# martellab-sri/ModalTune

Measured on AMD Instinct MI355X. Metric: slides/sec (train step) at 10k patches x 1536-d, higher is better.
Workload: dtype f16; 1 GPU; Prov-GigaPath ModalAdapter train step, 10000 patches x 1536-d, 6 pathways -> 64 gene tokens + 1 task token, 3 task passes, fp16 operands / fp32 accumulate, 1 slide per GPU per step, task passes as two concurrent groups (B = 2 | 1 on two HIP streams), train mode: Dropout(0.25) on the embedded input and both backbone branches, DropPath(0..0.1) per layer and on the Extractor FFN (Philox masks regener; patches=10000, parallelism=dp1, dropout=True

## Files before the change

include/modaltune_hip.h:

```cpp
#ifndef MODALTUNE_HIP_H
#define MODALTUNE_HIP_H

#include <stdint.h>

#ifdef __cplusplus
extern "C" {
#endif

typedef void* mt_stream_t;
typedef uint16_t mt_half;

typedef enum {
  MT_OK = 0,
  MT_ERR_BAD_ARG = -1,
  MT_ERR_LAUNCH = -2,
  MT_ERR_UNSUPPORTED = -3
} MtStatus;

typedef struct { int seg_rows, seg_stride, row0; } MtRowMap;

int mt_version(void);
const char* mt_status_string(int status);
const char* mt_build_id(void);

// ... 60 lines not shown
  float* rowsum;
  float* pre_out;
  const float* resid;
  MtDropout c_drop;
  const float* a_aux; int a_act;
  MtDropout a_drop;
  float resid_scale; int a_ld;
} MtSgemm;
int mt_sgemm_multi(const MtSgemm* probs, int n, mt_stream_t stream);

int mt_layernorm_fwd(const void* x, long ldx, const MtRowMap* xmap, int in_dtype, int gelu_in, const float* w,
                     const float* b, const float* add_rows, int add_period, void* y, long ldy, const MtRowMap* ymap,
                     int out_dtype, float* stats, int M, int D, mt_stream_t stream);
int mt_layernorm_fwd_live(const void* x, long ldx, const MtRowMap* xmap, int in_dtype, int gelu_in, const float* w,
                          const float* b, const float* add_rows, int add_period, void* y, long ldy, const MtRowMap* ymap,
                          int out_dtype, float* stats, int M, int D, const int* live, int live_rows, mt_stream_t stream);
int mt_add_layernorm_fwd(const float* x, const mt_half* branch, const MtDropout* drop, const float* w, const float* b,
                         float* h, mt_half* y, float* stats, int M, int D, mt_stream_t stream);

int mt_layernorm_fwd_eps(const void* x, long ldx, const MtRowMap* xmap, int in_dtype, int gelu_in, const float* w,
                         const float* b, const float* add_rows, int add_period, void* y, long ldy, const MtRowMap* ymap,
                         int out_dtype, float* stats, int M, int D, float eps, mt_stream_t stream);
int mt_add_layernorm_fwd_eps(const float* x, const mt_half* branch, const MtDropout* drop, const float* w, const float* b,
                             float* h, mt_half* y, float* stats, int M, int D, float eps, mt_stream_t stream);

int mt_layernorm_bwd(const void* dy, long lddy, const MtRowMap* dymap, int dy_dtype, const void* x, long ldx,
                     const MtRowMap* xmap, int in_dtype, int gelu_in, const float* w, const float* stats, void* dx,
                     long lddx, const MtRowMap* dxmap, int dx_dtype, int accumulate, float* dw, float* db,
                     mt_half* dx_f16, const MtDropout* dx_f16_drop, int M, int D, mt_stream_t stream);

int mt_layernorm_bwd_live(const void* dy, long lddy, const MtRowMap* dymap, int dy_dtype, const void* x, long ldx,
                          const MtRowMap* xmap, int in_dtype, int gelu_in, const float* w, const float* stats, void* dx,
                          long lddx, const MtRowMap* dxmap, int dx_dtype, int accumulate, float* dw, float* db,
                          mt_half* dx_f16, const MtDropout* dx_f16_drop, int M, int D, const int* live, int live_rows,
                          mt_stream_t stream);

#define MT_MAX_BRANCHES 8
#define MT_QK_SCALE_LOG2 0.20823509396846288f
typedef struct {
  int nbranch;
  int N;
  int B;
  int seg[MT_MAX_BRANCHES];
  int ratio[MT_MAX_BRANCHES];
  int nseg[MT_MAX_BRANCHES];
  int n[MT_MAX_BRANCHES];
  int qlimit[MT_MAX_BRANCHES];
} MtDilatedPlan;

int mt_dilated_attn_fwd(const mt_half* qkv, const MtDilatedPlan* plan, mt_half* o_br, float* lse_br,
                        mt_stream_t stream);

int mt_dilated_attn_fwd_live(const mt_half* qkv, const MtDilatedPlan* plan, mt_half* o_br, float* lse_br, const int* live,
                             mt_stream_t stream);

int mt_dilated_mix_ln_fwd(const mt_half* o_br, const float* lse_br, const MtDilatedPlan* plan, const float* ln_w,
                          const float* ln_b, mt_half* y, float* stats, float* lse_tot, mt_stream_t stream);

int mt_dilated_mix_ln_bwd(const mt_half* dy, const mt_half* o_br, const float* lse_br, const float* lse_tot,
                          const MtDilatedPlan* plan, const float* ln_w, const float* stats, mt_half* dmixed,
                          float* delta_br, mt_stream_t stream);
int mt_dilated_mix_ln_fwd_live(const mt_half* o_br, const float* lse_br, const MtDilatedPlan* plan, const float* ln_w,
                               const float* ln_b, mt_half* y, float* stats, float* lse_tot, const int* live, mt_stream_t stream);
int mt_dilated_mix_ln_bwd_live(const mt_half* dy, const mt_half* o_br, const float* lse_br, const float* lse_tot,
                               const MtDilatedPlan* plan, const float* ln_w, const float* stats, mt_half* dmixed,
                               float* delta_br, const int* live, mt_stream_t stream);
int mt_dilated_mix_ln_fwd_grid(const mt_half* o_br, const float* lse_br, const MtDilatedPlan* plan, const float* ln_w,
                               const float* ln_b, mt_half* y, float* stats, float* lse_tot, int grid_wgs, mt_stream_t stream);
int mt_dilated_mix_ln_bwd_grid(const mt_half* dy, const mt_half* o_br, const float* lse_br, const float* lse_tot,
                               const MtDilatedPlan* plan, const float* ln_w, const float* stats, mt_half* dmixed,
                               float* delta_br, int grid_wgs, mt_stream_t stream);

long mt_dilated_attn_bwd_workspace_bytes(const MtDilatedPlan* plan);
enum { MT_ATTN_BWD_KV = 1, MT_ATTN_BWD_Q = 2, MT_ATTN_BWD_COMBINE = 4, MT_ATTN_BWD_ALL = 7 };
int mt_dilated_attn_bwd(const mt_half* qkv, const mt_half* dmixed, const float* lse_tot, const float* delta_br,
                        const MtDilatedPlan* plan, void* workspace, mt_half* dqkv, int phases, mt_stream_t stream);
int mt_dilated_attn_bwd_inplace(const mt_half* qkv, const mt_half* dmixed, const float* lse_tot, const float* delta_br,
                                const MtDilatedPlan* plan, void* workspace, mt_half* dqkv, int phases, mt_stream_t stream);

int mt_dilated_attn_bwd_inplace_live(const mt_half* qkv, const mt_half* dmixed, const float* lse_tot, const float* delta_br,
                                     const MtDilatedPlan* plan, void* workspace, mt_half* dqkv, int phases, const int* live,
                                     mt_stream_t stream);

#define MT_DENSE_QK_SCALE_LOG2 0.18033688011112042f
typedef struct {
  int N;
  int B;
  int H;
  const mt_half* dist;
  const float* nslope;
} MtDensePlan;
long mt_alibi_dist_halves(int N);
int mt_alibi_dist(const int* cells, int N, mt_half* table, mt_stream_t stream);
int mt_dense_attn_fwd(const mt_half* qkv, const MtDensePlan* plan, mt_half* o, float* lse, mt_stream_t stream);
enum { MT_DENSE_BWD_DELTA = 1, MT_DENSE_BWD_KV = 2, MT_DENSE_BWD_Q = 4, MT_DENSE_BWD_ALL = 7 };
int mt_dense_attn_bwd(const mt_half* qkv, const mt_half* o, const mt_half* d_o, const float* lse, const MtDensePlan* plan,
                      float* delta, mt_half* dqkv, int phases, mt_stream_t stream);

int mt_gelu_f16_fwd(const mt_half* x, mt_half* y, long n, mt_stream_t stream);
int mt_gelu_f16_bwd(const mt_half* x, const mt_half* dy, mt_half* dx, long n, mt_stream_t stream);

long mt_pool_attn_workspace_floats(int B, int N, int heads, int nq);
int mt_pool_attn_fwd(const float* q, const mt_half* kv, int B, int N, int E, int heads, int nq, float* out, float* scores,
                     float* lse, float* workspace, mt_stream_t stream);
int mt_pool_attn_bwd(const float* q, const mt_half* kv, const float* scores, const float* lse, const float* out,
                     const float* dout, int B, int N, int E, int heads, int nq, mt_half* dkv, mt_stream_t stream);

typedef struct {
  const float *ln1_w, *ln1_b, *inner_ln_w, *inner_ln_b, *ln2_w, *ln2_b, *ffn_ln_w, *ffn_ln_b;
  const float *b_qkv, *b_out, *b_fc1, *b_fc2;
  const mt_half *w_qkv, *w_out, *w_fc1, *w_fc2;
  const mt_half *wt_qkv, *wt_out, *wt_fc1, *wt_fc2;
} MtLongNetLayerWeights;
typedef struct {
  float *hin, *hmid; mt_half *qkv, *o_br; float *lse_br, *lse_tot; mt_half* a1; float *st1, *stin, *st2, *stf;
  mt_half *u16, *br16, *t16;
  float* dh; mt_half *dy16, *dh16, *dt16, *da1, *dmixed, *dqkv16; float* delta; void* attn_ws;
  const int *live_attn, *live_ffn;
} MtLongNetLayerBuffers;
enum { MT_LAYER_ALL = 0x7fffffff };
enum { MT_LNF_LN1 = 1 << 0, MT_LNF_QKV = 1 << 1, MT_LNF_ATTN = 1 << 2, MT_LNF_MIX = 1 << 3, MT_LNF_OUT = 1 << 4, MT_LNF_LN2 = 1 << 5,
       MT_LNF_FC1 = 1 << 6, MT_LNF_FFN_LN = 1 << 7, MT_LNF_FC2 = 1 << 8 };
int mt_longnet_layer_fwd(const MtLongNetLayerWeights* w, const MtLongNetLayerBuffers* b, const MtDilatedPlan* plan, int M, int D, int F,
                         const float* pend_x, const mt_half* pend_branch, const MtDropout* pend_drop, int defer, float* out,
                         const MtDropout* drop_attn, const MtDropout* drop_ffn, int steps, mt_stream_t stream);
enum { MT_LNB_CAST = 1 << 0, MT_LNB_FC2 = 1 << 1, MT_LNB_FFN_LN = 1 << 2, MT_LNB_FC1 = 1 << 3, MT_LNB_LN2 = 1 << 4, MT_LNB_OUT = 1 << 5,
       MT_LNB_MIX = 1 << 6, MT_LNB_ATTN_SHIFT = 7, MT_LNB_QKV = 1 << 10, MT_LNB_LN1 = 1 << 11 };
int mt_longnet_layer_bwd(const MtLongNetLayerWeights* w, const MtLongNetLayerBuffers* b, const MtDilatedPlan* plan, int M, int D, int F,
                         int dh16_valid, int feeds_lower, const MtDropout* drop_attn, const MtDropout* drop_ffn,
                         const MtDropout* drop_lower_ffn, int steps, mt_stream_t stream);
typedef struct {
  const float *n1_w, *n1_b, *n2_w, *n2_b; float n1_eps, n2_eps;
  const float *b_qkv, *b_proj, *b_fc1, *b_fc2;
  const mt_half *w_qkv, *w_proj, *w_fc1, *w_fc2;
  const mt_half *wt_qkv, *wt_proj, *wt_fc1, *wt_fc2;
} MtVitBlockWeights;
typedef struct {
  float *hin, *hmid; mt_half *qkv, *o16; float* lse; mt_half* a1; float *st1, *st2;
  mt_half *u16, *br16, *t16;
  float* dh; mt_half *dy16, *dh16, *dt16, *da1, *dqkv16; float* delta;
} MtVitBlockBuffers;
enum { MT_VBF_LN1 = 1 << 0, MT_VBF_QKV = 1 << 1, MT_VBF_ATTN = 1 << 2, MT_VBF_PROJ = 1 << 3, MT_VBF_LN2 = 1 << 4, MT_VBF_FC1 = 1 << 5,
       MT_VBF_GELU = 1 << 6, MT_VBF_FC2 = 1 << 7 };
int mt_vit_block_fwd(const MtVitBlockWeights* w, const MtVitBlockBuffers* b, const MtDensePlan* plan, int M, int D, int F,
                     const float* pend_x, const mt_half* pend_branch, int defer, float* out, int steps, mt_stream_t stream);
enum { MT_VBB_CAST = 1 << 0, MT_VBB_FC2 = 1 << 1, MT_VBB_GELU = 1 << 2, MT_VBB_FC1 = 1 << 3, MT_VBB_LN2 = 1 << 4, MT_VBB_PROJ = 1 << 5,
       MT_VBB_ATTN_SHIFT = 6, MT_VBB_QKV = 1 << 9, MT_VBB_LN1 = 1 << 10 };
int mt_vit_block_bwd(const MtVitBlockWeights* w, const MtVitBlockBuffers* b, const MtDensePlan* plan, int M, int D, int F,
                     int dh16_valid, int feeds_lower, int steps, mt_stream_t stream);

int mt_inject_attn_fwd(const mt_half* q, int M, int rows_per_pass, const float* k, const float* v, int T,
                       mt_half* a, float* lse, mt_stream_t stream);
int mt_inject_attn_bwd(const mt_half* q, const mt_half* a, const float* lse, const mt_half* da, int M,
                       int rows_per_pass, const float* k, const float* v, int T, mt_half* dq, float* dk, float* dv,
                       mt_stream_t stream);

int mt_extract_attn_fwd(const float* q, const mt_half* kv, int B, int T, int L, float* out, float* lse,
                        float* part_acc, float* part_ml, int nsplit, mt_stream_t stream);
int mt_extract_attn_bwd(const float* q, const mt_half* kv, const float* out, const float* lse, const float* dout,
                        int B, int T, int L, float* dq, mt_half* dkv, mt_stream_t stream);

int mt_inject_attn_fwd_hd(const mt_half* q, int M, int rows_per_pass, const float* k, const float* v, int T, int heads,
                          int head_dim, mt_half* a, float* lse, mt_stream_t stream);
int mt_inject_attn_bwd_hd(const mt_half* q, const mt_half* a, const float* lse, const mt_half* da, int M,
                          int rows_per_pass, const float* k, const float* v, int T, int heads, int head_dim, mt_half* dq,
                          float* dk, float* dv, mt_stream_t stream);
int mt_extract_attn_fwd_hd(const float* q, const mt_half* kv, int B, int T, int L, int heads, int head_dim, float* out,
                           float* lse, float* part_acc, float* part_ml, int nsplit, mt_stream_t stream);
int mt_extract_attn_bwd_hd(const float* q, const mt_half* kv, const float* out, const float* lse, const float* dout,
                           int B, int T, int L, int heads, int head_dim, float* dq, mt_half* dkv, mt_stream_t stream);

int mt_gene_snn_fwd(const float* params, const long* offs, const int* sizes, const long* goff, const float* genes, int G,
                    int latent, int passes, float* a1, float* a2, float* z, const MtDropout* alpha_drop, mt_stream_t stream);
int mt_gene_snn_bwd(const float* params, float* grads, const long* offs, const int* sizes, const long* goff,
                    const float* genes, int G, int latent, int passes, const float* a1, const float* a2, const float* dz,
                    const MtDropout* alpha_drop, mt_stream_t stream);

int mt_gene_snn_fwd_points(const float* params, const long* offs, const int* sizes, const long* goff, const float* genes,
                           const float* baseline, const float* alphas, int G, int latent, int points, float* a1, float* a2, float* z,
                           mt_stream_t stream);
int mt_gene_snn_bwd_input(const float* params, const long* offs, const int* sizes, const long* goff, int G, int latent, int points,
                          const float* a1, const float* a2, const float* dz, const float* weights, const float* unscale,
                          float* dgenes, int accumulate, mt_stream_t stream);
int mt_ig_finalize(const float* genes, const float* baseline, const float* dgenes, const int* sizes, const long* goff, int G,
                   float* attr, float* pathway, mt_stream_t stream);

int mt_token_mha_fwd(const float* q, const float* k, const float* v, int B, int T, int E, int heads, float* out,
                     float* probs, mt_stream_t stream);
int mt_token_mha_bwd(const float* q, const float* k, const float* v, const float* probs, const float* dout, int B,
                     int T, int E, int heads, float* dq, float* dk, float* dv, mt_stream_t stream);

int mt_extract_attn_probs(const float* q, const mt_half* kv, const float* lse, int B, int T, int L, float* w, mt_stream_t stream);
int mt_inject_attn_probs(const mt_half* q, int M, int rows_per_pass, const float* k, const float* lse, int T, float* w,
                         mt_stream_t stream);
int mt_extract_attn_probs_hd(const float* q, const mt_half* kv, const float* lse, int B, int T, int L, int heads,
                             int head_dim, float* w, mt_stream_t stream);
int mt_inject_attn_probs_hd(const mt_half* q, int M, int rows_per_pass, const float* k, const float* lse, int T, int heads,
                            int head_dim, float* w, mt_stream_t stream);
int mt_token_probs_mean(const float* probs, int B, int heads, int T, float* out, mt_stream_t stream);

int mt_cast_f32_to_f16(const float* x, mt_half* y, long n, const MtDropout* drop, int D, mt_stream_t stream);
// ... 75 lines not shown
```

modaltune_amd/_lib.py:

```python
from __future__ import annotations

import ctypes as C
import os

_HERE = os.path.dirname(os.path.abspath(__file__))
LIB_PATH = os.environ.get("MODALTUNE_HIP_LIB", os.path.join(_HERE, "_C", "libmodaltune_hip.so"))

P, I, L, F, D = C.c_void_p, C.c_int, C.c_long, C.c_float, C.c_double


class MtRowMap(C.Structure):
    _fields_ = [("seg_rows", I), ("seg_stride", I), ("row0", I)]


class MtDropout(C.Structure):
    _fields_ = [("rng", P), ("site", C.c_uint), ("p", F), ("path_site", C.c_uint), ("path_p", F), ("rows_per_pass", I)]


class MtGemmEpilogue(C.Structure):
    _fields_ = [("bias", P), ("resid", P), ("ldr", L), ("rmap", MtRowMap), ("colscale", P),
                ("pos_table", P), ("pos_row", P), ("pos_col", P), ("drop", MtDropout)]


MT_SGEMM_MAX = 3


class MtSgemm(C.Structure):
    _fields_ = [("A", P), ("as0", L), ("as1", L), ("a_bs", L), ("B", P), ("bs0", L), ("bs1", L), ("b_bs", L),
                ("bias", P), ("bias_on_m", I), ("C", P), ("cs0", L), ("cs1", L), ("c_bs", L),
                ("M", I), ("N", I), ("K", I), ("batch", I), ("act", I), ("accumulate", I),
                ("rowsum", P), ("pre_out", P), ("resid", P), ("c_drop", MtDropout),
                ("a_aux", P), ("a_act", I), ("a_drop", MtDropout), ("resid_scale", F), ("a_ld", I)]


MT_MAX_BRANCHES = 8


class MtDilatedPlan(C.Structure):
    _fields_ = [("nbranch", I), ("N", I), ("B", I), ("seg", I * MT_MAX_BRANCHES), ("ratio", I * MT_MAX_BRANCHES),
                ("nseg", I * MT_MAX_BRANCHES), ("n", I * MT_MAX_BRANCHES), ("qlimit", I * MT_MAX_BRANCHES)]


class MtDensePlan(C.Structure):
    _fields_ = [("N", I), ("B", I), ("H", I), ("dist", P), ("nslope", P)]


class MtLongNetLayerWeights(C.Structure):
    _fields_ = [(n, P) for n in ("ln1_w", "ln1_b", "inner_ln_w", "inner_ln_b", "ln2_w", "ln2_b", "ffn_ln_w", "ffn_ln_b", "b_qkv", "b_out",
                                 "b_fc1", "b_fc2", "w_qkv", "w_out", "w_fc1", "w_fc2", "wt_qkv", "wt_out", "wt_fc1", "wt_fc2")]


class MtLongNetLayerBuffers(C.Structure):
    _fields_ = [(n, P) for n in ("hin", "hmid", "qkv", "o_br", "lse_br", "lse_tot", "a1", "st1", "stin", "st2", "stf", "u16", "br16", "t16",
                                 "dh", "dy16", "dh16", "dt16", "da1", "dmixed", "dqkv16", "delta", "attn_ws", "live_attn", "live_ffn")]


class MtVitBlockWeights(C.Structure):
    _fields_ = [(n, P) for n in ("n1_w", "n1_b", "n2_w", "n2_b")] + [("n1_eps", F), ("n2_eps", F)] + \
               [(n, P) for n in ("b_qkv", "b_proj", "b_fc1", "b_fc2", "w_qkv", "w_proj", "w_fc1", "w_fc2", "wt_qkv", "wt_proj", "wt_fc1", "wt_fc2")]


class MtVitBlockBuffers(C.Structure):
    _fields_ = [(n, P) for n in ("hin", "hmid", "qkv", "o16", "lse", "a1", "st1", "st2", "u16", "br16", "t16", "dh", "dy16", "dh16", "dt16",
                                 "da1", "dqkv16", "delta")]


RM = C.POINTER(MtRowMap)
DR = C.POINTER(MtDropout)
EP = C.POINTER(MtGemmEpilogue)
PL = C.POINTER(MtDilatedPlan)
DP = C.POINTER(MtDensePlan)

SIGNATURES = {
    "mt_version": [],
    "mt_status_string": [I],
    "mt_build_id": [],
    "mt_gemm_nt_f16": [P, L, RM, P, I, I, I, I, EP, P, L, RM, I, P],
    "mt_gemm_tn_f16": [P, L, RM, P, L, RM, I, I, I, P, L, P, P],
    "mt_colsum_f16": [P, L, RM, I, I, P, P],
    "mt_sgemm_small": [P, L, L, L, P, L, L, L, P, I, P, L, L, L, I, I, I, I, I, I, P, P],
    "mt_sgemm_multi": [C.POINTER(MtSgemm), I, P],
    "mt_layernorm_fwd": [P, L, RM, I, I, P, P, P, I, P, L, RM, I, P, I, I, P],
    "mt_add_layernorm_fwd": [P, P, DR, P, P, P, P, P, I, I, P],
    "mt_layernorm_fwd_eps": [P, L, RM, I, I, P, P, P, I, P, L, RM, I, P, I, I, F, P],
    "mt_add_layernorm_fwd_eps": [P, P, DR, P, P, P, P, P, I, I, F, P],
    "mt_layernorm_bwd": [P, L, RM, I, P, L, RM, I, I, P, P, P, L, RM, I, I, P, P, P, DR, I, I, P],
    "mt_droppath_live": [P, P, I, I, P, P, P],
    "mt_gemm_nt_f16_live": [P, L, RM, P, I, I, I, I, EP, P, L, RM, I, P, I, P],
    "mt_layernorm_fwd_live": [P, L, RM, I, I, P, P, P, I, P, L, RM, I, P, I, I, P, I, P],
    "mt_layernorm_bwd_live": [P, L, RM, I, P, L, RM, I, I, P, P, P, L, RM, I, I, P, P, P, DR, I, I, P, I, P],
    "mt_dilated_attn_fwd_live": [P, PL, P, P, P, P],
    "mt_dilated_mix_ln_fwd_live": [P, P, PL, P, P, P, P, P, P, P],
    "mt_dilated_mix_ln_bwd_live": [P, P, P, P, PL, P, P, P, P, P, P],
    "mt_dilated_attn_bwd_inplace_live": [P, P, P, P, PL, P, P, I, P, P],
    "mt_dilated_attn_fwd": [P, PL, P, P, P],
    "mt_dilated_mix_ln_fwd": [P, P, PL, P, P, P, P, P, P],
    "mt_dilated_mix_ln_bwd": [P, P, P, P, PL, P, P, P, P, P],
    "mt_dilated_mix_ln_fwd_grid": [P, P, PL, P, P, P, P, P, I, P],
    "mt_dilated_mix_ln_bwd_grid": [P, P, P, P, PL, P, P, P, P, I, P],
    "mt_dilated_attn_bwd_workspace_bytes": [PL],
    "mt_dilated_attn_bwd": [P, P, P, P, PL, P, P, I, P],
    "mt_dilated_attn_bwd_inplace": [P, P, P, P, PL, P, P, I, P],
    "mt_gene_snn_fwd": [P, P, P, P, P, I, I, I, P, P, P, DR, P],
    "mt_gene_snn_bwd": [P, P, P, P, P, P, I, I, I, P, P, P, DR, P],
    "mt_gene_snn_fwd_points": [P, P, P, P, P, P, P, I, I, I, P, P, P, P],
    "mt_gene_snn_bwd_input": [P, P, P, P, I, I, I, P, P, P, P, P, P, I, P],
    "mt_ig_finalize": [P, P, P, P, P, I, P, P, P],
    "mt_inject_attn_fwd": [P, I, I, P, P, I, P, P, P],
    "mt_inject_attn_bwd": [P, P, P, P, I, I, P, P, I, P, P, P, P],
    "mt_extract_attn_fwd": [P, P, I, I, I, P, P, P, P, I, P],
    "mt_extract_attn_bwd": [P, P, P, P, P, I, I, I, P, P, P],
    "mt_inject_attn_fwd_hd": [P, I, I, P, P, I, I, I, P, P, P],
    "mt_inject_attn_bwd_hd": [P, P, P, P, I, I, P, P, I, I, I, P, P, P, P],
    "mt_extract_attn_fwd_hd": [P, P, I, I, I, I, I, P, P, P, P, I, P],
    "mt_extract_attn_bwd_hd": [P, P, P, P, P, I, I, I, I, I, P, P, P],
    "mt_token_mha_fwd": [P, P, P, I, I, I, I, P, P, P],
    "mt_token_mha_bwd": [P, P, P, P, P, I, I, I, I, P, P, P, P],
    "mt_extract_attn_probs": [P, P, P, I, I, I, P, P],
    "mt_inject_attn_probs": [P, I, I, P, P, I, P, P],
    "mt_extract_attn_probs_hd": [P, P, P, I, I, I, I, I, P, P],
    "mt_inject_attn_probs_hd": [P, I, I, P, P, I, I, I, P, P],
    "mt_token_probs_mean": [P, I, I, I, P, P],
    "mt_cast_f32_to_f16": [P, P, L, DR, I, P],
    "mt_rng_advance": [P, P],
    "mt_dropout_f32": [P, L, RM, P, I, I, DR, P],
    "mt_droppath_rows_f32": [P, I, I, DR, P],
    "mt_cast_f16_to_f32": [P, P, L, P],
    "mt_pack_weight_f16": [P, I, I, P, I, P],
    "mt_pack_weights_f16": [P, I, P],
    "mt_act_fwd": [P, P, L, I, P],
    "mt_act_bwd": [P, P, P, L, I, P],
    "mt_axpy": [P, P, F, P, L, P],
    "mt_axpy_bcast": [P, P, F, P, L, L, P],
    "mt_fold_rows": [P, I, L, P, P],
    "mt_copy_rows_f32": [P, L, RM, P, L, RM, I, I, I, P],
    "mt_inject_resid_bwd": [P, L, RM, P, L, RM, P, P, P, L, RM, I, P, P, I, I, P],
    "mt_l2norm_rows": [P, P, I, I, P],
    "mt_distill_loss": [P, P, I, I, F, P, P, P, P],
    "mt_adamw_step": [P, P, P, P, L, D, D, D, D, D, I, P, F, P, P, P, P],
    "mt_scaler_update": [P, P, P, P, F, F, I, P],
    "mt_check_finite": [P, L, P, P],
    "mt_absmax_scale": [P, L, F, P, P],
    "mt_axpy_dev": [P, P, P, P, L, P],
    "mt_coords_to_grid": [P, I, F, I, P, P, P, P],
    "mt_mfma_probe": [P, I, I, P],
    "mt_longnet_layer_fwd": [P, P, PL, I, I, I, P, P, DR, I, P, DR, DR, I, P],
    "mt_longnet_layer_bwd": [P, P, PL, I, I, I, I, I, DR, DR, DR, I, P],
    "mt_vit_block_fwd": [P, P, DP, I, I, I, P, P, I, P, I, P],
    "mt_vit_block_bwd": [P, P, DP, I, I, I, I, I, I, P],
    "mt_alibi_dist": [P, I, P, P],
    "mt_alibi_dist_halves": [I],
    "mt_dense_attn_fwd": [P, DP, P, P, P],
    "mt_dense_attn_bwd": [P, P, P, P, DP, P, P, I, P],
    "mt_gelu_f16_fwd": [P, P, L, P],
    "mt_gelu_f16_bwd": [P, P, P, L, P],
    "mt_pool_attn_workspace_floats": [I, I, I, I],
    "mt_pool_attn_fwd": [P, P, I, I, I, I, I, P, P, P, P, P],
    "mt_pool_attn_bwd": [P, P, P, P, P, P, I, I, I, I, I, P, P],
    "mt_titan_grid": [P, I, F, P, P, P, P],
    "mt_titan_cell_sums": [P, L, P, I, I, P, P, P, P, P],
    "mt_titan_token_order": [P, P, P, I, P, P, P, P],
    "mt_titan_gather_tokens": [P, P, I, I, P, P],
    "mt_scatter_rows_f32": [P, P, P, P, I, I, I, P],
    "mt_row_absmax_f32": [P, P, I, I, P],
    "mt_gemm_tn_f16_det_elems": [I, I, I, I],
    "mt_gemm_tn_f16_det": [P, L, RM, P, L, RM, I, I, I, P, L, P, P, L, P],
    "mt_colsum_f16_det_elems": [I, I],
    "mt_colsum_f16_det": [P, L, RM, I, I, P, P, L, P],
    "mt_layernorm_bwd_det_elems": [I, I],
    "mt_layernorm_bwd_det": [P, L, RM, I, P, L, RM, I, I, P, P, P, L, RM, I, I, P, P, P, DR, I, I, P, L, P],
    "mt_inject_resid_bwd_det_elems": [I, I],
    "mt_inject_resid_bwd_det": [P, L, RM, P, L, RM, P, P, P, L, RM, I, P, P, I, I, P, L, P],
    "mt_inject_attn_bwd_hd_det_elems": [I, I, I, I, I],
    "mt_inject_attn_bwd_hd_det": [P, P, P, P, I, I, P, P, I, I, I, P, P, P, P, L, P],
    "mt_extract_attn_bwd_hd_det_elems": [I, I, I, I, I],
    "mt_extract_attn_bwd_hd_det": [P, P, P, P, P, I, I, I, I, I, P, P, P, L, P],
}
_RESTYPE = {"mt_status_string": C.c_char_p, "mt_build_id": C.c_char_p, "mt_dilated_attn_bwd_workspace_bytes": C.c_long, "mt_pool_attn_workspace_floats": C.c_long,
             "mt_alibi_dist_halves": C.c_long,
             **{n + "_det_elems": C.c_long for n in ("mt_gemm_tn_f16", "mt_colsum_f16", "mt_layernorm_bwd", "mt_inject_resid_bwd",
                                                     "mt_inject_attn_bwd_hd", "mt_extract_attn_bwd_hd")}}

_lib = None


def load():
    global _lib
    if _lib is not None:
        return _lib
    import torch
    if not os.path.exists(LIB_PATH):
        raise RuntimeError(
            f"modaltune_amd: {LIB_PATH} is missing -- run `python __graft_entry__.py` (hipcc, gfx950) first; "
            "there is no CPU/PyTorch fallback for the hot path")
    lib = C.CDLL(LIB_PATH)
    for name, args in SIGNATURES.items():
        fn = getattr(lib, name)
        fn.argtypes = args
        fn.restype = _RESTYPE.get(name, I)
    _lib = lib
    return lib


def build_info() -> dict:
    from ._build_id import tree_build_id
    bid = load().mt_build_id().decode()
    try:
        ok = bid == tree_build_id()
    except Exception:
        ok = None
    return {"build_id": bid, "build_id_matches_tree": ok, "lib": os.path.relpath(LIB_PATH, os.path.dirname(_HERE))}


def check(status: int, what: str = ""):
    if status != 0:
        msg = load().mt_status_string(status).decode()
        raise RuntimeError(f"modaltune_hip {what} failed: {msg} ({status})")


def rowmap(seg_rows=0, seg_stride=0, row0=0):
    return MtRowMap(seg_rows, seg_stride, row0)
```

modaltune_amd/csrc/attn.hip:

```cpp
#include "attn_common.h"

namespace {

template <bool LIVE>
__global__ __launch_bounds__(256) void dilated_attn_fwd_kernel(const h16* __restrict__ qkv, Plan p, h16* __restrict__ o_br,
                                                               float* __restrict__ lse_br) {
  __shared__ __attribute__((aligned(16))) h16 smem[4 * IMG_HALVES];
  h16* const Ks = smem;
  h16* const Vs = smem + 2 * IMG_HALVES;
  const int tid = threadIdx.x, lane = tid & 63, wave = tid >> 6;
  const int hh = lane >> 5, l31 = lane & 31;
  const WorkItem w = decode(p, blockIdx.x);
  const Seq sq = make_seq(p, w);
  const long M = (long)p.B * p.N;
  const int nv = __builtin_amdgcn_readfirstlane(sq.nvalid());
  const int nvq = min(nv, p.qlimit[w.br]);
  if (w.qt * 128 >= nvq || (LIVE && pass_dead(p, w.b))) return;

  {
    const int buf = tid >> 7, row = (tid >> 1) & 63, which = 6 + (tid & 1);
    const h16x8 one = {(h16)1.f, 0, 0, 0, (h16)1.f, 0, 0, 0}, zero = {0, 0, 0, 0, 0, 0, 0, 0};
    *reinterpret_cast<h16x8*>(&Vs[buf * IMG_HALVES + img_off(row, which)]) = which == 6 ? one : zero;
  }

  const int iq = w.qt * 128 + wave * 32 + l31;
  const bool qvalid = sq.valid(iq) && iq < nvq;
  const long qrow = sq.row_clamped(iq);
  h16x8 qf[3];
#pragma unroll
  for (int ks = 0; ks < 3; ++ks)
    qf[ks] = sel8(qvalid, ldg8(hm_ptr(qkv, M, w.h, qrow) + ks * 16 + hh * 8));

  const int ntile = (sq.n + 63) / 64;
  const int nproc = (nv + 63) >> 6;
  const int row_bytes = sq.dr * HD * 2;
  const long valid_bytes = (long)(nv - 1) * row_bytes + HD * 2;
  const long tile_bytes = 64L * row_bytes;
  const h16* const kseq = hm_ptr(qkv, M, H + w.h, sq.row(0));
  const h16* const vseq = hm_ptr(qkv, M, 2 * H + w.h, sq.row(0));
  const DmaLane dl(tid, row_bytes);
  auto dma = [&](int t) {
    dma_tile(Ks + (t & 1) * IMG_HALVES, tile_rsrc(kseq, t * tile_bytes, valid_bytes), dl);
    dma_tile(Vs + (t & 1) * IMG_HALVES, tile_rsrc(vseq, t * tile_bytes, valid_bytes), dl);
  };
  const int grp = lane >> 4, li = lane & 15, tq = li >> 2, tp = li & 3;
  int krd[3];
#pragma unroll
  for (int ks = 0; ks < 3; ++ks) krd[ks] = img_off(l31, 2 * ks + hh);
  const int vc = 2 * (grp & 1) + (tp >> 1), vo = 4 * (tp & 1);
  const int va0 = img_off(4 * hh + tq, vc) + vo, va1 = img_off(4 * hh + tq, vc + 4) + vo;
  const int vb0 = img_off(4 * hh + tq + 8, vc) + vo, vb1 = img_off(4 * hh + tq + 8, vc + 4) + vo;

  auto qk = [&](const h16* Kb, f32x16 (&s)[2], const f32x16& init) {
#pragma unroll
    for (int sub = 0; sub < 2; ++sub) {
#pragma unroll
      for (int ks = 0; ks < 3; ++ks) {
        const h16x8 kf = *reinterpret_cast<const h16x8*>(&Kb[sub * 32 * IMG_ROW + krd[ks]]);
        s[sub] = __builtin_amdgcn_mfma_f32_32x32x16_f16(kf, qf[ks], ks == 0 ? init : s[sub], 0, 0, 0);
      }
    }
  };

  f32x16 o0, o1;
#pragma unroll
  for (int i = 0; i < 16; ++i) { o0[i] = 0.f; o1[i] = 0.f; }

  dma(0);
  dma_wait_all();
  __syncthreads();
  float m2;
  f32x16 minit;
  {
    f32x16 s0[2], zero;
#pragma unroll
    for (int i = 0; i < 16; ++i) zero[i] = 0.f;
    qk(Ks, s0, zero);
    float mx = NEG_BIG;
#pragma unroll
    for (int sub = 0; sub < 2; ++sub)
#pragma unroll
      for (int i = 0; i < 16; ++i) {
        const int kidx = sub * 32 + (i & 3) + 8 * (i >> 2) + 4 * hh;
        mx = fmaxf(mx, kidx < sq.n ? s0[sub][i] : NEG_BIG);
      }
    m2 = max_halves(mx);
#pragma unroll
    for (int i = 0; i < 16; ++i) minit[i] = -m2;
  }

  auto tile = [&](int t, auto tail_tag) {
    constexpr bool TAIL = decltype(tail_tag)::value;
    const int kb = t * 64;
    const h16* Kb = Ks + (t & 1) * IMG_HALVES;
    const h16* Vb = Vs + (t & 1) * IMG_HALVES;
    if (t + 1 < nproc) dma(t + 1);
    f32x16 s_cur[2];
    qk(Kb, s_cur, minit);
    float mx = NEG_BIG;
#pragma unroll
    for (int sub = 0; sub < 2; ++sub)
#pragma unroll
      for (int i = 0; i < 16; ++i) {
        if (TAIL) {
          const int kidx = kb + sub * 32 + (i & 3) + 8 * (i >> 2) + 4 * hh;
          if (kidx >= sq.n) s_cur[sub][i] = NEG_BIG;
        }
        mx = fmaxf(mx, s_cur[sub][i]);
      }
    mx = max_halves(mx);
    if (__any(mx > RESCALE_LOG2)) {
      const float up = fmaxf(mx, 0.f);
      const float alpha = __builtin_amdgcn_exp2f(-up);
#pragma unroll
      for (int i = 0; i < 16; ++i) { o0[i] *= alpha; o1[i] *= alpha; s_cur[0][i] -= up; s_cur[1][i] -= up; }
      m2 += up;
#pragma unroll
      for (int i = 0; i < 16; ++i) minit[i] = -m2;
    }
#pragma unroll
    for (int sub = 0; sub < 2; ++sub)
#pragma unroll
      for (int s2 = 0; s2 < 2; ++s2) {
        h16x8 pf;
#pragma unroll
        for (int e = 0; e < 8; e += 2) {
          const f32x2 a = pk_exp2((f32x2){s_cur[sub][8 * s2 + e], s_cur[sub][8 * s2 + e + 1]});
          pf[e] = (h16)a[0]; pf[e + 1] = (h16)a[1];
        }
        const h16* vblk = Vb + (sub * 32 + s2 * 16) * IMG_ROW;
        const h16x8 v0 = cat8(lds_tr4(vblk + va0), lds_tr4(vblk + vb0));
        const h16x8 v1 = cat8(lds_tr4(vblk + va1), lds_tr4(vblk + vb1));
        o0 = __builtin_amdgcn_mfma_f32_32x32x16_f16(v0, pf, o0, 0, 0, 0);
        o1 = __builtin_amdgcn_mfma_f32_32x32x16_f16(v1, pf, o1, 0, 0, 0);
      }
    dma_wait_all();
    __syncthreads();
  };
  const bool tail_last = nproc == ntile && (sq.n & 63);
  const int nplain = tail_last ? nproc - 1 : nproc;
  for (int t = 0; t < nplain; ++t) tile(t, std::false_type{});
  if (tail_last) tile(nproc - 1, std::true_type{});
  const int rest = sq.n - nproc * 64;
  if (rest > 0) {
    if (__any(-m2 > RESCALE_LOG2)) {
      const float up = fmaxf(-m2, 0.f);
      const float alpha = __builtin_amdgcn_exp2f(-up);
#pragma unroll
      for (int i = 0; i < 16; ++i) { o0[i] *= alpha; o1[i] *= alpha; }
      m2 += up;
    }
    o1[8] += (float)rest * __builtin_amdgcn_exp2f(-m2);
  }

  if (qvalid) {
    const float l = o1[8];
    const float inv = 1.0f / l;
    h16* orow = o_br + ((long)w.br * M + qrow) * DM + w.h * HD;
#pragma unroll
    for (int gq = 0; gq < 4; ++gq) {
      h16x4 v = {(h16)(o0[4 * gq] * inv), (h16)(o0[4 * gq + 1] * inv), (h16)(o0[4 * gq + 2] * inv), (h16)(o0[4 * gq + 3] * inv)};
      *reinterpret_cast<h16x4*>(orow + 8 * gq + 4 * hh) = v;
    }
#pragma unroll
    for (int gq = 0; gq < 2; ++gq) {
      h16x4 v = {(h16)(o1[4 * gq] * inv), (h16)(o1[4 * gq + 1] * inv), (h16)(o1[4 * gq + 2] * inv), (h16)(o1[4 * gq + 3] * inv)};
      *reinterpret_cast<h16x4*>(orow + 32 + 8 * gq + 4 * hh) = v;
    }
    if (hh == 0) lse_br[((long)w.br * M + qrow) * H + w.h] = (m2 + __log2f(l)) * LN2;
  }
}

struct MixGeom {
  int grp[MT_MAX_BRANCHES];
  MT_DEVINL MixGeom(const Plan& p, int h) {
#pragma unroll
    for (int b = 0; b < MT_MAX_BRANCHES; ++b) grp[b] = b < p.nbranch ? h / (H / p.ratio[b]) : -1;
  }
};
MT_DEVINL void seg_split(const Plan& p, int b, int pos, int& j, int& loc) {
  const int sg = p.seg[b];
  if (sg >= p.N) { j = 0; loc = pos; return; }
  j = (int)((float)pos * p.inv_seg[b]);
  loc = pos - j * sg;
  if (loc < 0) { loc += sg; --j; }
  if (loc >= sg) { loc -= sg; ++j; }
}
MT_DEVINL int residue(const Plan& p, int b, int pos) {
  int j, loc;
  seg_split(p, b, pos, j, loc);
  const int dr = p.ratio[b];
  return (dr & (dr - 1)) == 0 ? (loc & (dr - 1)) : loc % dr;
}
MT_DEVINL int dense_branch(const Plan& p) {
  int d = 0;
#pragma unroll
  for (int b = 0; b < MT_MAX_BRANCHES; ++b) if (b < p.nbranch && p.ratio[b] == 1) d = b;
  return d;
}
constexpr int MIX_CPL = 24;
struct H24 { h16x8 a, b, c; };
MT_DEVINL H24 ld24(const h16* p) {
  return H24{*reinterpret_cast<const h16x8*>(p), *reinterpret_cast<const h16x8*>(p + 8), *reinterpret_cast<const h16x8*>(p + 16)};
}
MT_DEVINL float h24(const H24& v, int e) { return (float)(e < 8 ? v.a[e & 7] : e < 16 ? v.b[e & 7] : v.c[e & 7]); }
MT_DEVINL float half_sum(float v) {
#pragma unroll
  for (int o = 16; o > 0; o >>= 1) v += __shfl_xor(v, o, 64);
  return v;
}

template <int NB>
__global__ __launch_bounds__(256) void mix_ln_fwd_kernel(const h16* __restrict__ o_br, const float* __restrict__ lse_br, Plan p,
                                                         const float* __restrict__ ln_w, const float* __restrict__ ln_b,
                                                         h16* __restrict__ y, float* __restrict__ stats, float* __restrict__ lse_tot) {
  const int lane = threadIdx.x & 63, wave = __builtin_amdgcn_readfirstlane(threadIdx.x >> 6), sub = lane >> 5, l5 = lane & 31;
  const long M = (long)p.B * p.N;
  const int h = l5 >> 1, c0 = l5 * MIX_CPL;
  const MixGeom geo(p, h);
  const int db = dense_branch(p);
  float w[MIX_CPL], bb[MIX_CPL];
#pragma unroll
  for (int e = 0; e < MIX_CPL; ++e) { w[e] = ln_w[c0 + e]; bb[e] = ln_b[c0 + e]; }
  const LivePasses lp = live_passes(p);
  const long m_end = min(M, (long)lp.b1 * p.N);
  for (long m2 = (long)lp.b0 * p.N + ((long)blockIdx.x * 4 + wave) * 2; m2 < m_end; m2 += (long)gridDim.x * 8) {
    const bool live = m2 + sub < m_end;
    const long m = live ? m2 + sub : m_end - 1;
    const int pos = (int)(m % p.N);
    bool cov[NB];
    float lse[NB];
    H24 ob[NB];
#pragma unroll
    for (int b = 0; b < NB; ++b) {
      cov[b] = b < p.nbranch && geo.grp[b] == residue(p, b, pos);
      const int sb = cov[b] ? b : db;
      lse[b] = lse_br[((long)sb * M + m) * H + h];
      ob[b] = ld24(o_br + ((long)sb * M + m) * DM + c0);
    }
    float mx = NEG_BIG;
#pragma unroll
    for (int b = 0; b < NB; ++b) { lse[b] = cov[b] ? lse[b] : NEG_BIG; mx = fmaxf(mx, lse[b]); }
    float den = 0.f;
#pragma unroll
    for (int b = 0; b < NB; ++b) den += cov[b] ? __expf(lse[b] - mx) : 0.f;
    const float tot = mx + __logf(den);
    float v[MIX_CPL];
#pragma unroll
    for (int e = 0; e < MIX_CPL; ++e) v[e] = 0.f;
#pragma unroll
    for (int b = 0; b < NB; ++b) {
      const float wgt = cov[b] ? __expf(lse[b] - tot) : 0.f;
#pragma unroll
      for (int e = 0; e < MIX_CPL; ++e) v[e] = fmaf(wgt, cov[b] ? h24(ob[b], e) : 0.f, v[e]);
    }
    float s = 0.f;
#pragma unroll
    for (int e = 0; e < MIX_CPL; ++e) s += v[e];
    const float mean = half_sum(s) * (1.0f / DM);
    float q = 0.f;
#pragma unroll
    for (int e = 0; e < MIX_CPL; ++e) { const float d = v[e] - mean; q += d * d; }
    const float rstd = rsqrtf(half_sum(q) * (1.0f / DM) + 1e-5f);
    if (live) {
      h16* dst = y + m * DM + c0;
#pragma unroll
      for (int k = 0; k < 3; ++k) {
        h16x8 o;
#pragma unroll
        for (int e = 0; e < 8; ++e) o[e] = (h16)((v[8 * k + e] - mean) * rstd * w[8 * k + e] + bb[8 * k + e]);
        *reinterpret_cast<h16x8*>(dst + 8 * k) = o;
      }
      if (l5 == 0) { stats[2 * m] = mean; stats[2 * m + 1] = rstd; }
      if ((l5 & 1) == 0) lse_tot[m * H + h] = tot;
    }
  }
}

template <int NB>
__global__ __launch_bounds__(256) void mix_ln_bwd_kernel(const h16* __restrict__ dy, const h16* __restrict__ o_br,
                                                         const float* __restrict__ lse_br, const float* __restrict__ lse_tot, Plan p,
                                                         const float* __restrict__ ln_w, const float* __restrict__ stats,
                                                         h16* __restrict__ dmixed, float* __restrict__ delta_br) {
  const int lane = threadIdx.x & 63, wave = __builtin_amdgcn_readfirstlane(threadIdx.x >> 6), sub = lane >> 5, l5 = lane & 31;
  const long M = (long)p.B * p.N;
  const int h = l5 >> 1, c0 = l5 * MIX_CPL;
  const MixGeom geo(p, h);
  const int db = dense_branch(p);
  float w[MIX_CPL];
#pragma unroll
  for (int e = 0; e < MIX_CPL; ++e) w[e] = ln_w[c0 + e];
  const LivePasses lp = live_passes(p);
  const long m_end = min(M, (long)lp.b1 * p.N);
  for (long m2 = (long)lp.b0 * p.N + ((long)blockIdx.x * 4 + wave) * 2; m2 < m_end; m2 += (long)gridDim.x * 8) {
    const bool live = m2 + sub < m_end;
    const long m = live ? m2 + sub : m_end - 1;
    const int pos = (int)(m % p.N);
    const float tot = lse_tot[m * H + h];
    const float mean = stats[2 * m], rstd = stats[2 * m + 1];
    const H24 dyv = ld24(dy + m * DM + c0);
    bool cov[NB];
    float lse[NB];
    H24 ob[NB];
#pragma unroll
    for (int b = 0; b < NB; ++b) {
      cov[b] = b < p.nbranch && geo.grp[b] == residue(p, b, pos);
      const int sb = cov[b] ? b : db;
      lse[b] = lse_br[((long)sb * M + m) * H + h];
      ob[b] = ld24(o_br + ((long)sb * M + m) * DM + c0);
    }
    float v[MIX_CPL];
#pragma unroll
    for (int e = 0; e < MIX_CPL; ++e) v[e] = 0.f;
#pragma unroll
    for (int b = 0; b < NB; ++b) {
      const float wgt = cov[b] ? __expf(lse[b] - tot) : 0.f;
#pragma unroll
      for (int e = 0; e < MIX_CPL; ++e) v[e] = fmaf(wgt, cov[b] ? h24(ob[b], e) : 0.f, v[e]);
    }
    float g[MIX_CPL], xh[MIX_CPL];
    float s1 = 0.f, s2 = 0.f;
#pragma unroll
    for (int i = 0; i < MIX_CPL; ++i) {
      xh[i] = (v[i] - mean) * rstd;
      g[i] = h24(dyv, i) * w[i];
      s1 += g[i]; s2 = fmaf(g[i], xh[i], s2);
    }
    const float c1 = half_sum(s1) * (1.0f / DM), c2 = half_sum(s2) * (1.0f / DM);
    float dm[MIX_CPL];
    h16* dst = dmixed + ((long)h * M + m) * HD + (c0 - h * HD);
#pragma unroll
    for (int k = 0; k < 3; ++k) {
      h16x8 o;
#pragma unroll
      for (int e = 0; e < 8; ++e) {
        const int i = 8 * k + e;
        o[e] = (h16)(rstd * (g[i] - c1 - xh[i] * c2));
        dm[i] = (float)o[e];
      }
      if (live) *reinterpret_cast<h16x8*>(dst + 8 * k) = o;
    }
#pragma unroll
    for (int b = 0; b < NB; ++b) {
      float d = 0.f;
#pragma unroll
      for (int e = 0; e < MIX_CPL; ++e) d = fmaf(dm[e], h24(ob[b], e), d);
      d += __shfl_xor(d, 1, 64);
      if (live && (l5 & 1) == 0 && cov[b]) delta_br[((long)b * M + m) * H + h] = d;
    }
  }
}


}

extern "C" int mt_dilated_attn_fwd_live(const mt_half* qkv, const MtDilatedPlan* plan, mt_half* o_br, float* lse_br, const int* live,
                                        mt_stream_t stream) {
  if (!qkv || !o_br || !lse_br || !plan_ok(plan)) return MT_ERR_BAD_ARG;
  const Plan p = make_plan(plan, 128, live);
  const int nblk = p.blk_off[p.nbranch];
  if (p.live) hipLaunchKernelGGL(dilated_attn_fwd_kernel<true>, dim3(nblk), dim3(256), 0, (hipStream_t)stream, (const h16*)qkv, p,
                     (h16*)o_br, lse_br);
  else hipLaunchKernelGGL(dilated_attn_fwd_kernel<false>, dim3(nblk), dim3(256), 0, (hipStream_t)stream, (const h16*)qkv, p,
                     (h16*)o_br, lse_br);
  MT_CHECK_LAUNCH();
  return MT_OK;
}

extern "C" int mt_dilated_attn_fwd(const mt_half* qkv, const MtDilatedPlan* plan, mt_half* o_br, float* lse_br,
                                   mt_stream_t stream) {
  return mt_dilated_attn_fwd_live(qkv, plan, o_br, lse_br, nullptr, stream);
}

constexpr int MIX_CUS = 256, MIX_FWD_WG_PER_CU = 3, MIX_BWD_WG_PER_CU = 2;
static dim3 mix_grid(long M, int grid_wgs, int wg_per_cu) {
  return dim3((int)min((M + 7) / 8, (long)(grid_wgs > 0 ? grid_wgs : wg_per_cu * MIX_CUS)));
}

namespace {
int mix_ln_fwd(const mt_half* o_br, const float* lse_br, const MtDilatedPlan* plan, const float* ln_w, const float* ln_b, mt_half* y,
               float* stats, float* lse_tot, int grid_wgs, const int* live, mt_stream_t stream) {
  if (!o_br || !lse_br || !ln_w || !ln_b || !y || !stats || !lse_tot || !plan_ok(plan)) return MT_ERR_BAD_ARG;
  const Plan p = make_plan(plan, 128, live);
  const long M = (long)p.B * p.N;
  const dim3 grid = mix_grid(M, grid_wgs, MIX_FWD_WG_PER_CU);
  if (p.nbranch <= 5)
    hipLaunchKernelGGL(mix_ln_fwd_kernel<5>, grid, dim3(256), 0, (hipStream_t)stream, (const h16*)o_br, lse_br, p, ln_w, ln_b,
                       (h16*)y, stats, lse_tot);
  else
    hipLaunchKernelGGL(mix_ln_fwd_kernel<MT_MAX_BRANCHES>, grid, dim3(256), 0, (hipStream_t)stream, (const h16*)o_br, lse_br, p,
                       ln_w, ln_b, (h16*)y, stats, lse_tot);
  MT_CHECK_LAUNCH();
  return MT_OK;
}
}

extern "C" int mt_dilated_mix_ln_fwd_grid(const mt_half* o_br, const float* lse_br, const MtDilatedPlan* plan,
                                          const float* ln_w, const float* ln_b, mt_half* y, float* stats, float* lse_tot,
                                          int grid_wgs, mt_stream_t stream) {
  return mix_ln_fwd(o_br, lse_br, plan, ln_w, ln_b, y, stats, lse_tot, grid_wgs, nullptr, stream);
}

extern "C" int mt_dilated_mix_ln_fwd(const mt_half* o_br, const float* lse_br, const MtDilatedPlan* plan,
                                     const float* ln_w, const float* ln_b, mt_half* y, float* stats, float* lse_tot,
                                     mt_stream_t stream) {
  return mix_ln_fwd(o_br, lse_br, plan, ln_w, ln_b, y, stats, lse_tot, 0, nullptr, stream);
}

extern "C" int mt_dilated_mix_ln_fwd_live(const mt_half* o_br, const float* lse_br, const MtDilatedPlan* plan,
                                          const float* ln_w, const float* ln_b, mt_half* y, float* stats, float* lse_tot,
                                          const int* live, mt_stream_t stream) {
  return mix_ln_fwd(o_br, lse_br, plan, ln_w, ln_b, y, stats, lse_tot, 0, live, stream);
}

namespace {
int mix_ln_bwd(const mt_half* dy, const mt_half* o_br, const float* lse_br, const float* lse_tot, const MtDilatedPlan* plan,
               const float* ln_w, const float* stats, mt_half* dmixed, float* delta_br, int grid_wgs, const int* live, mt_stream_t stream) {
  if (!dy || !o_br || !lse_br || !lse_tot || !ln_w || !stats || !dmixed || !delta_br || !plan_ok(plan)) return MT_ERR_BAD_ARG;
  const Plan p = make_plan(plan, 128, live);
  const long M = (long)p.B * p.N;
  const dim3 grid = mix_grid(M, grid_wgs, MIX_BWD_WG_PER_CU);
  if (p.nbranch <= 5)
    hipLaunchKernelGGL(mix_ln_bwd_kernel<5>, grid, dim3(256), 0, (hipStream_t)stream, (const h16*)dy, (const h16*)o_br, lse_br,
                       lse_tot, p, ln_w, stats, (h16*)dmixed, delta_br);
  else
    hipLaunchKernelGGL(mix_ln_bwd_kernel<MT_MAX_BRANCHES>, grid, dim3(256), 0, (hipStream_t)stream, (const h16*)dy,
                       (const h16*)o_br, lse_br, lse_tot, p, ln_w, stats, (h16*)dmixed, delta_br);
  MT_CHECK_LAUNCH();
  return MT_OK;
}
}

extern "C" int mt_dilated_mix_ln_bwd_grid(const mt_half* dy, const mt_half* o_br, const float* lse_br, const float* lse_tot,
                                          const MtDilatedPlan* plan, const float* ln_w, const float* stats, mt_half* dmixed,
                                          float* delta_br, int grid_wgs, mt_stream_t stream) {
  return mix_ln_bwd(dy, o_br, lse_br, lse_tot, plan, ln_w, stats, dmixed, delta_br, grid_wgs, nullptr, stream);
}

extern "C" int mt_dilated_mix_ln_bwd(const mt_half* dy, const mt_half* o_br, const float* lse_br, const float* lse_tot,
                                     const MtDilatedPlan* plan, const float* ln_w, const float* stats, mt_half* dmixed,
                                     float* delta_br, mt_stream_t stream) {
  return mix_ln_bwd(dy, o_br, lse_br, lse_tot, plan, ln_w, stats, dmixed, delta_br, 0, nullptr, stream);
}

extern "C" int mt_dilated_mix_ln_bwd_live(const mt_half* dy, const mt_half* o_br, const float* lse_br, const float* lse_tot,
                                          const MtDilatedPlan* plan, const float* ln_w, const float* stats, mt_half* dmixed,
                                          float* delta_br, const int* live, mt_stream_t stream) {
  return mix_ln_bwd(dy, o_br, lse_br, lse_tot, plan, ln_w, stats, dmixed, delta_br, 0, live, stream);
}

extern "C" long mt_dilated_attn_bwd_workspace_bytes(const MtDilatedPlan* plan) {
  if (!plan_ok(plan)) return MT_ERR_BAD_ARG;
  const Plan p = make_plan(plan, 128);
  return p.ws_off[p.nbranch] * (long)sizeof(h16);
}

namespace {
int attn_bwd(const mt_half* qkv, const mt_half* dmixed, const float* lse_tot, const float* delta_br, const MtDilatedPlan* plan,
             void* workspace, mt_half* dqkv, int phases, bool inplace, const int* live, mt_stream_t stream) {
  if (!qkv || !dmixed || !lse_tot || !delta_br || !workspace || !dqkv || !plan_ok(plan) || !(phases & 7)) return MT_ERR_BAD_ARG;
  hipStream_t s = (hipStream_t)stream;
  inplace = inplace && dense_branch_host(plan) >= 0;
  if (inplace && (long)plan->B * plan->N >= (1L << 31)) return MT_ERR_UNSUPPORTED;
  mt_half* dense_dst = inplace ? dqkv : nullptr;
  if (phases & MT_ATTN_BWD_KV) mt_attn::launch_bwd_kv(qkv, dmixed, lse_tot, delta_br, plan, workspace, dense_dst, live, s);
  if (phases & MT_ATTN_BWD_Q) mt_attn::launch_bwd_q(qkv, dmixed, lse_tot, delta_br, plan, workspace, dense_dst, live, s);
  if (phases & MT_ATTN_BWD_COMBINE) {
    if (inplace) mt_attn::launch_bwd_combine_inplace(workspace, plan, dqkv, live, s);
    else mt_attn::launch_bwd_combine(workspace, plan, dqkv, s);
  }
  MT_CHECK_LAUNCH();
  return MT_OK;
}
}

extern "C" int mt_dilated_attn_bwd(const mt_half* qkv, const mt_half* dmixed, const float* lse_tot,
                                   const float* delta_br, const MtDilatedPlan* plan, void* workspace, mt_half* dqkv,
                                   int phases, mt_stream_t stream) {
  return attn_bwd(qkv, dmixed, lse_tot, delta_br, plan, workspace, dqkv, phases, false, nullptr, stream);
}

extern "C" int mt_dilated_attn_bwd_inplace(const mt_half* qkv, const mt_half* dmixed, const float* lse_tot,
                                           const float* delta_br, const MtDilatedPlan* plan, void* workspace, mt_half* dqkv,
                                           int phases, mt_stream_t stream) {
  return attn_bwd(qkv, dmixed, lse_tot, delta_br, plan, workspace, dqkv, phases, true, nullptr, stream);
}

extern "C" int mt_dilated_attn_bwd_inplace_live(const mt_half* qkv, const mt_half* dmixed, const float* lse_tot,
                                                const float* delta_br, const MtDilatedPlan* plan, void* workspace, mt_half* dqkv,
                                                int phases, const int* live, mt_stream_t stream) {
  return attn_bwd(qkv, dmixed, lse_tot, delta_br, plan, workspace, dqkv, phases, true, live, stream);
}
```

modaltune_amd/csrc/attn_bwd_kv.hip:

```cpp
#include "attn_common.h"

namespace {

template <bool LIVE>
__global__ __launch_bounds__(256, 3) void dilated_attn_bwd_kv_kernel(const h16* __restrict__ qkv, const h16* __restrict__ dmixed,
                                                                  const float* __restrict__ lse_tot, const float* __restrict__ delta_br,
                                                                  Plan p, h16* __restrict__ ws, DenseDst dd) {
  __shared__ __attribute__((aligned(16))) h16 smem[4 * IMG_HALVES];
  __shared__ __attribute__((aligned(16))) float L2s[2][64];
  __shared__ __attribute__((aligned(16))) float Dls[2][64];
  h16* const Qx = smem;
  h16* const Dx = smem + 2 * IMG_HALVES;
  const int tid = threadIdx.x, lane = tid & 63, wave = tid >> 6;
  const int hh = lane >> 5, l31 = lane & 31;
  const WorkItem w = decode(p, blockIdx.x);
  const Seq sq = make_seq(p, w);
  const long M = (long)p.B * p.N;
  const h16x8 zero8 = {0, 0, 0, 0, 0, 0, 0, 0};
  const int nv = __builtin_amdgcn_readfirstlane(sq.nvalid());
  if (w.qt * 128 >= nv || (LIVE && pass_dead(p, w.b))) return;

  {
    const int img = tid >> 6, row = tid & 63;
    *reinterpret_cast<h16x8*>(&smem[img * IMG_HALVES + img_off(row, 6)]) = zero8;
    *reinterpret_cast<h16x8*>(&smem[img * IMG_HALVES + img_off(row, 7)]) = zero8;
  }

  const int ik = w.qt * 128 + wave * 32 + l31;
  const bool kvalid = sq.valid(ik);
  const long krow = sq.row_clamped(ik);
  h16x8 kf[3], vf[3];
#pragma unroll
  for (int ks = 0; ks < 3; ++ks) {
    kf[ks] = sel8(kvalid, ldg8(hm_ptr(qkv, M, H + w.h, krow) + ks * 16 + hh * 8));
    vf[ks] = sel8(kvalid, ldg8(hm_ptr(qkv, M, 2 * H + w.h, krow) + ks * 16 + hh * 8));
  }

  const int nvq = min(nv, p.qlimit[w.br]);
  const int ntile = (nvq + 63) >> 6;
  const int row_bytes = sq.dr * HD * 2;
  const long valid_bytes = (long)(nvq - 1) * row_bytes + HD * 2;
  const long tile_bytes = 64L * row_bytes;
  const h16* const qseq = hm_ptr(qkv, M, w.h, sq.row(0));
  const h16* const dseq = hm_ptr(dmixed, M, w.h, sq.row(0));
  const DmaLane dl(tid, row_bytes);
  const float* const lbase = lse_tot + sq.row(0) * H + w.h;
  const float* const dbase = delta_br + ((long)w.br * M + sq.row(0)) * H + w.h;
  float rl2 = 0.f, rdl = 0.f;
  auto issue = [&](int t) {
    dma_tile(Qx + (t & 1) * IMG_HALVES, tile_rsrc(qseq, t * tile_bytes, valid_bytes), dl);
    dma_tile(Dx + (t & 1) * IMG_HALVES, tile_rsrc(dseq, t * tile_bytes, valid_bytes), dl);
    if (tid < 64) {
      const long off = (long)min(t * 64 + lane, nvq - 1) * sq.dr * H;
      rl2 = lbase[off];
      rdl = dbase[off];
    }
  };
  auto publish = [&](int t) {
    if (tid < 64) {
      const bool ok = t * 64 + lane < nvq;
      L2s[t & 1][tid] = ok ? fmaf(-rl2, LOG2E, LOG2_LN2) : 0.f;
      Dls[t & 1][tid] = ok ? -rdl : 0.f;
    }
  };

  f32x16 dk0, dk1, dv0, dv1;
#pragma unroll
  for (int i = 0; i < 16; ++i) { dk0[i] = 0.f; dk1[i] = 0.f; dv0[i] = 0.f; dv1[i] = 0.f; }
  const int grp = lane >> 4, li = lane & 15, tq = li >> 2, tp = li & 3;
  int rrd[3];
#pragma unroll
  for (int ks = 0; ks < 3; ++ks) rrd[ks] = img_off(l31, 2 * ks + hh);
  const int trc = 2 * (grp & 1) + (tp >> 1), tro = 4 * (tp & 1);
  const int tr_a0 = img_off(4 * hh + tq, trc) + tro, tr_a1 = img_off(4 * hh + tq, trc + 4) + tro;
  const int tr_b0 = img_off(4 * hh + tq + 8, trc) + tro, tr_b1 = img_off(4 * hh + tq + 8, trc + 4) + tro;

  issue(0);
  publish(0);
  dma_wait_all();
  __syncthreads();
  for (int t = 0; t < ntile; ++t) {
    const h16* Qb = Qx + (t & 1) * IMG_HALVES;
    const h16* Db = Dx + (t & 1) * IMG_HALVES;
    const float* L2b = L2s[t & 1];
    const float* Dlb = Dls[t & 1];
    if (t + 1 < ntile) issue(t + 1);
#pragma unroll
    for (int sub = 0; sub < 2; ++sub) {
      f32x16 s, dp;
#pragma unroll
      for (int g4 = 0; g4 < 4; ++g4) {
        const f32x4 a = *reinterpret_cast<const f32x4*>(&L2b[sub * 32 + 8 * g4 + 4 * hh]);
        const f32x4 b = *reinterpret_cast<const f32x4*>(&Dlb[sub * 32 + 8 * g4 + 4 * hh]);
#pragma unroll
        for (int e = 0; e < 4; ++e) { s[4 * g4 + e] = a[e]; dp[4 * g4 + e] = b[e]; }
      }
      __builtin_amdgcn_sched_barrier(0);
      h16x8 qa[3], da[3];
#pragma unroll
      for (int ks = 0; ks < 3; ++ks) {
        qa[ks] = *reinterpret_cast<const h16x8*>(&Qb[sub * 32 * IMG_ROW + rrd[ks]]);
        da[ks] = *reinterpret_cast<const h16x8*>(&Db[sub * 32 * IMG_ROW + rrd[ks]]);
      }
#pragma unroll
      for (int ks = 0; ks < 3; ++ks) {
        s = __builtin_amdgcn_mfma_f32_32x32x16_f16(qa[ks], kf[ks], s, 0, 0, 0);
        dp = __builtin_amdgcn_mfma_f32_32x32x16_f16(da[ks], vf[ks], dp, 0, 0, 0);
      }
      __builtin_amdgcn_sched_group_barrier(0x100, 3, 0);
#pragma unroll
      for (int i = 0; i < 3; ++i) {
        __builtin_amdgcn_sched_group_barrier(0x8, 1, 0);
        __builtin_amdgcn_sched_group_barrier(0x100, 1, 0);
      }
      __builtin_amdgcn_sched_group_barrier(0x8, 3, 0);
      h16x8 pf[2], dsf[2];
#pragma unroll
      for (int i = 0; i < 16; i += 2) {
        const f32x2 pt = pk_exp2((f32x2){s[i], s[i + 1]});
        const f32x2 d = pt * (f32x2){dp[i], dp[i + 1]};
        pf[i >> 3][i & 7] = (h16)pt[0]; pf[i >> 3][(i & 7) + 1] = (h16)pt[1];
        dsf[i >> 3][i & 7] = (h16)d[0]; dsf[i >> 3][(i & 7) + 1] = (h16)d[1];
      }
#pragma unroll
      for (int s2 = 0; s2 < 2; ++s2) {
        const int rb = (sub * 32 + s2 * 16) * IMG_ROW;
        const h16x8 d0 = cat8(lds_tr4(&Db[rb + tr_a0]), lds_tr4(&Db[rb + tr_b0]));
        const h16x8 d1 = cat8(lds_tr4(&Db[rb + tr_a1]), lds_tr4(&Db[rb + tr_b1]));
        dv0 = __builtin_amdgcn_mfma_f32_32x32x16_f16(d0, pf[s2], dv0, 0, 0, 0);
        dv1 = __builtin_amdgcn_mfma_f32_32x32x16_f16(d1, pf[s2], dv1, 0, 0, 0);
        const h16x8 q0 = cat8(lds_tr4(&Qb[rb + tr_a0]), lds_tr4(&Qb[rb + tr_b0]));
        const h16x8 q1 = cat8(lds_tr4(&Qb[rb + tr_a1]), lds_tr4(&Qb[rb + tr_b1]));
        dk0 = __builtin_amdgcn_mfma_f32_32x32x16_f16(q0, dsf[s2], dk0, 0, 0, 0);
        dk1 = __builtin_amdgcn_mfma_f32_32x32x16_f16(q1, dsf[s2], dk1, 0, 0, 0);
      }
    }
    if (t + 1 < ntile) publish(t + 1);
    dma_wait_all();
    __syncthreads();
  }
  if (kvalid) {
    h16* outk = ws_base(ws, dd, w) + ws_slot(p, w, krow) + ws_which_stride(p, w.br);
    h16* outv = outk + ws_which_stride(p, w.br);
#pragma unroll
    for (int gq = 0; gq < 4; ++gq) {
      const h16x4 a = {(h16)dk0[4 * gq], (h16)dk0[4 * gq + 1], (h16)dk0[4 * gq + 2], (h16)dk0[4 * gq + 3]};
      const h16x4 b = {(h16)(dv0[4 * gq] * INV_LN2), (h16)(dv0[4 * gq + 1] * INV_LN2), (h16)(dv0[4 * gq + 2] * INV_LN2),
                       (h16)(dv0[4 * gq + 3] * INV_LN2)};
      *reinterpret_cast<h16x4*>(outk + 8 * gq + 4 * hh) = a;
      *reinterpret_cast<h16x4*>(outv + 8 * gq + 4 * hh) = b;
    }
#pragma unroll
    for (int gq = 0; gq < 2; ++gq) {
      const h16x4 a = {(h16)dk1[4 * gq], (h16)dk1[4 * gq + 1], (h16)dk1[4 * gq + 2], (h16)dk1[4 * gq + 3]};
      const h16x4 b = {(h16)(dv1[4 * gq] * INV_LN2), (h16)(dv1[4 * gq + 1] * INV_LN2), (h16)(dv1[4 * gq + 2] * INV_LN2),
                       (h16)(dv1[4 * gq + 3] * INV_LN2)};
      *reinterpret_cast<h16x4*>(outk + 32 + 8 * gq + 4 * hh) = a;
      *reinterpret_cast<h16x4*>(outv + 32 + 8 * gq + 4 * hh) = b;
    }
  }
}

}

void mt_attn::launch_bwd_kv(const mt_half* qkv, const mt_half* dmixed, const float* lse_tot, const float* delta_br, const MtDilatedPlan* plan, void* ws, mt_half* dense_dst, const int* live, hipStream_t s) {
  const Plan p = make_plan(plan, 128, live);
  if (p.live) hipLaunchKernelGGL(dilated_attn_bwd_kv_kernel<true>, dim3(p.blk_off[p.nbranch]), dim3(256), 0, s, (const h16*)qkv, (const h16*)dmixed, lse_tot, delta_br, p, (h16*)ws, make_dense_dst(plan, p, dense_dst));
  else hipLaunchKernelGGL(dilated_attn_bwd_kv_kernel<false>, dim3(p.blk_off[p.nbranch]), dim3(256), 0, s, (const h16*)qkv, (const h16*)dmixed, lse_tot, delta_br, p, (h16*)ws, make_dense_dst(plan, p, dense_dst));
}
```

modaltune_amd/csrc/attn_bwd_q.hip:

```cpp
#include "attn_common.h"

namespace {

template <bool LIVE>
__global__ __launch_bounds__(256) void dilated_attn_bwd_q_kernel(const h16* __restrict__ qkv, const h16* __restrict__ dmixed,
                                                                 const float* __restrict__ lse_tot, const float* __restrict__ delta_br,
                                                                 Plan p, h16* __restrict__ ws, DenseDst dd) {
  __shared__ __attribute__((aligned(16))) h16 smem[4 * IMG_HALVES];
  h16* const Ks = smem;
  h16* const Vs = smem + 2 * IMG_HALVES;
  const int tid = threadIdx.x, lane = tid & 63, wave = tid >> 6;
  const int hh = lane >> 5, l31 = lane & 31;
  const WorkItem w = decode(p, blockIdx.x);
  const Seq sq = make_seq(p, w);
  const long M = (long)p.B * p.N;
  const h16x8 zero8 = {0, 0, 0, 0, 0, 0, 0, 0};
  const int nv = __builtin_amdgcn_readfirstlane(sq.nvalid());
  const int nvq = min(nv, p.qlimit[w.br]);
  if (w.qt * 128 >= nvq || (LIVE && pass_dead(p, w.b))) return;

  {
    const int buf = tid >> 7, row = (tid >> 1) & 63, which = 6 + (tid & 1);
    *reinterpret_cast<h16x8*>(&Ks[buf * IMG_HALVES + img_off(row, which)]) = zero8;
  }

  const int iq = w.qt * 128 + wave * 32 + l31;
  const bool qvalid = sq.valid(iq) && iq < nvq;
  const long qrow = sq.row_clamped(iq);
  h16x8 qf[3], dof[3];
#pragma unroll
  for (int ks = 0; ks < 3; ++ks) {
    qf[ks] = sel8(qvalid, ldg8(hm_ptr(qkv, M, w.h, qrow) + ks * 16 + hh * 8));
    dof[ks] = sel8(qvalid, ldg8(hm_ptr(dmixed, M, w.h, qrow) + ks * 16 + hh * 8));
  }
  const float L2raw = lse_tot[qrow * H + w.h], dlraw = delta_br[((long)w.br * M + qrow) * H + w.h];
  const float nl2 = qvalid ? fmaf(-L2raw, LOG2E, LOG2_LN2) : -1.0e30f;
  const float ndl = qvalid ? -dlraw : 0.f;
  f32x16 nl2i, ndli;
#pragma unroll
  for (int i = 0; i < 16; ++i) { nl2i[i] = nl2; ndli[i] = ndl; }

  const int ntile = (nv + 63) >> 6;
  const int row_bytes = sq.dr * HD * 2;
  const long valid_bytes = (long)(nv - 1) * row_bytes + HD * 2;
  const long tile_bytes = 64L * row_bytes;
  const h16* const kseq = hm_ptr(qkv, M, H + w.h, sq.row(0));
  const h16* const vseq = hm_ptr(qkv, M, 2 * H + w.h, sq.row(0));
  const DmaLane dl(tid, row_bytes);
  auto dma = [&](int t) {
    dma_tile_pair(Ks + (t & 1) * IMG_HALVES, tile_rsrc(kseq, t * tile_bytes, valid_bytes), Vs + (t & 1) * IMG_HALVES,
                  tile_rsrc(vseq, t * tile_bytes, valid_bytes), dl, __builtin_amdgcn_readfirstlane(tid >> 6));
  };
  const int grp = lane >> 4, li = lane & 15, tq = li >> 2, tp = li & 3;
  int rrd[3];
#pragma unroll
  for (int ks = 0; ks < 3; ++ks) rrd[ks] = img_off(l31, 2 * ks + hh);
  const int kc = 2 * (grp & 1) + (tp >> 1), ko = 4 * (tp & 1);
  const int ka0 = img_off(4 * hh + tq, kc) + ko, ka1 = img_off(4 * hh + tq, kc + 4) + ko;
  const int kb0 = img_off(4 * hh + tq + 8, kc) + ko, kb1 = img_off(4 * hh + tq + 8, kc + 4) + ko;

  f32x16 dq0, dq1;
#pragma unroll
  for (int i = 0; i < 16; ++i) { dq0[i] = 0.f; dq1[i] = 0.f; }
  dma(0);
  dma_wait_all();
  __syncthreads();
  auto tile = [&](int t, auto tail_tag) {
    constexpr bool TAIL = decltype(tail_tag)::value;
    const int kb = t * 64;
    const h16* Kb = Ks + (t & 1) * IMG_HALVES;
    const h16* Vb = Vs + (t & 1) * IMG_HALVES;
    if (t + 1 < ntile) dma(t + 1);
#pragma unroll
    for (int sub = 0; sub < 2; ++sub) {
      f32x16 s, dp;
      h16x8 ka[3], va[3];
#pragma unroll
      for (int ks = 0; ks < 3; ++ks) {
        ka[ks] = *reinterpret_cast<const h16x8*>(&Kb[sub * 32 * IMG_ROW + rrd[ks]]);
        va[ks] = *reinterpret_cast<const h16x8*>(&Vb[sub * 32 * IMG_ROW + rrd[ks]]);
      }
#pragma unroll
      for (int ks = 0; ks < 3; ++ks) {
        s = __builtin_amdgcn_mfma_f32_32x32x16_f16(ka[ks], qf[ks], ks == 0 ? nl2i : s, 0, 0, 0);
        dp = __builtin_amdgcn_mfma_f32_32x32x16_f16(va[ks], dof[ks], ks == 0 ? ndli : dp, 0, 0, 0);
      }
      __builtin_amdgcn_sched_group_barrier(0x100, 3, 0);
#pragma unroll
      for (int i = 0; i < 3; ++i) {
        __builtin_amdgcn_sched_group_barrier(0x8, 1, 0);
        __builtin_amdgcn_sched_group_barrier(0x100, 1, 0);
      }
      __builtin_amdgcn_sched_group_barrier(0x8, 3, 0);
      h16x8 dsf[2];
#pragma unroll
      for (int i = 0; i < 16; i += 2) {
        f32x2 pt = pk_exp2((f32x2){s[i], s[i + 1]});
        if (TAIL) {
          const int kidx = kb + sub * 32 + (i & 3) + 8 * (i >> 2) + 4 * hh;
          if (kidx >= sq.n) pt[0] = 0.f;
          if (kidx + 1 >= sq.n) pt[1] = 0.f;
        }
        const f32x2 d = pt * (f32x2){dp[i], dp[i + 1]};
        dsf[i >> 3][i & 7] = (h16)d[0];
        dsf[i >> 3][(i & 7) + 1] = (h16)d[1];
      }
#pragma unroll
      for (int s2 = 0; s2 < 2; ++s2) {
        const h16* kblk = Kb + (sub * 32 + s2 * 16) * IMG_ROW;
        const h16x8 k0 = cat8(lds_tr4(kblk + ka0), lds_tr4(kblk + kb0));
        const h16x8 k1 = cat8(lds_tr4(kblk + ka1), lds_tr4(kblk + kb1));
        dq0 = __builtin_amdgcn_mfma_f32_32x32x16_f16(k0, dsf[s2], dq0, 0, 0, 0);
        dq1 = __builtin_amdgcn_mfma_f32_32x32x16_f16(k1, dsf[s2], dq1, 0, 0, 0);
      }
    }
    dma_wait_all();
    __syncthreads();
  };
  const bool tail_last = ntile * 64 > sq.n;
  const int nplain = tail_last ? ntile - 1 : ntile;
  for (int t = 0; t < nplain; ++t) tile(t, std::false_type{});
  if (tail_last) tile(ntile - 1, std::true_type{});
  if (qvalid) {
    h16* out = ws_base(ws, dd, w) + ws_slot(p, w, qrow);
#pragma unroll
    for (int gq = 0; gq < 4; ++gq) {
      const h16x4 v = {(h16)dq0[4 * gq], (h16)dq0[4 * gq + 1], (h16)dq0[4 * gq + 2], (h16)dq0[4 * gq + 3]};
      *reinterpret_cast<h16x4*>(out + 8 * gq + 4 * hh) = v;
    }
#pragma unroll
    for (int gq = 0; gq < 2; ++gq) {
      const h16x4 v = {(h16)dq1[4 * gq], (h16)dq1[4 * gq + 1], (h16)dq1[4 * gq + 2], (h16)dq1[4 * gq + 3]};
      *reinterpret_cast<h16x4*>(out + 32 + 8 * gq + 4 * hh) = v;
    }
  }
}

}

void mt_attn::launch_bwd_q(const mt_half* qkv, const mt_half* dmixed, const float* lse_tot, const float* delta_br, const MtDilatedPlan* plan, void* ws, mt_half* dense_dst, const int* live, hipStream_t s) {
  const Plan p = make_plan(plan, 128, live);
  if (p.live) hipLaunchKernelGGL(dilated_attn_bwd_q_kernel<true>, dim3(p.blk_off[p.nbranch]), dim3(256), 0, s, (const h16*)qkv, (const h16*)dmixed, lse_tot, delta_br, p, (h16*)ws, make_dense_dst(plan, p, dense_dst));
  else hipLaunchKernelGGL(dilated_attn_bwd_q_kernel<false>, dim3(p.blk_off[p.nbranch]), dim3(256), 0, s, (const h16*)qkv, (const h16*)dmixed, lse_tot, delta_br, p, (h16*)ws, make_dense_dst(plan, p, dense_dst));
}
```

modaltune_amd/csrc/attn_common.h:

```cpp
#pragma once
#include <stdlib.h>
#include <type_traits>

#include "common.h"

namespace {

constexpr int H = 16, HD = 48, DM = 768, QKV_LD = 2304;
constexpr int KSTR = 56;
constexpr int VSTR = 96;
constexpr float LOG2E = 1.4426950408889634f, LN2 = 0.6931471805599453f;
constexpr float NEG_BIG = -1.0e30f;
constexpr float RESCALE_LOG2 = 8.0f;
constexpr float QK_SCALE_LOG2 = 0.14433756729740643f * 1.4426950408889634f;
constexpr float LOG2_LN2 = -0.52876637294489768f;
constexpr float INV_LN2 = 1.4426950408889634f;

struct Plan {
  int nbranch, N, B;
  int seg[MT_MAX_BRANCHES], ratio[MT_MAX_BRANCHES], nseg[MT_MAX_BRANCHES], n[MT_MAX_BRANCHES];
  int order[MT_MAX_BRANCHES], qtiles[MT_MAX_BRANCHES], blk_off[MT_MAX_BRANCHES + 1];
  long ws_off[MT_MAX_BRANCHES + 1];
  float inv_seg[MT_MAX_BRANCHES];
  int qlimit[MT_MAX_BRANCHES];
  const int* live;
};

Plan make_plan(const MtDilatedPlan* p, int qtile, const int* live = nullptr) {
  Plan d;
  d.nbranch = p->nbranch; d.N = p->N; d.B = p->B; d.live = live;
  for (int i = 0; i < p->nbranch; ++i) {
    d.seg[i] = p->seg[i]; d.ratio[i] = p->ratio[i]; d.nseg[i] = p->nseg[i]; d.n[i] = p->n[i];
    d.order[i] = i;
    d.qtiles[i] = cdiv(p->n[i], qtile);
    d.inv_seg[i] = 1.0f / (float)p->seg[i];
    d.qlimit[i] = p->qlimit[i] > 0 ? p->qlimit[i] : p->n[i];
  }
  for (int i = 0; i < d.nbranch; ++i)
    for (int j = i + 1; j < d.nbranch; ++j)
      if (d.n[d.order[j]] > d.n[d.order[i]]) { int t = d.order[i]; d.order[i] = d.order[j]; d.order[j] = t; }
  d.blk_off[0] = 0;
  for (int i = 0; i < d.nbranch; ++i) {
    const int b = d.order[i];
    d.blk_off[i + 1] = d.blk_off[i] + d.B * d.nseg[b] * H * d.qtiles[b];
  }
  d.ws_off[0] = 0;
  for (int b = 0; b < d.nbranch; ++b) d.ws_off[b + 1] = d.ws_off[b] + (long)d.B * d.N * 3 * (H / d.ratio[b]) * HD;
  return d;
}

int dense_branch_host(const MtDilatedPlan* p) {
  int d = -1;
  for (int b = 0; b < p->nbranch; ++b) if (p->ratio[b] == 1) d = b;
  return d;
}

bool plan_ok(const MtDilatedPlan* p) {
  if (!p || p->nbranch < 1 || p->nbranch > MT_MAX_BRANCHES || p->N < 1 || p->B < 1) return false;
  for (int i = 0; i < p->nbranch; ++i) {
    const int r = p->ratio[i], s = p->seg[i];
    if (r < 1 || r > H || (H % r) != 0 || s < 1 || s > p->N) return false;
    if (p->nseg[i] != cdiv(p->N, s) || p->n[i] != cdiv(s, r)) return false;
    if (p->qlimit[i] < 0 || p->qlimit[i] > p->n[i]) return false;
  }
  return true;
}

struct WorkItem { int br, b, j, h, qt; };

MT_DEVINL WorkItem decode(const Plan& p, int bid) {
  const int x = bid & 7, j = bid >> 3;
  int oi = 0;
#pragma unroll
  for (int i = 1; i < MT_MAX_BRANCHES; ++i)
    if (i < p.nbranch && j >= (p.blk_off[i] >> 3)) oi = i;
  WorkItem w;
  w.br = p.order[oi];
  int local = j - (p.blk_off[oi] >> 3);
  w.qt = local % p.qtiles[w.br];
  const int gid = (local / p.qtiles[w.br]) * 8 + x;
  w.h = gid % H;
  const int r = gid / H;
  w.j = r % p.nseg[w.br];
  w.b = r / p.nseg[w.br];
  w.br = __builtin_amdgcn_readfirstlane(w.br); w.qt = __builtin_amdgcn_readfirstlane(w.qt);
  w.h = __builtin_amdgcn_readfirstlane(w.h); w.j = __builtin_amdgcn_readfirstlane(w.j);
  w.b = __builtin_amdgcn_readfirstlane(w.b);
  return w;
}

struct LivePasses { int b0, b1; };
MT_DEVINL LivePasses live_passes(const Plan& p) {
  LivePasses r = {0, p.B};
  if (p.live) { r.b0 = max(p.live[0], 0); r.b1 = min(p.live[1], p.B); }
  return r;
}
MT_DEVINL bool pass_dead(const Plan& p, int b) {
  const LivePasses r = live_passes(p);
  return b < r.b0 || b >= r.b1;
}

MT_DEVINL WorkItem decode_branch(const Plan& p, int br, int bid) {
  const int x = bid & 7, j = bid >> 3;
  WorkItem w;
  w.br = br;
  w.qt = j % p.qtiles[br];
  const int gid = (j / p.qtiles[br]) * 8 + x;
  w.h = gid % H;
  const int r = gid / H;
  w.j = r % p.nseg[br];
  w.b = r / p.nseg[br];
  return w;
}

MT_DEVINL int swz(int row, int chunk) { return row * VSTR + ((chunk ^ ((row >> 2) & 3)) << 3); }

MT_DEVINL h16x4 lds_tr4(const h16* p) {
  s16x4 r = __builtin_amdgcn_ds_read_tr16_b64_v4i16(
      (__attribute__((address_space(3))) s16x4*)(__attribute__((address_space(3))) void*)p);
  return __builtin_bit_cast(h16x4, r);
}
MT_DEVINL h16x8 cat8(h16x4 lo, h16x4 hi) { return (h16x8){lo[0], lo[1], lo[2], lo[3], hi[0], hi[1], hi[2], hi[3]}; }

struct Seq {
  int n, s, dr, r, seg_base, N;
  long row_base;
  MT_DEVINL bool valid(int i) const {
    const int loc = r + i * dr;
    return i < n && loc < s && seg_base + loc < N;
  }
  MT_DEVINL long row(int i) const { return row_base + seg_base + r + (long)i * dr; }
  MT_DEVINL long row_clamped(int i) const { return min(row(i), row_base + (long)N - 1); }
  MT_DEVINL int nvalid() const {
    const int lim = min(s, N - seg_base) - r;
    return lim <= 0 ? 0 : min(n, (lim + dr - 1) / dr);
  }
};

MT_DEVINL const h16* hm_ptr(const h16* base, long M, int slab, long row) { return base + ((long)slab * M + row) * HD; }

MT_DEVINL h16x8 ldg8_off(const h16* base, uint32_t byte_off) {
  return *reinterpret_cast<const h16x8*>(reinterpret_cast<const char*>(base) + byte_off);
}
MT_DEVINL float ldf_off(const float* base, uint32_t byte_off) {
  return *reinterpret_cast<const float*>(reinterpret_cast<const char*>(base) + byte_off);
}
typedef __attribute__((ext_vector_type(4))) unsigned int u32x4;
MT_DEVINL __amdgpu_buffer_rsrc_t make_rsrc(const void* base) {
  return __builtin_amdgcn_make_buffer_rsrc(const_cast<void*>(base), 0, 0x7fffffff, 0x00020000);
}
MT_DEVINL h16x8 buf_ldg8(__amdgpu_buffer_rsrc_t r, uint32_t voff, uint32_t soff) {
  return __builtin_bit_cast(h16x8, __builtin_amdgcn_raw_buffer_load_b128(r, voff, soff, 0));
}
MT_DEVINL float buf_ldf(__amdgpu_buffer_rsrc_t r, uint32_t voff, uint32_t soff) {
  return __builtin_bit_cast(float, __builtin_amdgcn_raw_buffer_load_b32(r, voff, soff, 0));
}
MT_DEVINL f32x2 pk_fma(f32x2 a, f32x2 b, f32x2 c) { return __builtin_elementwise_fma(a, b, c); }
MT_DEVINL f32x2 pk_exp2(f32x2 a) { return (f32x2){__builtin_amdgcn_exp2f(a[0]), __builtin_amdgcn_exp2f(a[1])}; }

MT_DEVINL float max_halves(float x) {
  float lo = x, hi = x;
  asm volatile("s_nop 1\n\tv_permlane32_swap_b32 %0, %1" : "+v"(lo), "+v"(hi));
  return fmaxf(lo, hi);
}

MT_DEVINL h16x8 sel8(bool ok, h16x8 v) {
  const h16x8 z = {0, 0, 0, 0, 0, 0, 0, 0};
  return ok ? v : z;
}

MT_DEVINL long ws_slot(const Plan& p, const WorkItem& w, long token_row) {
  const int hb = H / p.ratio[w.br];
  return p.ws_off[w.br] + (token_row * 3) * (hb * HD) + (w.h % hb) * HD;
}
MT_DEVINL int ws_which_stride(const Plan& p, int br) { return (H / p.ratio[br]) * HD; }
struct DenseDst { h16* base; int br; };
DenseDst make_dense_dst(const MtDilatedPlan* plan, const Plan& p, mt_half* dense_dst) {
  const int db = dense_dst ? dense_branch_host(plan) : -1;
  return DenseDst{db >= 0 ? (h16*)dense_dst - p.ws_off[db] : nullptr, db};
}
MT_DEVINL h16* ws_base(h16* ws, const DenseDst& dd, const WorkItem& w) { return w.br == dd.br ? dd.base : ws; }

MT_DEVINL Seq make_seq(const Plan& p, const WorkItem& w) {
  Seq q;
  q.n = p.n[w.br]; q.s = p.seg[w.br]; q.dr = p.ratio[w.br];
  q.r = __builtin_amdgcn_readfirstlane(w.h / (H / q.dr));
  q.seg_base = w.j * q.s; q.N = p.N; q.row_base = (long)w.b * p.N;
  return q;
}

constexpr int IMG_ROW = 64;
constexpr int IMG_HALVES = 64 * IMG_ROW;
MT_DEVINL int img_f(int row) { return (((row >> 1) & 1) << 2) | ((row >> 2) & 3); }
MT_DEVINL int img_off(int row, int chunk) { return row * IMG_ROW + ((chunk ^ img_f(row)) << 3); }

struct DmaLane {
  uint32_t voff[2]; bool act[2]; int lds_halves[2];
  MT_DEVINL DmaLane(int tid, int row_stride_bytes) {
    const int wave = tid >> 6, j = tid & 63;
#pragma unroll
    for (int i = 0; i < 2; ++i) {
      const int piece = 2 * wave + i, row = 8 * piece + (j >> 3);
      const int c = (j & 7) ^ img_f(row);
      act[i] = c < 6;
      voff[i] = (uint32_t)(row * row_stride_bytes + min(c, 5) * 16);
      lds_halves[i] = piece * 512;
    }
  }
};
MT_DEVINL __amdgpu_buffer_rsrc_t tile_rsrc(const h16* seq_base, long tile_byte_off, long valid_bytes) {
  const long left = valid_bytes - tile_byte_off;
  const int rec = (int)__builtin_amdgcn_readfirstlane((int)(left > 0 ? (left < 0x7fffffffL ? left : 0x7fffffffL) : 0));
  const char* b = reinterpret_cast<const char*>(seq_base) + tile_byte_off;
  const uint32_t lo = __builtin_amdgcn_readfirstlane((uint32_t)(uintptr_t)b), hi = __builtin_amdgcn_readfirstlane((uint32_t)((uintptr_t)b >> 32));
  return __builtin_amdgcn_make_buffer_rsrc(reinterpret_cast<void*>(((uintptr_t)hi << 32) | lo), 0, rec, 0x00020000);
}
MT_DEVINL void dma_tile(h16* img, __amdgpu_buffer_rsrc_t rs, const DmaLane& d) {
#pragma unroll
  for (int i = 0; i < 2; ++i)
    if (d.act[i])
      __builtin_amdgcn_raw_ptr_buffer_load_lds(rs, (__attribute__((address_space(3))) void*)(img + d.lds_halves[i]), 16, d.voff[i], 0, 0, 0);
}
MT_DEVINL void dma_tile_pair(h16* img_a, __amdgpu_buffer_rsrc_t ra, h16* img_b, __amdgpu_buffer_rsrc_t rb, const DmaLane& d, int wave_u) {
#pragma unroll
  for (int i = 0; i < 2; ++i)
    if (d.act[i]) {
      const int off = (2 * wave_u + i) * 512;
      __builtin_amdgcn_raw_ptr_buffer_load_lds(ra, (__attribute__((address_space(3))) void*)(img_a + off), 16, d.voff[i], 0, 0, 0);
      __builtin_amdgcn_raw_ptr_buffer_load_lds(rb, (__attribute__((address_space(3))) void*)(img_b + off), 16, d.voff[i], 0, 0, 0);
    }
}
MT_DEVINL void dma_wait_all() { asm volatile("s_waitcnt vmcnt(0)" ::: "memory"); }

struct StageIdx {
  int row0, part0, row1, part1; bool has1;
  MT_DEVINL StageIdx(int tid) {
    row0 = tid / 6; part0 = tid - row0 * 6;
    const int c = 256 + tid;
    row1 = c / 6; part1 = c - row1 * 6; has1 = tid < 128;
  }
};
struct StageRow {
  int row0, row1, part; bool act;
  MT_DEVINL StageRow(int tid) {
    row0 = tid >> 3; row1 = 32 + row0;
    act = (tid & 7) < 6;
    part = min(tid & 7, 5);
  }
};

}

namespace mt_attn {
void launch_bwd_kv(const mt_half* qkv, const mt_half* dmixed, const float* lse_tot, const float* delta_br, const MtDilatedPlan* plan, void* ws, mt_half* dense_dst, const int* live, hipStream_t s);
void launch_bwd_q(const mt_half* qkv, const mt_half* dmixed, const float* lse_tot, const float* delta_br, const MtDilatedPlan* plan, void* ws, mt_half* dense_dst, const int* live, hipStream_t s);
void launch_bwd_combine(const void* ws, const MtDilatedPlan* plan, mt_half* dqkv, hipStream_t s);
void launch_bwd_combine_inplace(const void* ws, const MtDilatedPlan* plan, mt_half* dqkv, const int* live, hipStream_t s);
}
```

modaltune_amd/csrc/layer.hip:

```cpp
#include "common.h"

namespace {

MtGemmEpilogue epi_bias(const float* bias) {
  MtGemmEpilogue e{};
  e.bias = bias;
  return e;
}
#define MT_TRY(call)              \
  do {                            \
    const int st__ = (call);      \
    if (st__ != MT_OK) return st__; \
  } while (0)
#define MT_STEP(bits, call) \
  do { if (steps & (bits)) MT_TRY(call); } while (0)

}

extern "C" int mt_longnet_layer_fwd(const MtLongNetLayerWeights* w, const MtLongNetLayerBuffers* b, const MtDilatedPlan* plan, int M,
                                    int D, int F, const float* pend_x, const mt_half* pend_branch, const MtDropout* pend_drop, int defer,
                                    float* out, const MtDropout* drop_attn, const MtDropout* drop_ffn, int steps, mt_stream_t s) {
  if (!w || !b || !plan || M < 1 || D != 768 || (!defer && !out)) return MT_ERR_BAD_ARG;
  if (!pend_x)
    MT_STEP(MT_LNF_LN1, mt_layernorm_fwd(b->hin, D, nullptr, MT_OUT_F32, 0, w->ln1_w, w->ln1_b, nullptr, 0, b->u16, D, nullptr, MT_OUT_F16, b->st1, M, D, s));
  else
    MT_STEP(MT_LNF_LN1, mt_add_layernorm_fwd(pend_x, pend_branch, pend_drop, w->ln1_w, w->ln1_b, b->hin, b->u16, b->st1, M, D, s));
  MtGemmEpilogue e = epi_bias(w->b_qkv);
  MT_STEP(MT_LNF_QKV, mt_gemm_nt_f16_live(b->u16, D, nullptr, w->w_qkv, M, 3 * D, D, MT_EPI_QKV_HM, &e, b->qkv, 3 * D, nullptr, MT_OUT_F16, b->live_attn,
                                          plan->N, s));
  MT_STEP(MT_LNF_ATTN, mt_dilated_attn_fwd_live(b->qkv, plan, b->o_br, b->lse_br, b->live_attn, s));
  MT_STEP(MT_LNF_MIX, mt_dilated_mix_ln_fwd_live(b->o_br, b->lse_br, plan, w->inner_ln_w, w->inner_ln_b, b->u16, b->stin, b->lse_tot, b->live_attn, s));
  e = epi_bias(w->b_out);
  MT_STEP(MT_LNF_OUT, mt_gemm_nt_f16_live(b->u16, D, nullptr, w->w_out, M, D, D, MT_EPI_BIAS, &e, b->br16, D, nullptr, MT_OUT_F16, b->live_attn, plan->N, s));
  MT_STEP(MT_LNF_LN2, mt_add_layernorm_fwd(b->hin, b->br16, drop_attn, w->ln2_w, w->ln2_b, b->hmid, b->u16, b->st2, M, D, s));
  e = epi_bias(w->b_fc1);
  MT_STEP(MT_LNF_FC1, mt_gemm_nt_f16_live(b->u16, D, nullptr, w->w_fc1, M, F, D, MT_EPI_BIAS, &e, b->a1, F, nullptr, MT_OUT_F16, b->live_ffn, plan->N, s));
  MT_STEP(MT_LNF_FFN_LN,
          mt_layernorm_fwd_live(b->a1, F, nullptr, MT_OUT_F16, 1, w->ffn_ln_w, w->ffn_ln_b, nullptr, 0, b->t16, F, nullptr, MT_OUT_F16, b->stf, M, F,
                                b->live_ffn, plan->N, s));
  e = epi_bias(w->b_fc2);
  if (defer) {
    MT_STEP(MT_LNF_FC2, mt_gemm_nt_f16_live(b->t16, F, nullptr, w->w_fc2, M, D, F, MT_EPI_BIAS, &e, b->br16, D, nullptr, MT_OUT_F16, b->live_ffn, plan->N, s));
  } else {
    e.resid = b->hmid; e.ldr = D;
    if (drop_ffn) e.drop = *drop_ffn;
    MT_STEP(MT_LNF_FC2, mt_gemm_nt_f16(b->t16, F, nullptr, w->w_fc2, M, D, F, MT_EPI_BIAS_RESID, &e, out, D, nullptr, MT_OUT_F32, s));
  }
  return MT_OK;
}

extern "C" int mt_longnet_layer_bwd(const MtLongNetLayerWeights* w, const MtLongNetLayerBuffers* b, const MtDilatedPlan* plan, int M,
                                    int D, int F, int dh16_valid, int feeds_lower, const MtDropout* drop_attn, const MtDropout* drop_ffn,
                                    const MtDropout* drop_lower_ffn, int steps, mt_stream_t s) {
  if (!w || !b || !plan || M < 1 || D != 768) return MT_ERR_BAD_ARG;
  const MtGemmEpilogue none{};
  const mt_half* src16 = b->dh16;
  if (!dh16_valid) {
    MT_STEP(MT_LNB_CAST, mt_cast_f32_to_f16(b->dh, b->dy16, (long)M * D, drop_ffn, D, s));
    src16 = b->dy16;
  }
  MT_STEP(MT_LNB_FC2, mt_gemm_nt_f16_live(src16, D, nullptr, w->wt_fc2, M, F, D, MT_EPI_BIAS, &none, b->dt16, F, nullptr, MT_OUT_F16, b->live_ffn, plan->N, s));
  MT_STEP(MT_LNB_FFN_LN, mt_layernorm_bwd_live(b->dt16, F, nullptr, MT_OUT_F16, b->a1, F, nullptr, MT_OUT_F16, 1, w->ffn_ln_w, b->stf, b->da1, F,
                                               nullptr, MT_OUT_F16, 0, nullptr, nullptr, nullptr, nullptr, M, F, b->live_ffn, plan->N, s));
  MT_STEP(MT_LNB_FC1, mt_gemm_nt_f16_live(b->da1, F, nullptr, w->wt_fc1, M, D, F, MT_EPI_BIAS, &none, b->dy16, D, nullptr, MT_OUT_F16, b->live_ffn, plan->N, s));
  MT_STEP(MT_LNB_LN2, mt_layernorm_bwd_live(b->dy16, D, nullptr, MT_OUT_F16, b->hmid, D, nullptr, MT_OUT_F32, 0, w->ln2_w, b->st2, b->dh, D, nullptr,
                                            MT_OUT_F32, 1, nullptr, nullptr, b->dh16, drop_attn, M, D, b->live_ffn, plan->N, s));
  MT_STEP(MT_LNB_OUT, mt_gemm_nt_f16_live(b->dh16, D, nullptr, w->wt_out, M, D, D, MT_EPI_BIAS, &none, b->u16, D, nullptr, MT_OUT_F16, b->live_attn, plan->N, s));
  MT_STEP(MT_LNB_MIX, mt_dilated_mix_ln_bwd_live(b->u16, b->o_br, b->lse_br, b->lse_tot, plan, w->inner_ln_w, b->stin, b->dmixed, b->delta,
                                                 b->live_attn, s));
  MT_STEP(MT_ATTN_BWD_ALL << MT_LNB_ATTN_SHIFT, mt_dilated_attn_bwd_inplace_live(b->qkv, b->dmixed, b->lse_tot, b->delta, plan, b->attn_ws, b->dqkv16,
                                                                         (steps >> MT_LNB_ATTN_SHIFT) & MT_ATTN_BWD_ALL, b->live_attn, s));
  MT_STEP(MT_LNB_QKV, mt_gemm_nt_f16_live(b->dqkv16, 3 * D, nullptr, w->wt_qkv, M, D, 3 * D, MT_EPI_BIAS, &none, b->dy16, D, nullptr, MT_OUT_F16, b->live_attn,
                                          plan->N, s));
  MT_STEP(MT_LNB_LN1, mt_layernorm_bwd_live(b->dy16, D, nullptr, MT_OUT_F16, b->hin, D, nullptr, MT_OUT_F32, 0, w->ln1_w, b->st1, b->dh, D, nullptr,
                                            MT_OUT_F32, 1, nullptr, nullptr, feeds_lower ? b->dh16 : nullptr,
                                            feeds_lower ? drop_lower_ffn : nullptr, M, D, b->live_attn, plan->N, s));
  return MT_OK;
}

extern "C" int mt_vit_block_fwd(const MtVitBlockWeights* w, const MtVitBlockBuffers* b, const MtDensePlan* plan, int M, int D, int F,
                                const float* pend_x, const mt_half* pend_branch, int defer, float* out, int steps, mt_stream_t s) {
  if (!w || !b || !plan || M < 1 || D != 768 || (!defer && !out)) return MT_ERR_BAD_ARG;
  if (!pend_x)
    MT_STEP(MT_VBF_LN1, mt_layernorm_fwd_eps(b->hin, D, nullptr, MT_OUT_F32, 0, w->n1_w, w->n1_b, nullptr, 0, b->u16, D, nullptr, MT_OUT_F16, b->st1,
                                             M, D, w->n1_eps, s));
  else
    MT_STEP(MT_VBF_LN1, mt_add_layernorm_fwd_eps(pend_x, pend_branch, nullptr, w->n1_w, w->n1_b, b->hin, b->u16, b->st1, M, D, w->n1_eps, s));
  MtGemmEpilogue e = epi_bias(w->b_qkv);
  MT_STEP(MT_VBF_QKV, mt_gemm_nt_f16(b->u16, D, nullptr, w->w_qkv, M, 3 * D, D, MT_EPI_BIAS, &e, b->qkv, 3 * D, nullptr, MT_OUT_F16, s));
  MT_STEP(MT_VBF_ATTN, mt_dense_attn_fwd(b->qkv, plan, b->o16, b->lse, s));
  e = epi_bias(w->b_proj);
  MT_STEP(MT_VBF_PROJ, mt_gemm_nt_f16(b->o16, D, nullptr, w->w_proj, M, D, D, MT_EPI_BIAS, &e, b->br16, D, nullptr, MT_OUT_F16, s));
  MT_STEP(MT_VBF_LN2, mt_add_layernorm_fwd_eps(b->hin, b->br16, nullptr, w->n2_w, w->n2_b, b->hmid, b->u16, b->st2, M, D, w->n2_eps, s));
  e = epi_bias(w->b_fc1);
  MT_STEP(MT_VBF_FC1, mt_gemm_nt_f16(b->u16, D, nullptr, w->w_fc1, M, F, D, MT_EPI_BIAS, &e, b->a1, F, nullptr, MT_OUT_F16, s));
  MT_STEP(MT_VBF_GELU, mt_gelu_f16_fwd(b->a1, b->t16, (long)M * F, s));
  e = epi_bias(w->b_fc2);
  if (defer) {
    MT_STEP(MT_VBF_FC2, mt_gemm_nt_f16(b->t16, F, nullptr, w->w_fc2, M, D, F, MT_EPI_BIAS, &e, b->br16, D, nullptr, MT_OUT_F16, s));
  } else {
    e.resid = b->hmid; e.ldr = D;
    MT_STEP(MT_VBF_FC2, mt_gemm_nt_f16(b->t16, F, nullptr, w->w_fc2, M, D, F, MT_EPI_BIAS_RESID, &e, out, D, nullptr, MT_OUT_F32, s));
  }
  return MT_OK;
}

extern "C" int mt_vit_block_bwd(const MtVitBlockWeights* w, const MtVitBlockBuffers* b, const MtDensePlan* plan, int M, int D, int F,
                                int dh16_valid, int feeds_lower, int steps, mt_stream_t s) {
  if (!w || !b || !plan || M < 1 || D != 768) return MT_ERR_BAD_ARG;
  const MtGemmEpilogue none{};
  const mt_half* src16 = b->dh16;
  if (!dh16_valid) {
    MT_STEP(MT_VBB_CAST, mt_cast_f32_to_f16(b->dh, b->dy16, (long)M * D, nullptr, 0, s));
    src16 = b->dy16;
  }
  MT_STEP(MT_VBB_FC2, mt_gemm_nt_f16(src16, D, nullptr, w->wt_fc2, M, F, D, MT_EPI_BIAS, &none, b->dt16, F, nullptr, MT_OUT_F16, s));
  MT_STEP(MT_VBB_GELU, mt_gelu_f16_bwd(b->a1, b->dt16, b->da1, (long)M * F, s));
  MT_STEP(MT_VBB_FC1, mt_gemm_nt_f16(b->da1, F, nullptr, w->wt_fc1, M, D, F, MT_EPI_BIAS, &none, b->dy16, D, nullptr, MT_OUT_F16, s));
  MT_STEP(MT_VBB_LN2, mt_layernorm_bwd(b->dy16, D, nullptr, MT_OUT_F16, b->hmid, D, nullptr, MT_OUT_F32, 0, w->n2_w, b->st2, b->dh, D, nullptr,
                                       MT_OUT_F32, 1, nullptr, nullptr, b->dh16, nullptr, M, D, s));
  MT_STEP(MT_VBB_PROJ, mt_gemm_nt_f16(b->dh16, D, nullptr, w->wt_proj, M, D, D, MT_EPI_BIAS, &none, b->u16, D, nullptr, MT_OUT_F16, s));
  MT_STEP(MT_DENSE_BWD_ALL << MT_VBB_ATTN_SHIFT, mt_dense_attn_bwd(b->qkv, b->o16, b->u16, b->lse, plan, b->delta, b->dqkv16,
                                                                   (steps >> MT_VBB_ATTN_SHIFT) & MT_DENSE_BWD_ALL, s));
  MT_STEP(MT_VBB_QKV, mt_gemm_nt_f16(b->dqkv16, 3 * D, nullptr, w->wt_qkv, M, D, 3 * D, MT_EPI_BIAS, &none, b->dy16, D, nullptr, MT_OUT_F16, s));
  MT_STEP(MT_VBB_LN1, mt_layernorm_bwd(b->dy16, D, nullptr, MT_OUT_F16, b->hin, D, nullptr, MT_OUT_F32, 0, w->n1_w, b->st1, b->dh, D, nullptr,
                                       MT_OUT_F32, 1, nullptr, nullptr, feeds_lower ? b->dh16 : nullptr, nullptr, M, D, s));
  return MT_OK;
}
```

modaltune_amd/engine.py:

```python
from __future__ import annotations


import os
from typing import Dict, List, Optional, Sequence

import numpy as np
import torch

from . import ops
from ._lib import rowmap
from .config import ModelConfig, attention_sites, branch_table, coords_to_rowcol, segment_lengths, sincos_1d_table, DILATED_RATIOS
from .synth import param_specs
from .tape import Param, Tape, Var

H16 = torch.float16
F32 = torch.float32


class ParamStore:

    def __init__(self, cfg: ModelConfig, group_sizes: Sequence[int], device):
        self.cfg, self.group_sizes, self.device = cfg, list(group_sizes), device
        self.specs = param_specs(cfg, group_sizes)
        off = 0
# ... 89 lines not shown

    def refresh(self):
        r = 0
        for s in self.srcs:
            n = s.shape[0]
            ops.pack_weight(s, self.w[r:r + n], n, self.K, transpose=False)
            r += n
        if self.wt is not None:
            if len(self.srcs) == 1:
                ops.pack_weight(self.srcs[0], self.wt, self.N, self.K, transpose=True)
            else:
                full = torch.empty(self.N, self.K, dtype=F32, device=self.w.device)
                r = 0
                for s in self.srcs:
                    full[r:r + s.shape[0]].copy_(s)
                    r += s.shape[0]
                ops.pack_weight(full, self.wt, self.N, self.K, transpose=True)


class GenePoints:
    __slots__ = ("baseline", "alphas", "weights", "dgenes", "unscale")

    def __init__(self, baseline, alphas, weights, dgenes, unscale=None):
        self.baseline, self.alphas, self.weights, self.dgenes, self.unscale = baseline, alphas, weights, dgenes, unscale


def deterministic_default() -> bool:
    return os.environ.get("MT_DETERMINISTIC", "0") == "1" or torch.are_deterministic_algorithms_enabled()


class Engine:
    DETERMINISTIC_REFUSAL = None

    def __init__(self, cfg: ModelConfig, group_sizes: Sequence[int], device="cuda", deterministic: Optional[bool] = None):
        self.deterministic = deterministic_default() if deterministic is None else bool(deterministic)
        if self.deterministic and self.DETERMINISTIC_REFUSAL:
            raise NotImplementedError(self.DETERMINISTIC_REFUSAL)
        cfg.validate()
        self.cfg, self.device = cfg, torch.device(device)
        self.group_sizes = list(group_sizes)
        self.store = ParamStore(cfg, group_sizes, self.device)
        self.tape = Tape(self.device)
        self._fresh_arenas = {"need": 0, "pool": []}
        self.tape.on_realloc = self._bump_generation
        self._main_tape = self.tape
        self.seg_lengths = segment_lengths(cfg.max_wsi_size, cfg.tile_size)
        self.pos_table = torch.from_numpy(sincos_1d_table(cfg.slide_ngrids, cfg.embed_dim // 2)).to(self.device)
        self._frozen16: Dict[str, _W16] = {}
        self._train16: Dict[str, _W16] = {}
        self._ws: Dict[tuple, Dict[str, torch.Tensor]] = {}
        self._ws_store: Dict[tuple, dict] = {}
        self._caches_ready = False
        self.generation = 0
        self.grad_ready_hook = None
        self.record_markers = False
        self._coord_err = torch.zeros(1, dtype=torch.int32, device=self.device)
        self._coord_err_host = None
        self._coord_err_event = None
        self._pin_ring: List[tuple] = []
        self._pin_next = 0
        self.collect_taps = False
        self.taps: Dict[str, torch.Tensor] = {}
        self._maps: Dict[str, torch.Tensor] = {}
        self.T = cfg.num_tokens
        self._mean_w = torch.full((max(self.T, 2),), 1.0 / max(1, cfg.gene.final_groups), device=self.device)
        sl, G = self.store.slots, len(self.group_sizes)
        offs = [[sl[f"gene_encoder.gene_networks.{i}.{a}.0.{w}"][0] for a, w in ((0, "weight"), (0, "bias"), (1, "weight"), (1, "bias"))]
                for i in range(G)]
        goff = np.concatenate([[0], np.cumsum(self.group_sizes)[:-1]]).astype(np.int64)
        self._gene_offs = torch.tensor(offs, dtype=torch.int64, device=self.device)
        self._gene_sizes = torch.tensor(self.group_sizes, dtype=torch.int32, device=self.device)
        self._gene_goff = torch.from_numpy(goff).to(self.device)
        self._gene_total = int(sum(self.group_sizes))
        self.stochastic = False
        self.rng = torch.zeros(4, dtype=torch.int32, device=self.device)
        self._drop_now = False
        self._fresh_calls, self._site_base = 0, 0
        self._fresh_tick = 0
        self._fresh_pool: Dict[int, list] = {}
        dpr = np.linspace(0.0, float(cfg.drop_path_rate), cfg.depth) if cfg.depth > 1 else np.zeros(1)
        self._layer_path_p = [float(v) for v in dpr]
        self.leaf_stream = os.environ.get("MT_LEAF_STREAM", "0") == "1"
        self.droppath_skip = os.environ.get("MT_DROPPATH_SKIP", "1") != "0"
        self._side, self._side_refs, self._side_busy = None, [], False
        if self.deterministic and self.leaf_stream:
            raise ValueError(self._LEAF_DET)

    _LEAF_DET = "MT_LEAF_STREAM=1 / engine.leaf_stream and the deterministic mode exclude each other: the side stream's weight-gradient " \
                "leaves would share the partial workspace of the main stream's launches"

    def _bump_generation(self):
        self.generation += 1

    def _leaf(self, fn, *keep):
        if self.leaf_stream and self.deterministic:
            raise ValueError(self._LEAF_DET)
        if not self.leaf_stream:
            fn()
            return
        if self._side is None:
            self._side = torch.cuda.Stream(device=self.device)
        self._side.wait_stream(torch.cuda.current_stream(self.device))
        with torch.cuda.stream(self._side):
            fn()
        self._side_refs.extend(keep)
        self._side_busy = True

    def _leaf_join(self):
        if self._side_busy:
            torch.cuda.current_stream(self.device).wait_stream(self._side)
            self._side_refs.clear()
            self._side_busy = False

    def set_stochastic(self, on: bool, seed: int = 0):
        if bool(on) != self.stochastic:
            self.generation += 1
        self.stochastic = bool(on)
        self.rng.copy_(torch.tensor([seed & 0x7FFFFFFF, (seed >> 31) & 0x7FFFFFFF, 0, 0], dtype=torch.int32))

    def _drop(self, site: int, p: float, path_site: int = 0, path_p: float = 0.0, rows_per_pass: int = 1):
        if not self._drop_now or (p <= 0.0 and path_p <= 0.0):
            return None
        off = self._site_base
        return ops.dropout_spec(self.rng, site + off, p, path_site + off, path_p, rows_per_pass)

    def _layer_drops(self, l: int, N: int):
        if l < 0:
            return None, None
        p, pp = float(self.cfg.dropout), self._layer_path_p[l]
        return (self._drop(16 + 4 * l, p, 17 + 4 * l, pp, N), self._drop(18 + 4 * l, p, 19 + 4 * l, pp, N))

    def _live_table(self, ws, B: int):
        depth = self.cfg.depth
        if not (self._drop_now and self.droppath_skip) or "live" not in ws or 2 * depth > ops.LIVE_SITES_MAX \
                or not any(p > 0.0 for p in self._layer_path_p):
            return None
        off = self._site_base
        ops.droppath_live([s + 4 * l + off for l in range(depth) for s in (17, 19)],
                          [self._layer_path_p[l] for l in range(depth) for _ in range(2)], B, self.rng, ws["live"])
        return ws["live"]

    def load_state_dict(self, state, strict=True):
        self.store.load(state, strict)
        self._caches_ready = False
        self.generation += 1

    def _build_caches(self):
        t, dev, cfg = self.store.tensors, self.device, self.cfg
        self._frozen16 = {"patch": _W16([t["patch_embed.proj.weight"]], dev, need_t=False)}
        for l in range(cfg.depth):
            p = f"encoder.layers.{l}."
            self._frozen16[p + "qkv"] = _W16([_scaled_copy(t[p + "self_attn.q_proj.weight"], QK_SCALE_LOG2),
                                              t[p + "self_attn.k_proj.weight"], t[p + "self_attn.v_proj.weight"]], dev)
            self._frozen16[p + "out"] = _W16([t[p + "self_attn.out_proj.weight"]], dev)
            self._frozen16[p + "fc1"] = _W16([t[p + "ffn.fc1.weight"]], dev)
            self._frozen16[p + "fc2"] = _W16([t[p + "ffn.fc2.weight"]], dev)
            self._frozen16[p + "bqkv"] = torch.cat([_scaled_copy(t[p + "self_attn.q_proj.bias"], QK_SCALE_LOG2),
                                                    t[p + "self_attn.k_proj.bias"], t[p + "self_attn.v_proj.bias"]]).contiguous()
        self._layer_w = []
        for l in range(cfg.depth):
            p = f"encoder.layers.{l}."
            f16 = self._frozen16
            self._layer_w.append(ops.struct_of(
                ops.MtLongNetLayerWeights, ln1_w=t[p + "self_attn_layer_norm.weight"], ln1_b=t[p + "self_attn_layer_norm.bias"],
                inner_ln_w=t[p + "self_attn.inner_attn_ln.weight"], inner_ln_b=t[p + "self_attn.inner_attn_ln.bias"],
                ln2_w=t[p + "final_layer_norm.weight"], ln2_b=t[p + "final_layer_norm.bias"], ffn_ln_w=t[p + "ffn.ffn_layernorm.weight"],
# ... 15 lines not shown
        if not self._caches_ready:
            self._build_caches()
            return
        if getattr(self, "_pack_table", None) is None:
            recs = []
            for w in self._train16.values():
                r = 0
                for src in w.srcs:
                    assert src.is_contiguous() and src.shape[1] == w.K
                    recs.append([src.data_ptr(), w.w.data_ptr(), 0 if w.wt is None else w.wt.data_ptr(), src.shape[0], w.K, r,
                                 w.K, w.N])
                    r += src.shape[0]
            self._pack_table = torch.tensor(recs, dtype=torch.int64, device=self.device)
        ops.pack_weights(self._pack_table, self._pack_table.shape[0])

    def _cross_attn_prefixes(self) -> List[str]:
        out = []
        nint = len(self.cfg.interaction_indexes)
        for i in range(nint):
            out.append(f"interactions.{i}.injector.attn.")
            out.append(f"interactions.{i}.extractor.attn.")
            if i == nint - 1 and self.cfg.use_extra_extractor:
                out += [f"interactions.{i}.extra_extractors.{j}.attn." for j in range(2)]
        return out

    def _workspace(self, B: int, L: int, fresh: bool = False, slot: int = 0) -> Dict[str, torch.Tensor]:
        key = (B, L, slot)
        if not fresh and key in self._ws:
            return self._ws[key]
        dev = self.device

        def spec(Lx):
            return self._ws_spec(B, Lx)

        def numel(shape):
            n = 1
            for d in shape:
                n *= d
            return n

        if fresh:
            want = spec(L)
            self._fresh_tick += 1
            for pl in self._fresh_pool.values():
                pl[:] = [st for st in pl if self._fresh_tick - st.get("tick", 0) <= 64]
            pool = self._fresh_pool.setdefault(B, [])
            fit = [st for st in pool if st["cap"] >= L and all(k in st["flat"] for k in want)]
            if fit:
                store = min(fit, key=lambda st: st["cap"])
                pool.remove(store)
            else:
                small = [st for st in pool if all(k in st["flat"] for k in want)]
                cap = max([L] + [st["cap"] + st["cap"] // 4 for st in small])
                if small:
                    pool.remove(max(small, key=lambda st: st["cap"]))
                store = {"cap": cap, "flat": {k: torch.empty(numel(shape), dtype=dt, device=dev) for k, (dt, shape) in spec(cap).items()}}
            store["tick"] = self._fresh_tick
            w = {k: store["flat"][k][:numel(shape)].view(shape) for k, (dt, shape) in want.items()}
            w["_lease"] = _Lease(pool, store)
            return w
        store = self._ws_store.get((B, slot))
        if store is None or L > store["cap"] or (self.stochastic and "x0d" not in store["flat"]):
            cap = L if store is None else max(L, store["cap"] + store["cap"] // 4)
            self._ws_store.pop((B, slot), None)
            self._ws.clear()
            self.generation += 1
            store = {"cap": cap, "flat": {k: torch.empty(numel(shape), dtype=dt, device=dev) for k, (dt, shape) in spec(cap).items()}}
            self._ws_store[(B, slot)] = store
        if len(self._ws) > 64:
            self._ws.clear()
        w = {k: store["flat"][k][:numel(shape)].view(shape) for k, (dt, shape) in spec(L).items()}
        self._ws[key] = w
        return w

    def _ws_spec(self, B: int, Lx: int) -> Dict[str, tuple]:
        cfg = self.cfg
        D, Fd = cfg.embed_dim, cfg.ffn_dim
        nb = len(self.seg_lengths)
        N = Lx + 1
        M, Mp = B * N, B * Lx
        sp = {"x16": (H16, (Lx, cfg.in_chans)), "x0": (F32, (Lx, D)), "prow": (torch.int32, (Lx,)), "pcol": (torch.int32, (Lx,))}
        if self.stochastic:
            sp["x0d"] = (F32, (B * Lx, D))
        for l in range(cfg.depth):
            sp[f"hin{l}"] = (F32, (M, D)); sp[f"hmid{l}"] = (F32, (M, D)); sp[f"qkv{l}"] = (H16, (M, 3 * D))
            sp[f"obr{l}"] = (H16, (nb, M, D)); sp[f"lsebr{l}"] = (F32, (nb, M, 16)); sp[f"lsetot{l}"] = (F32, (M, 16))
            sp[f"a1_{l}"] = (H16, (M, Fd))
            for st in ("st1", "stin", "st2", "stf"):
                sp[f"{st}_{l}"] = (F32, (M, 2))
        for i in range(len(cfg.interaction_indexes)):
            sp[f"hout{i}"] = (F32, (M, D))
        if cfg.first_interaction_layer > 0:
            sp["hpre"] = (F32, (M, D))
        for nm in ("u16", "br16", "dy16", "dh16", "dmixed"):
            sp[nm] = (H16, (M, D))
        for nm in ("t16", "dt16", "da1"):
            sp[nm] = (H16, (M, Fd))
        sp["dh"] = (F32, (M, D)); sp["delta"] = (F32, (nb, M, 16)); sp["dqkv16"] = (H16, (M, 3 * D))
        sp["scratch32"] = (F32, (Mp, D))
        sp["live"] = (torch.int32, (2 * cfg.depth, 2))
        plan = ops.make_plan(branch_table(N, self.seg_lengths, DILATED_RATIOS), N, B)
        sp["attn_ws"] = (H16, (ops.dilated_attn_bwd_workspace_bytes(plan) // 2,))
        if self.deterministic:
            sp["det"] = (F32, (self._det_elems(B, Lx),))
        return sp

    def _det_elems(self, B: int, Lx: int) -> int:
        cfg = self.cfg
        D, E, T, Mp = cfg.embed_dim, cfg.adapter_dim, self.T, B * Lx
        AHn, AHd = cfg.num_heads, cfg.adapter_head_dim
        need = [ops.det_elems("gemm_tn_f16", Mp, n1, n2, 1) for n1, n2 in ((D, E), (E, E), (E, D), (2 * E, D))]
        need += [ops.det_elems("layernorm_bwd", Mp, D), ops.det_elems("inject_resid_bwd", Mp, D),
                 ops.det_elems("inject_attn_bwd_hd", Mp, Lx, T, AHn, AHd), ops.det_elems("extract_attn_bwd_hd", B, T, Lx, AHn, AHd)]
        return max(need)

    def forward(self, x: torch.Tensor, coords, genes: Sequence[torch.Tensor], task_onehots: torch.Tensor,
                need_grad: bool = True, fresh: bool = False, staged: bool = False, geometry=None,
                clinical: Optional[torch.Tensor] = None, share: Optional[dict] = None, tape: Optional[Tape] = None,
                site_group: int = 0, ws_slot: int = 0, attn_maps: Optional[Dict[str, torch.Tensor]] = None,
                points: Optional[GenePoints] = None, stochastic: Optional[bool] = None) -> torch.Tensor:
        cfg, dev, t = self.cfg, self.device, self.store.tensors
        drop_now = bool(self.stochastic and need_grad and stochastic is not False)
        if points is not None:
            if drop_now:
                raise ValueError("points: the path points are evaluated with the stochastic sites off (stochastic=False)")
            self._check_points(points, int(task_onehots.shape[0]))
        if self.store.sync is not None:
            self.store.sync()
        if not self._caches_ready:
            self._build_caches()
        if staged:
            B, L = geometry
        else:
            x = x.reshape(-1, x.shape[-1])
            L = x.shape[0]
            B = task_onehots.shape[0]
        if L < 1 or B < 1:
            raise ValueError(f"empty bag: {L} patches, {B} task passes (a slide needs at least one patch embedding; the reference's "
                             "datasets never produce an empty one, data_utils/datasets.py:213-285)")
        N, D, Fd, E, T = L + 1, cfg.embed_dim, cfg.ffn_dim, cfg.adapter_dim, self.T
        M, Mp = B * N, B * L
        self._maps = self._check_maps(attn_maps, B, L, need_grad) if attn_maps else {}
        ws = self._workspace(B, L, fresh=fresh, slot=ws_slot)
        self.tape = tape if tape is not None else (Tape(self.device, shared=self._fresh_arenas) if fresh else self._main_tape)
        tape = self.tape
        tape.deterministic = self.deterministic
        if fresh:
            tape.lease = ws["_lease"]
            if share is not None:
                share.setdefault("_leases", []).append(ws["_lease"])
        tape.grad_enabled = need_grad
        tape.reset()
        self._drop_now = drop_now
        self._ext_calls = 0
        if fresh and self._drop_now:
            self._fresh_calls += 1
        self._site_base = 4096 * (self._fresh_calls & 0xFFFFF) if fresh else 1024 * int(site_group)
        self._ctx = dict(B=B, L=L, N=N, M=M, Mp=Mp, ws=ws)
        self._ctx["plan"] = self._attention_plan(N, B)
        self._ctx["live"] = self._live_table(ws, B)
        P = self.store.param
        patch_map = rowmap(L, N, 1)
        self._ctx["patch_map"] = patch_map

        if share is not None and "x0" in share and tuple(share["x0"].shape) == (L, D):
            ws["x0"] = share["x0"]
        else:
            self._embed_patches(x, coords, ws, staged, L)
            if share is not None:
                share["x0"] = ws["x0"]

        gene = self._gene_encoder(genes, passes=int(task_onehots.shape[0]), points=points)
        c = self._assemble_tokens(gene, task_onehots, clinical)
        pe = P("gene_pe")

        nint = len(cfg.interaction_indexes)
        src, src_map = ws["x0"], rowmap(L, 0, 0)
        d_in = self._drop(1, float(cfg.dropout), rows_per_pass=L)
        if d_in is not None:
            if "x0d" not in ws:
                ws["x0d"] = torch.empty(B * L, D, dtype=F32, device=dev)
            ops.dropout_f32(ws["x0"], ws["x0d"], B * L, D, d_in, xmap=rowmap(L, 0, 0))
            src, src_map = ws["x0d"], rowmap(L, L, 0)
        a0 = cfg.first_interaction_layer
# ... 313 lines not shown
        o = tape.linear(a, P(pref + "self_attn.out_proj.weight"), P(pref + "self_attn.out_proj.bias"))
        return tape.linear(o, P(pref + "output_proj.weight"), P(pref + "output_proj.bias"), resid=c)

    def _injector(self, i: int, c: Var, pe: Param, src: torch.Tensor, src_map, hin: torch.Tensor, first: bool):
        cfg, ctx, tape, P, t = self.cfg, self._ctx, self.tape, self.store.param, self.store.tensors
        B, L, N, Mp, D, E, T = ctx["B"], ctx["L"], ctx["N"], ctx["Mp"], cfg.embed_dim, cfg.adapter_dim, self.T
        pref = f"interactions.{i}.injector."
        ap = pref + "attn."
        pm = ctx["patch_map"]
        w16 = self._train16
        dev = self.device
        chat = tape.layernorm(c, P(ap + "norm_kq.weight"), P(ap + "norm_kq.bias"), add_rows=pe)
        _, Wk, Wv, _, bk, bv = self._mha_in(ap + "multihead_attn.")
        k, v = tape.linear_group([(chat, Wk, bk), (chat, Wv, bv)])
        xhat = torch.empty(Mp, D, dtype=H16, device=dev)
        st = torch.empty(Mp, 2, dtype=F32, device=dev)
        ops.layernorm_fwd(src, t[ap + "norm.weight"], t[ap + "norm.bias"], xhat, st, Mp, D, xmap=src_map)
        q1 = torch.empty(Mp, E, dtype=H16, device=dev)
        ops.gemm_nt(xhat, w16[ap + "q_proj"].w, q1, Mp, E, D, bias=t[ap + "q_proj.bias"])
        q2 = torch.empty(Mp, E, dtype=H16, device=dev)
        bqi = t[ap + "multihead_attn.in_proj_bias"][:E]
        ops.gemm_nt(q1, w16[ap + "q_in"].w, q2, Mp, E, E, bias=bqi)
        a = torch.empty(Mp, E, dtype=H16, device=dev)
        AHn, AHd = cfg.num_heads, cfg.adapter_head_dim
        alse = torch.empty(Mp, AHn, dtype=F32, device=dev)
        ops.inject_attn_fwd(q2, k.data, v.data, a, Mp, L, T, lse=alse, heads=AHn, head_dim=AHd)
        wmap = self._maps.get(ap + "multihead_attn")
        if wmap is not None:
            ops.inject_attn_probs(q2, k.data, alse, wmap, Mp, L, T, heads=AHn, head_dim=AHd)
        o1 = torch.empty(Mp, E, dtype=H16, device=dev)
        ops.gemm_nt(a, w16[ap + "out_in"].w, o1, Mp, E, E, bias=t[ap + "multihead_attn.out_proj.bias"])
        ops.gemm_nt(o1, w16[ap + "output_proj"].w, hin, Mp, D, E, cmap=pm, epilogue=ops.EPI_INJECT, bias=t[ap + "output_proj.bias"],
                    resid=src, ldr=D, rmap=src_map, colscale=t[pref + "gamma"])
        g = self.store.grads
        ws = ctx["ws"]
        det = ws.get("det")

        def bwd():
            dh = ws["dh"]
            proj = torch.empty(Mp, D, dtype=H16, device=dev)
            ops.gemm_nt(o1, w16[ap + "output_proj"].w, proj, Mp, D, E, bias=t[ap + "output_proj.bias"])
            dproj = torch.empty(Mp, D, dtype=H16, device=dev)
            ops.inject_resid_bwd(dh, src, proj, t[pref + "gamma"], dh if not first else ws["scratch32"], dproj,
                                 g[pref + "gamma"], Mp, D, dymap=pm, xmap=src_map, dxmap=pm if not first else None, det=det)
            self._leaf(lambda: ops.gemm_tn(dproj, o1, g[ap + "output_proj.weight"], Mp, D, E, colsum=g[ap + "output_proj.bias"], det=det), dproj, o1)
            do1 = torch.empty(Mp, E, dtype=H16, device=dev)
            ops.gemm_nt(dproj, w16[ap + "output_proj"].wt, do1, Mp, E, D)
            self._leaf(lambda: ops.gemm_tn(do1, a, g[ap + "multihead_attn.out_proj.weight"], Mp, E, E, colsum=g[ap + "multihead_attn.out_proj.bias"], det=det),
                       do1, a)
            da = torch.empty(Mp, E, dtype=H16, device=dev)
            ops.gemm_nt(do1, w16[ap + "out_in"].wt, da, Mp, E, E)
            dq2 = torch.empty(Mp, E, dtype=H16, device=dev)
            ops.inject_attn_bwd(q2, a, alse, da, k.data, v.data, dq2, k.g(), v.g(), Mp, L, T, heads=AHn, head_dim=AHd, det=det)
            self._leaf(lambda: ops.gemm_tn(dq2, q1, g[ap + "multihead_attn.q_proj_weight"], Mp, E, E, colsum=g[ap + "multihead_attn.in_proj_bias"][:E], det=det),
                       dq2, q1)
            dq1 = torch.empty(Mp, E, dtype=H16, device=dev)
            ops.gemm_nt(dq2, w16[ap + "q_in"].wt, dq1, Mp, E, E)
            self._leaf(lambda: ops.gemm_tn(dq1, xhat, g[ap + "q_proj.weight"], Mp, E, D, colsum=g[ap + "q_proj.bias"], det=det), dq1, xhat)
            dxhat = torch.empty(Mp, D, dtype=H16, device=dev)
            ops.gemm_nt(dq1, w16[ap + "q_proj"].wt, dxhat, Mp, D, E)
            if first:
                ops.layernorm_bwd(dxhat, src, t[ap + "norm.weight"], st, ws["scratch32"], Mp, D, xmap=src_map,
                                  dw=g[ap + "norm.weight"], db=g[ap + "norm.bias"], det=det)
            else:
                ops.layernorm_bwd(dxhat, src, t[ap + "norm.weight"], st, dh, Mp, D, xmap=src_map, dxmap=pm, accumulate=True,
                                  dw=g[ap + "norm.weight"], db=g[ap + "norm.bias"], det=det)
        tape.record(bwd)

    def _layer(self, l: int, out: torch.Tensor, pend=None, defer: bool = False):
        cfg, ctx = self.cfg, self._ctx
        M, D, Fd, ws, plan = ctx["M"], cfg.embed_dim, cfg.ffn_dim, ctx["ws"], ctx["plan"]
        N_tok = ctx["N"]
        d_attn, d_ffn = self._layer_drops(l, N_tok)
        feeds_lower = all(l != a for a, _ in cfg.interaction_indexes)
        d_lower_ffn = self._layer_drops(l - 1, N_tok)[1] if feeds_lower else None
        live = ctx.get("live")
        cb = ws.get(("_cb", l, live is not None))
        if cb is None:
            cb = ws[("_cb", l, live is not None)] = ops.struct_of(
                ops.MtLongNetLayerBuffers, hin=ws[f"hin{l}"], hmid=ws[f"hmid{l}"], qkv=ws[f"qkv{l}"], o_br=ws[f"obr{l}"], lse_br=ws[f"lsebr{l}"],
                lse_tot=ws[f"lsetot{l}"], a1=ws[f"a1_{l}"], st1=ws[f"st1_{l}"], stin=ws[f"stin_{l}"], st2=ws[f"st2_{l}"], stf=ws[f"stf_{l}"],
                u16=ws["u16"], br16=ws["br16"], t16=ws["t16"], dh=ws["dh"], dy16=ws["dy16"], dh16=ws["dh16"], dt16=ws["dt16"],
                da1=ws["da1"], dmixed=ws["dmixed"], dqkv16=ws["dqkv16"], delta=ws["delta"], attn_ws=ws["attn_ws"],
                live_attn=live[2 * l] if live is not None else None, live_ffn=live[2 * l + 1] if live is not None else None)
        lw = self._layer_w[l]
        ops.longnet_layer_fwd(lw, cb, plan, M, D, Fd, out, pend=pend, defer=defer, drop_attn=d_attn, drop_ffn=d_ffn)

        def bwd():
            ops.longnet_layer_bwd(lw, cb, plan, M, D, Fd, bool(ctx.get("dh16_valid")), feeds_lower, drop_attn=d_attn, drop_ffn=d_ffn,
                                  drop_lower_ffn=d_lower_ffn)
            ctx["dh16_valid"] = feeds_lower
        self.tape.record(bwd)
        return (ws[f"hmid{l}"], ws["br16"], d_ffn) if defer else None

    def _extractor(self, pref: str, c: Var, pe: Param, hout: torch.Tensor) -> Var:
        cfg, ctx, tape, P, t, g = self.cfg, self._ctx, self.tape, self.store.param, self.store.tensors, self.store.grads
        B, L, N, Mp, D, E, T = ctx["B"], ctx["L"], ctx["N"], ctx["Mp"], cfg.embed_dim, cfg.adapter_dim, self.T
        ap = pref + "attn."
        pm, dev, w16, ws = ctx["patch_map"], self.device, self._train16, ctx["ws"]
        xk = torch.empty(Mp, D, dtype=H16, device=dev)
        st = torch.empty(Mp, 2, dtype=F32, device=dev)
        ops.layernorm_fwd(hout, t[ap + "norm_kq.weight"], t[ap + "norm_kq.bias"], xk, st, Mp, D, xmap=pm)
        kv = torch.empty(Mp, 2 * E, dtype=H16, device=dev)
        bkv = t[ap + "multihead_attn.in_proj_bias"][E:]
        ops.gemm_nt(xk, w16[ap + "kv"].w, kv, Mp, 2 * E, D, bias=bkv)
        t2 = tape.layernorm(c, P(ap + "norm.weight"), P(ap + "norm.bias"), add_rows=pe)
        q1 = tape.linear(t2, P(ap + "q_proj.weight"), P(ap + "q_proj.bias"))
        Wq, _, _, bq, _, _ = self._mha_in(ap + "multihead_attn.")
        q2 = tape.linear(q1, Wq, bq)
        out = Var(tape.new(B, T, E))
        AHn, AHd = cfg.num_heads, cfg.adapter_head_dim
        lse = tape.new(B, T, AHn)
        kps = -(-(-(-L // max(1, min(64, L // 256))) ) // 64) * 64
        nsplit = -(-L // kps)
        pa = tape.new(B * AHn * nsplit * T * AHd)
        pml = tape.new(B * AHn * nsplit * T * 2)
        ops.extract_attn_fwd(q2.data, kv, out.data, lse, pa, pml, B, T, L, nsplit, heads=AHn, head_dim=AHd)
        wmap = self._maps.get(ap + "multihead_attn")
        if wmap is not None:
            ops.extract_attn_probs(q2.data, kv, lse, wmap, B, T, L, heads=AHn, head_dim=AHd)

        det = ws.get("det")

        def bwd_core():
            if out.grad is None:
                return
            dkv = torch.empty(Mp, 2 * E, dtype=H16, device=dev)
            ops.extract_attn_bwd(q2.data, kv, out.data, lse, out.grad, q2.g(), dkv, B, T, L, heads=AHn, head_dim=AHd, det=det)
            self._leaf(lambda: ops.gemm_tn(dkv, xk, g[ap + "multihead_attn.k_proj_weight"], Mp, 2 * E, D,
                                           colsum=g[ap + "multihead_attn.in_proj_bias"][E:], det=det), dkv, xk)
            dxk = torch.empty(Mp, D, dtype=H16, device=dev)
            ops.gemm_nt(dkv, w16[ap + "kv"].wt, dxk, Mp, D, 2 * E)
            ops.layernorm_bwd(dxk, hout, t[ap + "norm_kq.weight"], st, ws["dh"], Mp, D, xmap=pm, dxmap=pm, accumulate=True,
                              dw=g[ap + "norm_kq.weight"], db=g[ap + "norm_kq.bias"], det=det)
        tape.record(bwd_core)
        o = tape.linear(out, P(ap + "multihead_attn.out_proj.weight"), P(ap + "multihead_attn.out_proj.bias"))
        c1 = tape.linear(o, P(ap + "output_proj.weight"), P(ap + "output_proj.bias"), resid=c, resid_scale=2.0)
        fp = pref + "ffn."
        tn = tape.layernorm(c1, P(fp + "norm.weight"), P(fp + "norm.bias"))
        f1 = tape.linear(tn, P(fp + "linear1.weight"), P(fp + "linear1.bias"), act=ops.ACT_RELU)
        self._ext_calls = getattr(self, "_ext_calls", 0) + 1
        d_path = self._drop(0, 0.0, 200 + self._ext_calls, float(cfg.drop_path_rate), T)
        return tape.linear(f1, P(fp + "linear2.weight"), P(fp + "linear2.bias"), drop=d_path, resid=c1)

    def _head(self, c: Var, hout: torch.Tensor) -> Var:
        cfg, ctx, tape, P = self.cfg, self._ctx, self.tape, self.store.param
        B, N, D, T, ws = ctx["B"], ctx["N"], cfg.embed_dim, self.T, ctx["ws"]
        nt, ncl, ngc = int(cfg.is_multi), int(cfg.clinical), int(cfg.has_gene_cls)
        off = ncl + nt
        G64 = T - off - ngc
        cls = self._image_token(hout)
        gene = Var(tape.new(B, D))
        if ngc:
            ops.copy_rows(c.data, gene.data, B, D, smap=rowmap(1, T, off))
        else:
            ops.sgemm(self._mean_w, (0, 1), c.data[:, off:], (1, D), gene.data, (D, 1), 1, D, G64, batch=B, b_bs=T * D, c_bs=D)
        task = clin = None
        if nt:
            task = Var(tape.new(B, D))
            ops.copy_rows(c.data, task.data, B, D, smap=rowmap(1, T, ncl))
        if ncl:
            clin = Var(tape.new(B, D))
            ops.copy_rows(c.data, clin.data, B, D, smap=rowmap(1, T, 0))

        def bwd_gather():
            cg = c.g()
            if gene.grad is not None and ngc:
# ... 46 lines not shown
```

modaltune_amd/ops.py:

```python
from __future__ import annotations

import ctypes as C
import os
from typing import Optional, Sequence

import torch

from . import _lib
from ._lib import MtLongNetLayerBuffers, MtLongNetLayerWeights, MtVitBlockBuffers, MtVitBlockWeights
from ._lib import MT_SGEMM_MAX, MtDensePlan, MtDilatedPlan, MtDropout, MtGemmEpilogue, MtRowMap, MtSgemm, check, rowmap

F16, F32 = 0, 1
EPI_BIAS, EPI_BIAS_RESID, EPI_INJECT, EPI_POSEMB, EPI_QKV_HM = 0, 1, 2, 3, 4
ACT_NONE, ACT_RELU, ACT_GELU, ACT_ELU = 0, 1, 2, 3


def _p(t: Optional[torch.Tensor]):
    return None if t is None else t.data_ptr()


_raw_stream = getattr(torch._C, "_cuda_getCurrentRawStream", None)
_raw_device = getattr(torch._C, "_cuda_getDevice", None)


# ... 108 lines not shown
    q.resid_scale, q.a_ld = float(resid_scale), int(a_ld)
    return q


def sgemm_multi(problems):
    for i in range(0, len(problems), MT_SGEMM_MAX):
        chunk = problems[i:i + MT_SGEMM_MAX]
        arr = (MtSgemm * len(chunk))(*chunk)
        check(_lib.load().mt_sgemm_multi(arr, len(chunk), _s()), "sgemm_multi")


def sgemm(A, a_str, B, b_str, Cm, c_str, M, N, K, **k):
    sgemm_multi([sgemm_problem(A, a_str, B, b_str, Cm, c_str, M, N, K, **k)])


def layernorm_fwd(x, w, b, y, stats, M, D, *, ldx=None, xmap=None, ldy=None, ymap=None, gelu_in=False, add_rows=None,
                  add_period=0, eps=1e-5, live=None, live_rows=0):
    if live is not None:
        if eps != 1e-5:
            raise ValueError("layernorm_fwd: a live table goes with the default eps")
        check(_lib.load().mt_layernorm_fwd_live(_p(x), ldx if ldx is not None else D, _rm(xmap), _dt(x), int(gelu_in), _p(w), _p(b),
                                                _p(add_rows), add_period, _p(y), ldy if ldy is not None else D, _rm(ymap), _dt(y),
                                                _p(stats), M, D, _p(live), int(live_rows), _s()), "layernorm_fwd_live")
        return
    check(_lib.load().mt_layernorm_fwd_eps(_p(x), ldx if ldx is not None else D, _rm(xmap), _dt(x), int(gelu_in), _p(w), _p(b),
                                           _p(add_rows), add_period, _p(y), ldy if ldy is not None else D, _rm(ymap), _dt(y),
                                           _p(stats), M, D, float(eps), _s()), "layernorm_fwd")


def add_layernorm_fwd(x, branch, w, b, h, y, stats, M, D, drop=None, eps=1e-5):
    check(_lib.load().mt_add_layernorm_fwd_eps(_p(x), _p(branch), _dr(drop), _p(w), _p(b), _p(h), _p(y), _p(stats), M, D,
                                               float(eps), _s()), "add_layernorm_fwd")


def layernorm_bwd(dy, x, w, stats, dx, M, D, *, lddy=None, dymap=None, ldx=None, xmap=None, lddx=None, dxmap=None,
                  gelu_in=False, accumulate=False, dw=None, db=None, dx16=None, dx16_drop=None, det=None, live=None, live_rows=0):
    if live is not None and dw is not None:
        raise ValueError("layernorm_bwd: a live table goes with a frozen norm (dw / db of a trainable one sum over every row)")
    if det is not None and dw is not None:
        check(_lib.load().mt_layernorm_bwd_det(_p(dy), lddy if lddy is not None else D, _rm(dymap), _dt(dy), _p(x),
                                               ldx if ldx is not None else D, _rm(xmap), _dt(x), int(gelu_in), _p(w), _p(stats),
                                               _p(dx), lddx if lddx is not None else D, _rm(dxmap), _dt(dx), int(accumulate),
                                               _p(dw), _p(db), _p(dx16), _dr(dx16_drop), M, D, *_det(det), _s()), "layernorm_bwd_det")
        return
    args = (_p(dy), lddy if lddy is not None else D, _rm(dymap), _dt(dy), _p(x), ldx if ldx is not None else D, _rm(xmap), _dt(x), int(gelu_in),
            _p(w), _p(stats), _p(dx), lddx if lddx is not None else D, _rm(dxmap), _dt(dx), int(accumulate), _p(dw), _p(db), _p(dx16),
            _dr(dx16_drop), M, D)
    if live is None:
        check(_lib.load().mt_layernorm_bwd(*args, _s()), "layernorm_bwd")
    else:
        check(_lib.load().mt_layernorm_bwd_live(*args, _p(live), int(live_rows), _s()), "layernorm_bwd_live")


LIVE_SITES_MAX = 64


def droppath_live(path_sites, path_ps, B, rng, table):
    n = len(path_sites)
    check(_lib.load().mt_droppath_live((C.c_uint * n)(*path_sites), (C.c_float * n)(*path_ps), n, B, _p(rng), _p(table), _s()),
          "droppath_live")


def dilated_attn_fwd(qkv, plan, o_br, lse_br, live=None):
    if live is None:
        check(_lib.load().mt_dilated_attn_fwd(_p(qkv), C.byref(plan), _p(o_br), _p(lse_br), _s()), "dilated_attn_fwd")
    else:
        check(_lib.load().mt_dilated_attn_fwd_live(_p(qkv), C.byref(plan), _p(o_br), _p(lse_br), _p(live), _s()), "dilated_attn_fwd_live")


def dilated_mix_ln_fwd(o_br, lse_br, plan, ln_w, ln_b, y, stats, lse_tot, live=None):
    args = (_p(o_br), _p(lse_br), C.byref(plan), _p(ln_w), _p(ln_b), _p(y), _p(stats), _p(lse_tot))
    if live is None:
        check(_lib.load().mt_dilated_mix_ln_fwd(*args, _s()), "dilated_mix_ln_fwd")
    else:
        check(_lib.load().mt_dilated_mix_ln_fwd_live(*args, _p(live), _s()), "dilated_mix_ln_fwd_live")


def dilated_mix_ln_bwd(dy, o_br, lse_br, lse_tot, plan, ln_w, stats, dmixed, delta_br, live=None):
    args = (_p(dy), _p(o_br), _p(lse_br), _p(lse_tot), C.byref(plan), _p(ln_w), _p(stats), _p(dmixed), _p(delta_br))
    if live is None:
        check(_lib.load().mt_dilated_mix_ln_bwd(*args, _s()), "dilated_mix_ln_bwd")
    else:
        check(_lib.load().mt_dilated_mix_ln_bwd_live(*args, _p(live), _s()), "dilated_mix_ln_bwd_live")


def dilated_mix_ln_fwd_grid(o_br, lse_br, plan, ln_w, ln_b, y, stats, lse_tot, grid_wgs=0):
    check(_lib.load().mt_dilated_mix_ln_fwd_grid(_p(o_br), _p(lse_br), C.byref(plan), _p(ln_w), _p(ln_b), _p(y), _p(stats),
                                                 _p(lse_tot), int(grid_wgs), _s()), "dilated_mix_ln_fwd_grid")


def dilated_mix_ln_bwd_grid(dy, o_br, lse_br, lse_tot, plan, ln_w, stats, dmixed, delta_br, grid_wgs=0):
    check(_lib.load().mt_dilated_mix_ln_bwd_grid(_p(dy), _p(o_br), _p(lse_br), _p(lse_tot), C.byref(plan), _p(ln_w), _p(stats),
                                                 _p(dmixed), _p(delta_br), int(grid_wgs), _s()), "dilated_mix_ln_bwd_grid")


def dilated_attn_bwd_workspace_bytes(plan) -> int:
    n = _lib.load().mt_dilated_attn_bwd_workspace_bytes(C.byref(plan))
    if n < 0:
        check(int(n), "dilated_attn_bwd_workspace_bytes")
    return int(n)


ATTN_BWD_KV, ATTN_BWD_Q, ATTN_BWD_COMBINE, ATTN_BWD_ALL = 1, 2, 4, 7


def _dilated_attn_bwd_phase(qkv, dmixed, lse_tot, delta_br, plan, workspace, dqkv16, phases):
    check(_lib.load().mt_dilated_attn_bwd(_p(qkv), _p(dmixed), _p(lse_tot), _p(delta_br), C.byref(plan), _p(workspace),
                                          _p(dqkv16), phases, _s()), "dilated_attn_bwd")


def dilated_attn_bwd_phases(qkv, dmixed, lse_tot, delta_br, plan, workspace, dqkv16, phases):
    _dilated_attn_bwd_phase(qkv, dmixed, lse_tot, delta_br, plan, workspace, dqkv16, phases)


def dilated_attn_bwd_inplace_phases(qkv, dmixed, lse_tot, delta_br, plan, workspace, dqkv16, phases=ATTN_BWD_ALL, live=None):
    args = (_p(qkv), _p(dmixed), _p(lse_tot), _p(delta_br), C.byref(plan), _p(workspace), _p(dqkv16), phases)
    if live is None:
        check(_lib.load().mt_dilated_attn_bwd_inplace(*args, _s()), "dilated_attn_bwd_inplace")
    else:
        check(_lib.load().mt_dilated_attn_bwd_inplace_live(*args, _p(live), _s()), "dilated_attn_bwd_inplace_live")


def dilated_attn_bwd(qkv, dmixed, lse_tot, delta_br, plan, workspace, dqkv16):
    if TIMER is None:
        return _dilated_attn_bwd_phase(qkv, dmixed, lse_tot, delta_br, plan, workspace, dqkv16, ATTN_BWD_ALL)
    for key, ph in (("dilated_attn_bwd_kv", ATTN_BWD_KV), ("dilated_attn_bwd_q", ATTN_BWD_Q), ("dilated_attn_bwd_combine", ATTN_BWD_COMBINE)):
        _bracket(key, _dilated_attn_bwd_phase, qkv, dmixed, lse_tot, delta_br, plan, workspace, dqkv16, ph)


DENSE_QK_SCALE_LOG2 = 0.125 * 1.4426950408889634
DENSE_BWD_DELTA, DENSE_BWD_KV, DENSE_BWD_Q, DENSE_BWD_ALL = 1, 2, 4, 7


def make_dense_plan(N: int, B: int, H: int, dist=None, nslope=None) -> MtDensePlan:
    p = MtDensePlan()
    p.N, p.B, p.H = N, B, H
    p.dist = dist.data_ptr() if dist is not None else None
    p.nslope = nslope.data_ptr() if nslope is not None else None
    return p


def alibi_dist_halves(N: int) -> int:
    return int(_lib.load().mt_alibi_dist_halves(N))


def alibi_dist(cells, N, table):
    assert table.numel() >= alibi_dist_halves(N) and table.dtype == torch.float16
    check(_lib.load().mt_alibi_dist(_p(cells), N, _p(table), _s()), "alibi_dist")


def dense_attn_fwd(qkv, plan, o, lse):
    check(_lib.load().mt_dense_attn_fwd(_p(qkv), C.byref(plan), _p(o), _p(lse), _s()), "dense_attn_fwd")


def _dense_attn_bwd_phase(qkv, o, d_o, lse, plan, delta, dqkv, phases):
    check(_lib.load().mt_dense_attn_bwd(_p(qkv), _p(o), _p(d_o), _p(lse), C.byref(plan), _p(delta), _p(dqkv), phases, _s()),
          "dense_attn_bwd")


def dense_attn_bwd(qkv, o, d_o, lse, plan, delta, dqkv):
    if TIMER is None:
        return _dense_attn_bwd_phase(qkv, o, d_o, lse, plan, delta, dqkv, DENSE_BWD_ALL)
    for key, ph in (("dense_attn_delta", DENSE_BWD_DELTA), ("dense_attn_bwd_kv", DENSE_BWD_KV), ("dense_attn_bwd_q", DENSE_BWD_Q)):
        _bracket(key, _dense_attn_bwd_phase, qkv, o, d_o, lse, plan, delta, dqkv, ph)


# ... 394 lines not shown
```

Baseline: 25.04 slides/s.

## Store dilated attention branch outputs in compact per-row layout instead of branch-major

Adds a compact layout for the per-branch attention outputs and log-sum-exp values. Each row stores only the heads its covering branches produce, rather than a full nb x M x D branch-major buffer. The forward attention, mix+LN forward/backward and in-place attention backward get COMPACT template variants that index through per-branch slot offsets. It is enabled by default through MT_ATTN_COMPACT. The goal is to cut memory footprint and bandwidth for o_br/lse_br/delta across all layers, at the cost of extra slot-index arithmetic and less regular access patterns.

Result: no change. 25.03 slides/s (-0.0%).

```diff
diff --git a/include/modaltune_hip.h b/include/modaltune_hip.h
--- a/include/modaltune_hip.h
+++ b/include/modaltune_hip.h
@@ -166,6 +166,27 @@
                                      const MtDilatedPlan* plan, void* workspace, mt_half* dqkv, int phases, const int* live,
                                      mt_stream_t stream);
 
+long mt_dilated_compact_elems(const MtDilatedPlan* plan, int which);
+int mt_dilated_attn_fwd_compact(const mt_half* qkv, const MtDilatedPlan* plan, mt_half* o_c, float* lse_c, mt_stream_t stream);
+int mt_dilated_attn_fwd_compact_live(const mt_half* qkv, const MtDilatedPlan* plan, mt_half* o_c, float* lse_c, const int* live,
+                                     mt_stream_t stream);
+int mt_dilated_mix_ln_fwd_compact(const mt_half* o_c, const float* lse_c, const MtDilatedPlan* plan, const float* ln_w,
+                                  const float* ln_b, mt_half* y, float* stats, float* lse_tot, mt_stream_t stream);
+int mt_dilated_mix_ln_fwd_compact_live(const mt_half* o_c, const float* lse_c, const MtDilatedPlan* plan, const float* ln_w,
+                                       const float* ln_b, mt_half* y, float* stats, float* lse_tot, const int* live,
+                                       mt_stream_t stream);
+int mt_dilated_mix_ln_bwd_compact(const mt_half* dy, const mt_half* o_c, const float* lse_c, const float* lse_tot,
+                                  const MtDilatedPlan* plan, const float* ln_w, const float* stats, mt_half* dmixed,
+                                  float* delta_c, mt_stream_t stream);
+int mt_dilated_mix_ln_bwd_compact_live(const mt_half* dy, const mt_half* o_c, const float* lse_c, const float* lse_tot,
+                                       const MtDilatedPlan* plan, const float* ln_w, const float* stats, mt_half* dmixed,
+                                       float* delta_c, const int* live, mt_stream_t stream);
+int mt_dilated_attn_bwd_inplace_compact(const mt_half* qkv, const mt_half* dmixed, const float* lse_tot, const float* delta_c,
+                                        const MtDilatedPlan* plan, void* workspace, mt_half* dqkv, int phases, mt_stream_t stream);
+int mt_dilated_attn_bwd_inplace_compact_live(const mt_half* qkv, const mt_half* dmixed, const float* lse_tot, const float* delta_c,
+                                             const MtDilatedPlan* plan, void* workspace, mt_half* dqkv, int phases, const int* live,
+                                             mt_stream_t stream);
+
 #define MT_DENSE_QK_SCALE_LOG2 0.18033688011112042f
 typedef struct {
   int N;
@@ -201,6 +222,7 @@
   mt_half *u16, *br16, *t16;
   float* dh; mt_half *dy16, *dh16, *dt16, *da1, *dmixed, *dqkv16; float* delta; void* attn_ws;
   const int *live_attn, *live_ffn;
+  long attn_branch_major;
 } MtLongNetLayerBuffers;
 enum { MT_LAYER_ALL = 0x7fffffff };
 enum { MT_LNF_LN1 = 1 << 0, MT_LNF_QKV = 1 << 1, MT_LNF_ATTN = 1 << 2, MT_LNF_MIX = 1 << 3, MT_LNF_OUT = 1 << 4, MT_LNF_LN2 = 1 << 5,
diff --git a/modaltune_amd/_lib.py b/modaltune_amd/_lib.py
--- a/modaltune_amd/_lib.py
+++ b/modaltune_amd/_lib.py
@@ -52,7 +52,8 @@
 
 class MtLongNetLayerBuffers(C.Structure):
     _fields_ = [(n, P) for n in ("hin", "hmid", "qkv", "o_br", "lse_br", "lse_tot", "a1", "st1", "stin", "st2", "stf", "u16", "br16", "t16",
-                                 "dh", "dy16", "dh16", "dt16", "da1", "dmixed", "dqkv16", "delta", "attn_ws", "live_attn", "live_ffn")]
+                                 "dh", "dy16", "dh16", "dt16", "da1", "dmixed", "dqkv16", "delta", "attn_ws", "live_attn", "live_ffn")] + \
+               [("attn_branch_major", L)]
 
 
 class MtVitBlockWeights(C.Structure):
@@ -94,6 +95,15 @@
     "mt_dilated_mix_ln_bwd_live": [P, P, P, P, PL, P, P, P, P, P, P],
     "mt_dilated_attn_bwd_inplace_live": [P, P, P, P, PL, P, P, I, P, P],
     "mt_dilated_attn_fwd": [P, PL, P, P, P],
+    "mt_dilated_compact_elems": [PL, I],
+    "mt_dilated_attn_fwd_compact": [P, PL, P, P, P],
+    "mt_dilated_attn_fwd_compact_live": [P, PL, P, P, P, P],
+    "mt_dilated_mix_ln_fwd_compact": [P, P, PL, P, P, P, P, P, P],
+    "mt_dilated_mix_ln_fwd_compact_live": [P, P, PL, P, P, P, P, P, P, P],
+    "mt_dilated_mix_ln_bwd_compact": [P, P, P, P, PL, P, P, P, P, P],
+    "mt_dilated_mix_ln_bwd_compact_live": [P, P, P, P, PL, P, P, P, P, P, P],
+    "mt_dilated_attn_bwd_inplace_compact": [P, P, P, P, PL, P, P, I, P],
+    "mt_dilated_attn_bwd_inplace_compact_live": [P, P, P, P, PL, P, P, I, P, P],
     "mt_dilated_mix_ln_fwd": [P, P, PL, P, P, P, P, P, P],
     "mt_dilated_mix_ln_bwd": [P, P, P, P, PL, P, P, P, P, P],
     "mt_dilated_mix_ln_fwd_grid": [P, P, PL, P, P, P, P, P, I, P],
@@ -176,7 +186,7 @@
     "mt_extract_attn_bwd_hd_det_elems": [I, I, I, I, I],
     "mt_extract_attn_bwd_hd_det": [P, P, P, P, P, I, I, I, I, I, P, P, P, L, P],
 }
-_RESTYPE = {"mt_status_string": C.c_char_p, "mt_build_id": C.c_char_p, "mt_dilated_attn_bwd_workspace_bytes": C.c_long, "mt_pool_attn_workspace_floats": C.c_long,
+_RESTYPE = {"mt_status_string": C.c_char_p, "mt_build_id": C.c_char_p, "mt_dilated_attn_bwd_workspace_bytes": C.c_long, "mt_dilated_compact_elems": C.c_long, "mt_pool_attn_workspace_floats": C.c_long,
              "mt_alibi_dist_halves": C.c_long,
              **{n + "_det_elems": C.c_long for n in ("mt_gemm_tn_f16", "mt_colsum_f16", "mt_layernorm_bwd", "mt_inject_resid_bwd",
                                                      "mt_inject_attn_bwd_hd", "mt_extract_attn_bwd_hd")}}
diff --git a/modaltune_amd/csrc/attn.hip b/modaltune_amd/csrc/attn.hip
--- a/modaltune_amd/csrc/attn.hip
+++ b/modaltune_amd/csrc/attn.hip
@@ -2,7 +2,7 @@
 
 namespace {
 
-template <bool LIVE>
+template <bool LIVE, bool COMPACT>
 __global__ __launch_bounds__(256) void dilated_attn_fwd_kernel(const h16* __restrict__ qkv, Plan p, h16* __restrict__ o_br,
                                                                float* __restrict__ lse_br) {
   __shared__ __attribute__((aligned(16))) h16 smem[4 * IMG_HALVES];
@@ -156,7 +156,7 @@
   if (qvalid) {
     const float l = o1[8];
     const float inv = 1.0f / l;
-    h16* orow = o_br + ((long)w.br * M + qrow) * DM + w.h * HD;
+    h16* orow = COMPACT ? o_br + rec_slot(p, w, qrow) : o_br + ((long)w.br * M + qrow) * DM + w.h * HD;
 #pragma unroll
     for (int gq = 0; gq < 4; ++gq) {
       h16x4 v = {(h16)(o0[4 * gq] * inv), (h16)(o0[4 * gq + 1] * inv), (h16)(o0[4 * gq + 2] * inv), (h16)(o0[4 * gq + 3] * inv)};
@@ -167,7 +167,7 @@
       h16x4 v = {(h16)(o1[4 * gq] * inv), (h16)(o1[4 * gq + 1] * inv), (h16)(o1[4 * gq + 2] * inv), (h16)(o1[4 * gq + 3] * inv)};
       *reinterpret_cast<h16x4*>(orow + 32 + 8 * gq + 4 * hh) = v;
     }
-    if (hh == 0) lse_br[((long)w.br * M + qrow) * H + w.h] = (m2 + __log2f(l)) * LN2;
+    if (hh == 0) lse_br[COMPACT ? lse_slot(p, w, qrow) : ((long)w.br * M + qrow) * H + w.h] = (m2 + __log2f(l)) * LN2;
   }
 }
 
@@ -210,7 +210,21 @@
   return v;
 }
 
-template <int NB>
+template <int NB, bool ON>
+struct MixSlots {
+  int o[NB], l[NB];
+  MT_DEVINL MixSlots(const Plan& p, int h, int col) {
+    if (!ON) return;
+    asm volatile("" : "+v"(h));
+#pragma unroll
+    for (int b = 0; b < NB; ++b) {
+      const int slot = h & (p.hb[b] - 1);
+      o[b] = p.rec_off[b] + slot * HD + col;
+      l[b] = p.lse_off[b] + slot;
+    }
+  }
+};
+template <int NB, bool COMPACT>
 __global__ __launch_bounds__(256) void mix_ln_fwd_kernel(const h16* __restrict__ o_br, const float* __restrict__ lse_br, Plan p,
                                                          const float* __restrict__ ln_w, const float* __restrict__ ln_b,
                                                          h16* __restrict__ y, float* __restrict__ stats, float* __restrict__ lse_tot) {
@@ -228,15 +242,21 @@
     const bool live = m2 + sub < m_end;
     const long m = live ? m2 + sub : m_end - 1;
     const int pos = (int)(m % p.N);
+    const MixSlots<NB, COMPACT> sl(p, h, c0 - h * HD);
     bool cov[NB];
     float lse[NB];
     H24 ob[NB];
 #pragma unroll
     for (int b = 0; b < NB; ++b) {
       cov[b] = b < p.nbranch && geo.grp[b] == residue(p, b, pos);
-      const int sb = cov[b] ? b : db;
-      lse[b] = lse_br[((long)sb * M + m) * H + h];
-      ob[b] = ld24(o_br + ((long)sb * M + m) * DM + c0);
+      if (COMPACT) {
+        lse[b] = lse_br[m * p.lse_len + sl.l[b]];
+        ob[b] = ld24(o_br + m * p.rec_len + sl.o[b]);
+      } else {
+        const int sb = cov[b] ? b : db;
+        lse[b] = lse_br[((long)sb * M + m) * H + h];
+        ob[b] = ld24(o_br + ((long)sb * M + m) * DM + c0);
+      }
     }
     float mx = NEG_BIG;
 #pragma unroll
@@ -277,7 +297,7 @@
   }
 }
 
-template <int NB>
+template <int NB, bool COMPACT>
 __global__ __launch_bounds__(256) void mix_ln_bwd_kernel(const h16* __restrict__ dy, const h16* __restrict__ o_br,
                                                          const float* __restrict__ lse_br, const float* __restrict__ lse_tot, Plan p,
                                                          const float* __restrict__ ln_w, const float* __restrict__ stats,
@@ -296,6 +316,7 @@
     const bool live = m2 + sub < m_end;
     const long m = live ? m2 + sub : m_end - 1;
     const int pos = (int)(m % p.N);
+    const MixSlots<NB, COMPACT> sl(p, h, c0 - h * HD);
     const float tot = lse_tot[m * H + h];
     const float mean = stats[2 * m], rstd = stats[2 * m + 1];
     const H24 dyv = ld24(dy + m * DM + c0);
@@ -305,9 +326,14 @@
 #pragma unroll
     for (int b = 0; b < NB; ++b) {
       cov[b] = b < p.nbranch && geo.grp[b] == residue(p, b, pos);
-      const int sb = cov[b] ? b : db;
-      lse[b] = lse_br[((long)sb * M + m) * H + h];
-      ob[b] = ld24(o_br + ((long)sb * M + m) * DM + c0);
+      if (COMPACT) {
+        lse[b] = lse_br[m * p.lse_len + sl.l[b]];
+        ob[b] = ld24(o_br + m * p.rec_len + sl.o[b]);
+      } else {
+        const int sb = cov[b] ? b : db;
+        lse[b] = lse_br[((long)sb * M + m) * H + h];
+        ob[b] = ld24(o_br + ((long)sb * M + m) * DM + c0);
+      }
     }
     float v[MIX_CPL];
 #pragma unroll
@@ -346,30 +372,52 @@
 #pragma unroll
       for (int e = 0; e < MIX_CPL; ++e) d = fmaf(dm[e], h24(ob[b], e), d);
       d += __shfl_xor(d, 1, 64);
-      if (live && (l5 & 1) == 0 && cov[b]) delta_br[((long)b * M + m) * H + h] = d;
-    }
-  }
-}
-
-
-}
-
-extern "C" int mt_dilated_attn_fwd_live(const mt_half* qkv, const MtDilatedPlan* plan, mt_half* o_br, float* lse_br, const int* live,
-                                        mt_stream_t stream) {
+      if (live && (l5 & 1) == 0 && cov[b])
+        delta_br[COMPACT ? m * p.lse_len + sl.l[b] : ((long)b * M + m) * H + h] = d;
+    }
+  }
+}
+
+
+}
+
+namespace {
+int attn_fwd(const mt_half* qkv, const MtDilatedPlan* plan, mt_half* o_br, float* lse_br, const int* live, bool compact, mt_stream_t stream) {
   if (!qkv || !o_br || !lse_br || !plan_ok(plan)) return MT_ERR_BAD_ARG;
   const Plan p = make_plan(plan, 128, live);
   const int nblk = p.blk_off[p.nbranch];
-  if (p.live) hipLaunchKernelGGL(dilated_attn_fwd_kernel<true>, dim3(nblk), dim3(256), 0, (hipStream_t)stream, (const h16*)qkv, p,
-                     (h16*)o_br, lse_br);
-  else hipLaunchKernelGGL(dilated_attn_fwd_kernel<false>, dim3(nblk), dim3(256), 0, (hipStream_t)stream, (const h16*)qkv, p,
-                     (h16*)o_br, lse_br);
+  auto go = [&](auto kernel) {
+    hipLaunchKernelGGL(kernel, dim3(nblk), dim3(256), 0, (hipStream_t)stream, (const h16*)qkv, p, (h16*)o_br, lse_br);
+  };
+  if (compact) { if (p.live) go(dilated_attn_fwd_kernel<true, true>); else go(dilated_attn_fwd_kernel<false, true>); }
+  else { if (p.live) go(dilated_attn_fwd_kernel<true, false>); else go(dilated_attn_fwd_kernel<false, false>); }
   MT_CHECK_LAUNCH();
   return MT_OK;
 }
+}
+
+extern "C" int mt_dilated_attn_fwd_live(const mt_half* qkv, const MtDilatedPlan* plan, mt_half* o_br, float* lse_br, const int* live,
+                                        mt_stream_t stream) {
+  return attn_fwd(qkv, plan, o_br, lse_br, live, false, stream);
+}
 
 extern "C" int mt_dilated_attn_fwd(const mt_half* qkv, const MtDilatedPlan* plan, mt_half* o_br, float* lse_br,
                                    mt_stream_t stream) {
-  return mt_dilated_attn_fwd_live(qkv, plan, o_br, lse_br, nullptr, stream);
+  return attn_fwd(qkv, plan, o_br, lse_br, nullptr, false, stream);
+}
+
+extern "C" int mt_dilated_attn_fwd_compact(const mt_half* qkv, const MtDilatedPlan* plan, mt_half* o_c, float* lse_c, mt_stream_t stream) {
+  return attn_fwd(qkv, plan, o_c, lse_c, nullptr, true, stream);
+}
+
+extern "C" int mt_dilated_attn_fwd_compact_live(const mt_half* qkv, const MtDilatedPlan* plan, mt_half* o_c, float* lse_c, const int* live,
+                                                mt_stream_t stream) {
+  return attn_fwd(qkv, plan, o_c, lse_c, live, true, stream);
+}
+
+extern "C" long mt_dilated_compact_elems(const MtDilatedPlan* plan, int which) {
+  if (!plan_ok(plan) || which < 0 || which > 1) return MT_ERR_BAD_ARG;
+  return (long)plan->B * plan->N * (which == 0 ? compact_rec_len(plan) : compact_lse_len(plan));
 }
 
 constexpr int MIX_CUS = 256, MIX_FWD_WG_PER_CU = 3, MIX_BWD_WG_PER_CU = 2;
@@ -379,17 +427,16 @@
 
 namespace {
 int mix_ln_fwd(const mt_half* o_br, const float* lse_br, const MtDilatedPlan* plan, const float* ln_w, const float* ln_b, mt_half* y,
-               float* stats, float* lse_tot, int grid_wgs, const int* live, mt_stream_t stream) {
+               float* stats, float* lse_tot, int grid_wgs, const int* live, bool compact, mt_stream_t stream) {
   if (!o_br || !lse_br || !ln_w || !ln_b || !y || !stats || !lse_tot || !plan_ok(plan)) return MT_ERR_BAD_ARG;
   const Plan p = make_plan(plan, 128, live);
   const long M = (long)p.B * p.N;
   const dim3 grid = mix_grid(M, grid_wgs, MIX_FWD_WG_PER_CU);
-  if (p.nbranch <= 5)
-    hipLaunchKernelGGL(mix_ln_fwd_kernel<5>, grid, dim3(256), 0, (hipStream_t)stream, (const h16*)o_br, lse_br, p, ln_w, ln_b,
-                       (h16*)y, stats, lse_tot);
-  else
-    hipLaunchKernelGGL(mix_ln_fwd_kernel<MT_MAX_BRANCHES>, grid, dim3(256), 0, (hipStream_t)stream, (const h16*)o_br, lse_br, p,
-                       ln_w, ln_b, (h16*)y, stats, lse_tot);
+  auto go = [&](auto kernel) {
+    hipLaunchKernelGGL(kernel, grid, dim3(256), 0, (hipStream_t)stream, (const h16*)o_br, lse_br, p, ln_w, ln_b, (h16*)y, stats, lse_tot);
+  };
+  if (p.nbranch <= 5) { if (compact) go(mix_ln_fwd_kernel<5, true>); else go(mix_ln_fwd_kernel<5, false>); }
+  else { if (compact) go(mix_ln_fwd_kernel<MT_MAX_BRANCHES, true>); else go(mix_ln_fwd_kernel<MT_MAX_BRANCHES, false>); }
   MT_CHECK_LAUNCH();
   return MT_OK;
 }
@@ -398,34 +445,47 @@
 extern "C" int mt_dilated_mix_ln_fwd_grid(const mt_half* o_br, const float* lse_br, const MtDilatedPlan* plan,
                                           const float* ln_w, const float* ln_b, mt_half* y, float* stats, float* lse_tot,
                                           int grid_wgs, mt_stream_t stream) {
-  return mix_ln_fwd(o_br, lse_br, plan, ln_w, ln_b, y, stats, lse_tot, grid_wgs, nullptr, stream);
+  return mix_ln_fwd(o_br, lse_br, plan, ln_w, ln_b, y, stats, lse_tot, grid_wgs, nullptr, false, stream);
 }
 
 extern "C" int mt_dilated_mix_ln_fwd(const mt_half* o_br, const float* lse_br, const MtDilatedPlan* plan,
                                      const float* ln_w, const float* ln_b, mt_half* y, float* stats, float* lse_tot,
                                      mt_stream_t stream) {
-  return mix_ln_fwd(o_br, lse_br, plan, ln_w, ln_b, y, stats, lse_tot, 0, nullptr, stream);
+  return mix_ln_fwd(o_br, lse_br, plan, ln_w, ln_b, y, stats, lse_tot, 0, nullptr, false, stream);
 }
 
 extern "C" int mt_dilated_mix_ln_fwd_live(const mt_half* o_br, const float* lse_br, const MtDilatedPlan* plan,
                                           const float* ln_w, const float* ln_b, mt_half* y, float* stats, float* lse_tot,
                                           const int* live, mt_stream_t stream) {
-  return mix_ln_fwd(o_br, lse_br, plan, ln_w, ln_b, y, stats, lse_tot, 0, live, stream);
+  return mix_ln_fwd(o_br, lse_br, plan, ln_w, ln_b, y, stats, lse_tot, 0, live, false, stream);
+}
+
+extern "C" int mt_dilated_mix_ln_fwd_compact(const mt_half* o_c, const float* lse_c, const MtDilatedPlan* plan,
+                                             const float* ln_w, const float* ln_b, mt_half* y, float* stats, float* lse_tot,
+                                             mt_stream_t stream) {
+  return mix_ln_fwd(o_c, lse_c, plan, ln_w, ln_b, y, stats, lse_tot, 0, nullptr, true, stream);
+}
+
+extern "C" int mt_dilated_mix_ln_fwd_compact_live(const mt_half* o_c, const float* lse_c, const MtDilatedPlan* plan,
+                                                  const float* ln_w, const float* ln_b, mt_half* y, float* stats, float* lse_tot,
+                                                  const int* live, mt_stream_t stream) {
+  return mix_ln_fwd(o_c, lse_c, plan, ln_w, ln_b, y, stats, lse_tot, 0, live, true, stream);
 }
 
 namespace {
 int mix_ln_bwd(const mt_half* dy, const mt_half* o_br, const float* lse_br, const float* lse_tot, const MtDilatedPlan* plan,
-               const float* ln_w, const float* stats, mt_half* dmixed, float* delta_br, int grid_wgs, const int* live, mt_stream_t stream) {
+               const float* ln_w, const float* stats, mt_half* dmixed, float* delta_br, int grid_wgs, const int* live, bool compact,
+               mt_stream_t stream) {
   if (!dy || !o_br || !lse_br || !lse_tot || !ln_w || !stats || !dmixed || !delta_br || !plan_ok(plan)) return MT_ERR_BAD_ARG;
   const Plan p = make_plan(plan, 128, live);
   const long M = (long)p.B * p.N;
   const dim3 grid = mix_grid(M, grid_wgs, MIX_BWD_WG_PER_CU);
-  if (p.nbranch <= 5)
-    hipLaunchKernelGGL(mix_ln_bwd_kernel<5>, grid, dim3(256), 0, (hipStream_t)stream, (const h16*)dy, (const h16*)o_br, lse_br,
-                       lse_tot, p, ln_w, stats, (h16*)dmixed, delta_br);
-  else
-    hipLaunchKernelGGL(mix_ln_bwd_kernel<MT_MAX_BRANCHES>, grid, dim3(256), 0, (hipStream_t)stream, (const h16*)dy,
-                       (const h16*)o_br, lse_br, lse_tot, p, ln_w, stats, (h16*)dmixed, delta_br);
+  auto go = [&](auto kernel) {
+    hipLaunchKernelGGL(kernel, grid, dim3(256), 0, (hipStream_t)stream, (const h16*)dy, (const h16*)o_br, lse_br, lse_tot, p, ln_w, stats,
+                       (h16*)dmixed, delta_br);
+  };
+  if (p.nbranch <= 5) { if (compact) go(mix_ln_bwd_kernel<5, true>); else go(mix_ln_bwd_kernel<5, false>); }
+  else { if (compact) go(mix_ln_bwd_kernel<MT_MAX_BRANCHES, true>); else go(mix_ln_bwd_kernel<MT_MAX_BRANCHES, false>); }
   MT_CHECK_LAUNCH();
   return MT_OK;
 }
@@ -434,19 +494,31 @@
 extern "C" int mt_dilated_mix_ln_bwd_grid(const mt_half* dy, const mt_half* o_br, const float* lse_br, const float* lse_tot,
                                           const MtDilatedPlan* plan, const float* ln_w, const float* stats, mt_half* dmixed,
                                           float* delta_br, int grid_wgs, mt_stream_t stream) {
-  return mix_ln_bwd(dy, o_br, lse_br, lse_tot, plan, ln_w, stats, dmixed, delta_br, grid_wgs, nullptr, stream);
+  return mix_ln_bwd(dy, o_br, lse_br, lse_tot, plan, ln_w, stats, dmixed, delta_br, grid_wgs, nullptr, false, stream);
 }
 
 extern "C" int mt_dilated_mix_ln_bwd(const mt_half* dy, const mt_half* o_br, const float* lse_br, const float* lse_tot,
                                      const MtDilatedPlan* plan, const float* ln_w, const float* stats, mt_half* dmixed,
                                      float* delta_br, mt_stream_t stream) {
-  return mix_ln_bwd(dy, o_br, lse_br, lse_tot, plan, ln_w, stats, dmixed, delta_br, 0, nullptr, stream);
+  return mix_ln_bwd(dy, o_br, lse_br, lse_tot, plan, ln_w, stats, dmixed, delta_br, 0, nullptr, false, stream);
 }
 
 extern "C" int mt_dilated_mix_ln_bwd_live(const mt_half* dy, const mt_half* o_br, const float* lse_br, const float* lse_tot,
                                           const MtDilatedPlan* plan, const float* ln_w, const float* stats, mt_half* dmixed,
                                           float* delta_br, const int* live, mt_stream_t stream) {
-  return mix_ln_bwd(dy, o_br, lse_br, lse_tot, plan, ln_w, stats, dmixed, delta_br, 0, live, stream);
+  return mix_ln_bwd(dy, o_br, lse_br, lse_tot, plan, ln_w, stats, dmixed, delta_br, 0, live, false, stream);
+}
+
+extern "C" int mt_dilated_mix_ln_bwd_compact(const mt_half* dy, const mt_half* o_c, const float* lse_c, const float* lse_tot,
+                                             const MtDilatedPlan* plan, const float* ln_w, const float* stats, mt_half* dmixed,
+                                             float* delta_c, mt_stream_t stream) {
+  return mix_ln_bwd(dy, o_c, lse_c, lse_tot, plan, ln_w, stats, dmixed, delta_c, 0, nullptr, true, stream);
+}
+
+extern "C" int mt_dilated_mix_ln_bwd_compact_live(const mt_half* dy, const mt_half* o_c, const float* lse_c, const float* lse_tot,
+                                                  const MtDilatedPlan* plan, const float* ln_w, const float* stats, mt_half* dmixed,
+                                                  float* delta_c, const int* live, mt_stream_t stream) {
+  return mix_ln_bwd(dy, o_c, lse_c, lse_tot, plan, ln_w, stats, dmixed, delta_c, 0, live, true, stream);
 }
 
 extern "C" long mt_dilated_attn_bwd_workspace_bytes(const MtDilatedPlan* plan) {
@@ -457,14 +529,14 @@
 
 namespace {
 int attn_bwd(const mt_half* qkv, const mt_half* dmixed, const float* lse_tot, const float* delta_br, const MtDilatedPlan* plan,
-             void* workspace, mt_half* dqkv, int phases, bool inplace, const int* live, mt_stream_t stream) {
+             void* workspace, mt_half* dqkv, int phases, bool inplace, const int* live, bool compact, mt_stream_t stream) {
   if (!qkv || !dmixed || !lse_tot || !delta_br || !workspace || !dqkv || !plan_ok(plan) || !(phases & 7)) return MT_ERR_BAD_ARG;
   hipStream_t s = (hipStream_t)stream;
   inplace = inplace && dense_branch_host(plan) >= 0;
   if (inplace && (long)plan->B * plan->N >= (1L << 31)) return MT_ERR_UNSUPPORTED;
   mt_half* dense_dst = inplace ? dqkv : nullptr;
-  if (phases & MT_ATTN_BWD_KV) mt_attn::launch_bwd_kv(qkv, dmixed, lse_tot, delta_br, plan, workspace, dense_dst, live, s);
-  if (phases & MT_ATTN_BWD_Q) mt_attn::launch_bwd_q(qkv, dmixed, lse_tot, delta_br, plan, workspace, dense_dst, live, s);
+  if (phases & MT_ATTN_BWD_KV) mt_attn::launch_bwd_kv(qkv, dmixed, lse_tot, delta_br, plan, workspace, dense_dst, live, compact, s);
+  if (phases & MT_ATTN_BWD_Q) mt_attn::launch_bwd_q(qkv, dmixed, lse_tot, delta_br, plan, workspace, dense_dst, live, compact, s);
   if (phases & MT_ATTN_BWD_COMBINE) {
     if (inplace) mt_attn::launch_bwd_combine_inplace(workspace, plan, dqkv, live, s);
     else mt_attn::launch_bwd_combine(workspace, plan, dqkv, s);
@@ -477,17 +549,29 @@
 extern "C" int mt_dilated_attn_bwd(const mt_half* qkv, const mt_half* dmixed, const float* lse_tot,
                                    const float* delta_br, const MtDilatedPlan* plan, void* workspace, mt_half* dqkv,
                                    int phases, mt_stream_t stream) {
-  return attn_bwd(qkv, dmixed, lse_tot, delta_br, plan, workspace, dqkv, phases, false, nullptr, stream);
+  return attn_bwd(qkv, dmixed, lse_tot, delta_br, plan, workspace, dqkv, phases, false, nullptr, false, stream);
 }
 
 extern "C" int mt_dilated_attn_bwd_inplace(const mt_half* qkv, const mt_half* dmixed, const float* lse_tot,
                                            const float* delta_br, const MtDilatedPlan* plan, void* workspace, mt_half* dqkv,
                                            int phases, mt_stream_t stream) {
-  return attn_bwd(qkv, dmixed, lse_tot, delta_br, plan, workspace, dqkv, phases, true, nullptr, stream);
+  return attn_bwd(qkv, dmixed, lse_tot, delta_br, plan, workspace, dqkv, phases, true, nullptr, false, stream);
 }
 
 extern "C" int mt_dilated_attn_bwd_inplace_live(const mt_half* qkv, const mt_half* dmixed, const float* lse_tot,
                                                 const float* delta_br, const MtDilatedPlan* plan, void* workspace, mt_half* dqkv,
                                                 int phases, const int* live, mt_stream_t stream) {
-  return attn_bwd(qkv, dmixed, lse_tot, delta_br, plan, workspace, dqkv, phases, true, live, stream);
-}
+  return attn_bwd(qkv, dmixed, lse_tot, delta_br, plan, workspace, dqkv, phases, true, live, false, stream);
+}
+
+extern "C" int mt_dilated_attn_bwd_inplace_compact(const mt_half* qkv, const mt_half* dmixed, const float* lse_tot,
+                                                   const float* delta_c, const MtDilatedPlan* plan, void* workspace, mt_half* dqkv,
+                                                   int phases, mt_stream_t stream) {
+  return attn_bwd(qkv, dmixed, lse_tot, delta_c, plan, workspace, dqkv, phases, true, nullptr, true, stream);
+}
+
+extern "C" int mt_dilated_attn_bwd_inplace_compact_live(const mt_half* qkv, const mt_half* dmixed, const float* lse_tot,
+                                                        const float* delta_c, const MtDilatedPlan* plan, void* workspace, mt_half* dqkv,
+                                                        int phases, const int* live, mt_stream_t stream) {
+  return attn_bwd(qkv, dmixed, lse_tot, delta_c, plan, workspace, dqkv, phases, true, live, true, stream);
+}
diff --git a/modaltune_amd/csrc/attn_bwd_kv.hip b/modaltune_amd/csrc/attn_bwd_kv.hip
--- a/modaltune_amd/csrc/attn_bwd_kv.hip
+++ b/modaltune_amd/csrc/attn_bwd_kv.hip
@@ -2,7 +2,7 @@
 
 namespace {
 
-template <bool LIVE>
+template <bool LIVE, bool COMPACT>
 __global__ __launch_bounds__(256, 3) void dilated_attn_bwd_kv_kernel(const h16* __restrict__ qkv, const h16* __restrict__ dmixed,
                                                                   const float* __restrict__ lse_tot, const float* __restrict__ delta_br,
                                                                   Plan p, h16* __restrict__ ws, DenseDst dd) {
@@ -45,15 +45,16 @@
   const h16* const dseq = hm_ptr(dmixed, M, w.h, sq.row(0));
   const DmaLane dl(tid, row_bytes);
   const float* const lbase = lse_tot + sq.row(0) * H + w.h;
-  const float* const dbase = delta_br + ((long)w.br * M + sq.row(0)) * H + w.h;
+  const float* const dbase = delta_br + (COMPACT ? lse_slot(p, w, sq.row(0)) : ((long)w.br * M + sq.row(0)) * H + w.h);
+  const int dstride = COMPACT ? p.lse_len : H;
   float rl2 = 0.f, rdl = 0.f;
   auto issue = [&](int t) {
     dma_tile(Qx + (t & 1) * IMG_HALVES, tile_rsrc(qseq, t * tile_bytes, valid_bytes), dl);
     dma_tile(Dx + (t & 1) * IMG_HALVES, tile_rsrc(dseq, t * tile_bytes, valid_bytes), dl);
     if (tid < 64) {
-      const long off = (long)min(t * 64 + lane, nvq - 1) * sq.dr * H;
-      rl2 = lbase[off];
-      rdl = dbase[off];
+      const long ent = (long)min(t * 64 + lane, nvq - 1) * sq.dr;
+      rl2 = lbase[ent * H];
+      rdl = dbase[ent * dstride];
     }
   };
   auto publish = [&](int t) {
@@ -163,8 +164,11 @@
 
 }
 
-void mt_attn::launch_bwd_kv(const mt_half* qkv, const mt_half* dmixed, const float* lse_tot, const float* delta_br, const MtDilatedPlan* plan, void* ws, mt_half* dense_dst, const int* live, hipStream_t s) {
+void mt_attn::launch_bwd_kv(const mt_half* qkv, const mt_half* dmixed, const float* lse_tot, const float* delta_br, const MtDilatedPlan* plan, void* ws, mt_half* dense_dst, const int* live, bool compact, hipStream_t s) {
   const Plan p = make_plan(plan, 128, live);
-  if (p.live) hipLaunchKernelGGL(dilated_attn_bwd_kv_kernel<true>, dim3(p.blk_off[p.nbranch]), dim3(256), 0, s, (const h16*)qkv, (const h16*)dmixed, lse_tot, delta_br, p, (h16*)ws, make_dense_dst(plan, p, dense_dst));
-  else hipLaunchKernelGGL(dilated_attn_bwd_kv_kernel<false>, dim3(p.blk_off[p.nbranch]), dim3(256), 0, s, (const h16*)qkv, (const h16*)dmixed, lse_tot, delta_br, p, (h16*)ws, make_dense_dst(plan, p, dense_dst));
+  auto go = [&](auto kernel) {
+    hipLaunchKernelGGL(kernel, dim3(p.blk_off[p.nbranch]), dim3(256), 0, s, (const h16*)qkv, (const h16*)dmixed, lse_tot, delta_br, p, (h16*)ws, make_dense_dst(plan, p, dense_dst));
+  };
+  if (compact) { if (p.live) go(dilated_attn_bwd_kv_kernel<true, true>); else go(dilated_attn_bwd_kv_kernel<false, true>); }
+  else { if (p.live) go(dilated_attn_bwd_kv_kernel<true, false>); else go(dilated_attn_bwd_kv_kernel<false, false>); }
 }
diff --git a/modaltune_amd/csrc/attn_bwd_q.hip b/modaltune_amd/csrc/attn_bwd_q.hip
--- a/modaltune_amd/csrc/attn_bwd_q.hip
+++ b/modaltune_amd/csrc/attn_bwd_q.hip
@@ -2,7 +2,7 @@
 
 namespace {
 
-template <bool LIVE>
+template <bool LIVE, bool COMPACT>
 __global__ __launch_bounds__(256) void dilated_attn_bwd_q_kernel(const h16* __restrict__ qkv, const h16* __restrict__ dmixed,
                                                                  const float* __restrict__ lse_tot, const float* __restrict__ delta_br,
                                                                  Plan p, h16* __restrict__ ws, DenseDst dd) {
@@ -33,7 +33,7 @@
     qf[ks] = sel8(qvalid, ldg8(hm_ptr(qkv, M, w.h, qrow) + ks * 16 + hh * 8));
     dof[ks] = sel8(qvalid, ldg8(hm_ptr(dmixed, M, w.h, qrow) + ks * 16 + hh * 8));
   }
-  const float L2raw = lse_tot[qrow * H + w.h], dlraw = delta_br[((long)w.br * M + qrow) * H + w.h];
+  const float L2raw = lse_tot[qrow * H + w.h], dlraw = delta_br[COMPACT ? lse_slot(p, w, qrow) : ((long)w.br * M + qrow) * H + w.h];
   const float nl2 = qvalid ? fmaf(-L2raw, LOG2E, LOG2_LN2) : -1.0e30f;
   const float ndl = qvalid ? -dlraw : 0.f;
   f32x16 nl2i, ndli;
@@ -138,8 +138,11 @@
 
 }
 
-void mt_attn::launch_bwd_q(const mt_half* qkv, const mt_half* dmixed, const float* lse_tot, const float* delta_br, const MtDilatedPlan* plan, void* ws, mt_half* dense_dst, const int* live, hipStream_t s) {
+void mt_attn::launch_bwd_q(const mt_half* qkv, const mt_half* dmixed, const float* lse_tot, const float* delta_br, const MtDilatedPlan* plan, void* ws, mt_half* dense_dst, const int* live, bool compact, hipStream_t s) {
   const Plan p = make_plan(plan, 128, live);
-  if (p.live) hipLaunchKernelGGL(dilated_attn_bwd_q_kernel<true>, dim3(p.blk_off[p.nbranch]), dim3(256), 0, s, (const h16*)qkv, (const h16*)dmixed, lse_tot, delta_br, p, (h16*)ws, make_dense_dst(plan, p, dense_dst));
-  else hipLaunchKernelGGL(dilated_attn_bwd_q_kernel<false>, dim3(p.blk_off[p.nbranch]), dim3(256), 0, s, (const h16*)qkv, (const h16*)dmixed, lse_tot, delta_br, p, (h16*)ws, make_dense_dst(plan, p, dense_dst));
+  auto go = [&](auto kernel) {
+    hipLaunchKernelGGL(kernel, dim3(p.blk_off[p.nbranch]), dim3(256), 0, s, (const h16*)qkv, (const h16*)dmixed, lse_tot, delta_br, p, (h16*)ws, make_dense_dst(plan, p, dense_dst));
+  };
+  if (compact) { if (p.live) go(dilated_attn_bwd_q_kernel<true, true>); else go(dilated_attn_bwd_q_kernel<false, true>); }
+  else { if (p.live) go(dilated_attn_bwd_q_kernel<true, false>); else go(dilated_attn_bwd_q_kernel<false, false>); }
 }
diff --git a/modaltune_amd/csrc/attn_common.h b/modaltune_amd/csrc/attn_common.h
--- a/modaltune_amd/csrc/attn_common.h
+++ b/modaltune_amd/csrc/attn_common.h
@@ -24,7 +24,15 @@
   float inv_seg[MT_MAX_BRANCHES];
   int qlimit[MT_MAX_BRANCHES];
   const int* live;
-};
+  int hb[MT_MAX_BRANCHES], rec_off[MT_MAX_BRANCHES], lse_off[MT_MAX_BRANCHES], rec_len, lse_len;
+};
+
+inline int compact_rec_len(const MtDilatedPlan* p) {
+  int hs = 0;
+  for (int b = 0; b < p->nbranch; ++b) hs += H / p->ratio[b];
+  return hs * HD;
+}
+inline int compact_lse_len(const MtDilatedPlan* p) { return (compact_rec_len(p) / HD + 3) & ~3; }
 
 Plan make_plan(const MtDilatedPlan* p, int qtile, const int* live = nullptr) {
   Plan d;
@@ -46,6 +54,15 @@
   }
   d.ws_off[0] = 0;
   for (int b = 0; b < d.nbranch; ++b) d.ws_off[b + 1] = d.ws_off[b] + (long)d.B * d.N * 3 * (H / d.ratio[b]) * HD;
+  int heads = 0;
+  for (int b = 0; b < MT_MAX_BRANCHES; ++b) {
+    const bool in = b < d.nbranch;
+    d.hb[b] = in ? H / d.ratio[b] : 1;
+    d.rec_off[b] = in ? heads * HD : 0;
+    d.lse_off[b] = in ? heads : 0;
+    if (in) heads += d.hb[b];
+  }
+  d.rec_len = compact_rec_len(p); d.lse_len = compact_lse_len(p);
   return d;
 }
 
@@ -181,6 +198,13 @@
 }
 MT_DEVINL h16* ws_base(h16* ws, const DenseDst& dd, const WorkItem& w) { return w.br == dd.br ? dd.base : ws; }
 
+MT_DEVINL long rec_slot(const Plan& p, const WorkItem& w, long token_row) {
+  return token_row * p.rec_len + p.rec_off[w.br] + (w.h & (p.hb[w.br] - 1)) * HD;
+}
+MT_DEVINL long lse_slot(const Plan& p, const WorkItem& w, long token_row) {
+  return token_row * p.lse_len + p.lse_off[w.br] + (w.h & (p.hb[w.br] - 1));
+}
+
 MT_DEVINL Seq make_seq(const Plan& p, const WorkItem& w) {
   Seq q;
   q.n = p.n[w.br]; q.s = p.seg[w.br]; q.dr = p.ratio[w.br];
@@ -252,8 +276,8 @@
 }
 
 namespace mt_attn {
-void launch_bwd_kv(const mt_half* qkv, const mt_half* dmixed, const float* lse_tot, const float* delta_br, const MtDilatedPlan* plan, void* ws, mt_half* dense_dst, const int* live, hipStream_t s);
-void launch_bwd_q(const mt_half* qkv, const mt_half* dmixed, const float* lse_tot, const float* delta_br, const MtDilatedPlan* plan, void* ws, mt_half* dense_dst, const int* live, hipStream_t s);
+void launch_bwd_kv(const mt_half* qkv, const mt_half* dmixed, const float* lse_tot, const float* delta_br, const MtDilatedPlan* plan, void* ws, mt_half* dense_dst, const int* live, bool compact, hipStream_t s);
+void launch_bwd_q(const mt_half* qkv, const mt_half* dmixed, const float* lse_tot, const float* delta_br, const MtDilatedPlan* plan, void* ws, mt_half* dense_dst, const int* live, bool compact, hipStream_t s);
 void launch_bwd_combine(const void* ws, const MtDilatedPlan* plan, mt_half* dqkv, hipStream_t s);
 void launch_bwd_combine_inplace(const void* ws, const MtDilatedPlan* plan, mt_half* dqkv, const int* live, hipStream_t s);
 }
diff --git a/modaltune_amd/csrc/layer.hip b/modaltune_amd/csrc/layer.hip
--- a/modaltune_amd/csrc/layer.hip
+++ b/modaltune_amd/csrc/layer.hip
@@ -28,8 +28,13 @@
   MtGemmEpilogue e = epi_bias(w->b_qkv);
   MT_STEP(MT_LNF_QKV, mt_gemm_nt_f16_live(b->u16, D, nullptr, w->w_qkv, M, 3 * D, D, MT_EPI_QKV_HM, &e, b->qkv, 3 * D, nullptr, MT_OUT_F16, b->live_attn,
                                           plan->N, s));
-  MT_STEP(MT_LNF_ATTN, mt_dilated_attn_fwd_live(b->qkv, plan, b->o_br, b->lse_br, b->live_attn, s));
-  MT_STEP(MT_LNF_MIX, mt_dilated_mix_ln_fwd_live(b->o_br, b->lse_br, plan, w->inner_ln_w, w->inner_ln_b, b->u16, b->stin, b->lse_tot, b->live_attn, s));
+  if (b->attn_branch_major) {
+    MT_STEP(MT_LNF_ATTN, mt_dilated_attn_fwd_live(b->qkv, plan, b->o_br, b->lse_br, b->live_attn, s));
+    MT_STEP(MT_LNF_MIX, mt_dilated_mix_ln_fwd_live(b->o_br, b->lse_br, plan, w->inner_ln_w, w->inner_ln_b, b->u16, b->stin, b->lse_tot, b->live_attn, s));
+  } else {
+    MT_STEP(MT_LNF_ATTN, mt_dilated_attn_fwd_compact_live(b->qkv, plan, b->o_br, b->lse_br, b->live_attn, s));
+    MT_STEP(MT_LNF_MIX, mt_dilated_mix_ln_fwd_compact_live(b->o_br, b->lse_br, plan, w->inner_ln_w, w->inner_ln_b, b->u16, b->stin, b->lse_tot, b->live_attn, s));
+  }
   e = epi_bias(w->b_out);
   MT_STEP(MT_LNF_OUT, mt_gemm_nt_f16_live(b->u16, D, nullptr, w->w_out, M, D, D, MT_EPI_BIAS, &e, b->br16, D, nullptr, MT_OUT_F16, b->live_attn, plan->N, s));
   MT_STEP(MT_LNF_LN2, mt_add_layernorm_fwd(b->hin, b->br16, drop_attn, w->ln2_w, w->ln2_b, b->hmid, b->u16, b->st2, M, D, s));
@@ -66,10 +71,18 @@
   MT_STEP(MT_LNB_LN2, mt_layernorm_bwd_live(b->dy16, D, nullptr, MT_OUT_F16, b->hmid, D, nullptr, MT_OUT_F32, 0, w->ln2_w, b->st2, b->dh, D, nullptr,
                                             MT_OUT_F32, 1, nullptr, nullptr, b->dh16, drop_attn, M, D, b->live_ffn, plan->N, s));
   MT_STEP(MT_LNB_OUT, mt_gemm_nt_f16_live(b->dh16, D, nullptr, w->wt_out, M, D, D, MT_EPI_BIAS, &none, b->u16, D, nullptr, MT_OUT_F16, b->live_attn, plan->N, s));
-  MT_STEP(MT_LNB_MIX, mt_dilated_mix_ln_bwd_live(b->u16, b->o_br, b->lse_br, b->lse_tot, plan, w->inner_ln_w, b->stin, b->dmixed, b->delta,
-                                                 b->live_attn, s));
-  MT_STEP(MT_ATTN_BWD_ALL << MT_LNB_ATTN_SHIFT, mt_dilated_attn_bwd_inplace_live(b->qkv, b->dmixed, b->lse_tot, b->delta, plan, b->attn_ws, b->dqkv16,
-                                                                         (steps >> MT_LNB_ATTN_SHIFT) & MT_ATTN_BWD_ALL, b->live_attn, s));
+  if (b->attn_branch_major) {
+    MT_STEP(MT_LNB_MIX, mt_dilated_mix_ln_bwd_live(b->u16, b->o_br, b->lse_br, b->lse_tot, plan, w->inner_ln_w, b->stin, b->dmixed, b->delta,
+                                                   b->live_attn, s));
+    MT_STEP(MT_ATTN_BWD_ALL << MT_LNB_ATTN_SHIFT, mt_dilated_attn_bwd_inplace_live(b->qkv, b->dmixed, b->lse_tot, b->delta, plan, b->attn_ws, b->dqkv16,
+                                                                           (steps >> MT_LNB_ATTN_SHIFT) & MT_ATTN_BWD_ALL, b->live_attn, s));
+  } else {
+    MT_STEP(MT_LNB_MIX, mt_dilated_mix_ln_bwd_compact_live(b->u16, b->o_br, b->lse_br, b->lse_tot, plan, w->inner_ln_w, b->stin, b->dmixed,
+                                                           b->delta, b->live_attn, s));
+    MT_STEP(MT_ATTN_BWD_ALL << MT_LNB_ATTN_SHIFT,
+            mt_dilated_attn_bwd_inplace_compact_live(b->qkv, b->dmixed, b->lse_tot, b->delta, plan, b->attn_ws, b->dqkv16,
+                                                     (steps >> MT_LNB_ATTN_SHIFT) & MT_ATTN_BWD_ALL, b->live_attn, s));
+  }
   MT_STEP(MT_LNB_QKV, mt_gemm_nt_f16_live(b->dqkv16, 3 * D, nullptr, w->wt_qkv, M, D, 3 * D, MT_EPI_BIAS, &none, b->dy16, D, nullptr, MT_OUT_F16, b->live_attn,
                                           plan->N, s));
   MT_STEP(MT_LNB_LN1, mt_layernorm_bwd_live(b->dy16, D, nullptr, MT_OUT_F16, b->hin, D, nullptr, MT_OUT_F32, 0, w->ln1_w, b->st1, b->dh, D, nullptr,
diff --git a/modaltune_amd/engine.py b/modaltune_amd/engine.py
--- a/modaltune_amd/engine.py
+++ b/modaltune_amd/engine.py
@@ -195,6 +195,7 @@
         self._layer_path_p = [float(v) for v in dpr]
         self.leaf_stream = os.environ.get("MT_LEAF_STREAM", "0") == "1"
         self.droppath_skip = os.environ.get("MT_DROPPATH_SKIP", "1") != "0"
+        self.attn_compact = os.environ.get("MT_ATTN_COMPACT", "1") != "0"
         self._side, self._side_refs, self._side_busy = None, [], False
         if self.deterministic and self.leaf_stream:
             raise ValueError(self._LEAF_DET)
@@ -376,9 +377,13 @@
         sp = {"x16": (H16, (Lx, cfg.in_chans)), "x0": (F32, (Lx, D)), "prow": (torch.int32, (Lx,)), "pcol": (torch.int32, (Lx,))}
         if self.stochastic:
             sp["x0d"] = (F32, (B * Lx, D))
+        plan = ops.make_plan(branch_table(N, self.seg_lengths, DILATED_RATIOS), N, B)
+        o_elems, lse_elems = ops.dilated_compact_elems(plan)
+        o_shape, lse_shape = ((M, o_elems // M), (M, lse_elems // M)) if self.attn_compact else ((nb, M, D), (nb, M, 16))
         for l in range(cfg.depth):
             sp[f"hin{l}"] = (F32, (M, D)); sp[f"hmid{l}"] = (F32, (M, D)); sp[f"qkv{l}"] = (H16, (M, 3 * D))
-            sp[f"obr{l}"] = (H16, (nb, M, D)); sp[f"lsebr{l}"] = (F32, (nb, M, 16)); sp[f"lsetot{l}"] = (F32, (M, 16))
+            sp[f"obr{l}"] = (H16, o_shape)
+            sp[f"lsebr{l}"] = (F32, lse_shape); sp[f"lsetot{l}"] = (F32, (M, 16))
             sp[f"a1_{l}"] = (H16, (M, Fd))
             for st in ("st1", "stin", "st2", "stf"):
                 sp[f"{st}_{l}"] = (F32, (M, 2))
@@ -390,10 +395,9 @@
             sp[nm] = (H16, (M, D))
         for nm in ("t16", "dt16", "da1"):
             sp[nm] = (H16, (M, Fd))
-        sp["dh"] = (F32, (M, D)); sp["delta"] = (F32, (nb, M, 16)); sp["dqkv16"] = (H16, (M, 3 * D))
+        sp["dh"] = (F32, (M, D)); sp["delta"] = (F32, lse_shape); sp["dqkv16"] = (H16, (M, 3 * D))
         sp["scratch32"] = (F32, (Mp, D))
         sp["live"] = (torch.int32, (2 * cfg.depth, 2))
-        plan = ops.make_plan(branch_table(N, self.seg_lengths, DILATED_RATIOS), N, B)
         sp["attn_ws"] = (H16, (ops.dilated_attn_bwd_workspace_bytes(plan) // 2,))
         if self.deterministic:
             sp["det"] = (F32, (self._det_elems(B, Lx),))
@@ -873,7 +877,8 @@
                 lse_tot=ws[f"lsetot{l}"], a1=ws[f"a1_{l}"], st1=ws[f"st1_{l}"], stin=ws[f"stin_{l}"], st2=ws[f"st2_{l}"], stf=ws[f"stf_{l}"],
                 u16=ws["u16"], br16=ws["br16"], t16=ws["t16"], dh=ws["dh"], dy16=ws["dy16"], dh16=ws["dh16"], dt16=ws["dt16"],
                 da1=ws["da1"], dmixed=ws["dmixed"], dqkv16=ws["dqkv16"], delta=ws["delta"], attn_ws=ws["attn_ws"],
-                live_attn=live[2 * l] if live is not None else None, live_ffn=live[2 * l + 1] if live is not None else None)
+                live_attn=live[2 * l] if live is not None else None, live_ffn=live[2 * l + 1] if live is not None else None,
+                attn_branch_major=0 if self.attn_compact else 1)
         lw = self._layer_w[l]
         ops.longnet_layer_fwd(lw, cb, plan, M, D, Fd, out, pend=pend, defer=defer, drop_attn=d_attn, drop_ffn=d_ffn)
 
diff --git a/modaltune_amd/ops.py b/modaltune_amd/ops.py
--- a/modaltune_amd/ops.py
+++ b/modaltune_amd/ops.py
@@ -214,6 +214,44 @@
         check(_lib.load().mt_dilated_mix_ln_bwd(*args, _s()), "dilated_mix_ln_bwd")
     else:
         check(_lib.load().mt_dilated_mix_ln_bwd_live(*args, _p(live), _s()), "dilated_mix_ln_bwd_live")
+
+
+def dilated_compact_elems(plan):
+    n = [int(_lib.load().mt_dilated_compact_elems(C.byref(plan), which)) for which in (0, 1)]
+    if min(n) < 0:
+        check(min(n), "dilated_compact_elems")
+    return n[0], n[1]
+
+
+def dilated_attn_fwd_compact(qkv, plan, o_c, lse_c, live=None):
+    if live is None:
+        check(_lib.load().mt_dilated_attn_fwd_compact(_p(qkv), C.byref(plan), _p(o_c), _p(lse_c), _s()), "dilated_attn_fwd_compact")
+    else:
+        check(_lib.load().mt_dilated_attn_fwd_compact_live(_p(qkv), C.byref(plan), _p(o_c), _p(lse_c), _p(live), _s()), "dilated_attn_fwd_compact_live")
+
+
+def dilated_mix_ln_fwd_compact(o_c, lse_c, plan, ln_w, ln_b, y, stats, lse_tot, live=None):
+    args = (_p(o_c), _p(lse_c), C.byref(plan), _p(ln_w), _p(ln_b), _p(y), _p(stats), _p(lse_tot))
+    if live is None:
+        check(_lib.load().mt_dilated_mix_ln_fwd_compact(*args, _s()), "dilated_mix_ln_fwd_compact")
+    else:
+        check(_lib.load().mt_dilated_mix_ln_fwd_compact_live(*args, _p(live), _s()), "dilated_mix_ln_fwd_compact_live")
+
+
+def dilated_mix_ln_bwd_compact(dy, o_c, lse_c, lse_tot, plan, ln_w, stats, dmixed, delta_c, live=None):
+    args = (_p(dy), _p(o_c), _p(lse_c), _p(lse_tot), C.byref(plan), _p(ln_w), _p(stats), _p(dmixed), _p(delta_c))
+    if live is None:
+        check(_lib.load().mt_dilated_mix_ln_bwd_compact(*args, _s()), "dilated_mix_ln_bwd_compact")
+    else:
+        check(_lib.load().mt_dilated_mix_ln_bwd_compact_live(*args, _p(live), _s()), "dilated_mix_ln_bwd_compact_live")
+
+
+def dilated_attn_bwd_inplace_compact(qkv, dmixed, lse_tot, delta_c, plan, workspace, dqkv16, phases=7, live=None):
+    args = (_p(qkv), _p(dmixed), _p(lse_tot), _p(delta_c), C.byref(plan), _p(workspace), _p(dqkv16), phases)
+    if live is None:
+        check(_lib.load().mt_dilated_attn_bwd_inplace_compact(*args, _s()), "dilated_attn_bwd_inplace_compact")
+    else:
+        check(_lib.load().mt_dilated_attn_bwd_inplace_compact_live(*args, _p(live), _s()), "dilated_attn_bwd_inplace_compact_live")
 
 
 def dilated_mix_ln_fwd_grid(o_br, lse_br, plan, ln_w, ln_b, y, stats, lse_tot, grid_wgs=0):
```
